# KatanaMajesty/Nebulae

Measured on AMD Instinct MI355X. Metric: denoised frames/s (1920x1080: GI 1 spp + SVGF temporal + a-trous), higher is better.
Workload: dtype f32

## Files before the change

### include/nebulae_hip.h

```cpp
#ifndef NEBULAE_HIP_H
#define NEBULAE_HIP_H

#include <stddef.h>
#include <stdint.h>

#ifdef __cplusplus
extern "C" {
#endif

typedef struct neb_ctx neb_ctx;
typedef void* neb_stream;

typedef enum neb_status {
    NEB_OK = 0,
    NEB_ERR_INVALID_ARG = -1,
    NEB_ERR_HIP = -2,
    NEB_ERR_NO_DEVICE = -3,
    NEB_ERR_STATE = -4,
    NEB_ERR_OUT_OF_RANGE = -5
} neb_status;

typedef enum neb_plane {
    NEB_PLANE_RADIANCE = 0,
    NEB_PLANE_NORMAL = 1,
    NEB_PLANE_DEPTH = 2,
    NEB_PLANE_MOMENTS = 3,
    NEB_PLANE_VARIANCE = 4,
    NEB_PLANE_SCRATCH = 5,
    NEB_PLANE_ALBEDO = 6,
    NEB_PLANE_ROUGH_METAL = 7,
    NEB_PLANE_WORLDPOS = 8,
    NEB_PLANE_LDR = 9,
    NEB_PLANE_GEOMETRY = 10,
    NEB_PLANE_HISTORY_LENGTH = 11,
    NEB_PLANE_COUNT = 12
} neb_plane;
#define NEB_PLANE_SUBMESH_ID 12

#define NEB_SLOT_CURRENT (-1)
#define NEB_SLOT_HISTORY (-2)

typedef struct neb_create_info {
    int32_t device;
    uint32_t width;
    uint32_t height;
    uint32_t row_begin;
    uint32_t row_end;
    uint32_t atrous_levels;
} neb_create_info;

typedef struct neb_svgf_params {
    float depthSigma;
    float alpha;
    float varianceEps;
    float phiColor;
    float phiNormal;
    float phiDepth;
} neb_svgf_params;

int neb_create(const neb_create_info* info, neb_ctx** out_ctx);
int neb_resize(neb_ctx* ctx, uint32_t width, uint32_t height);
int neb_destroy(neb_ctx* ctx);
const char* neb_last_error(const neb_ctx* ctx);
const char* neb_version(void);

int neb_marker_push(const char* name);
int neb_marker_pop(void);

int neb_begin_frame(neb_ctx* ctx, uint32_t frame_index);
int neb_end_frame(neb_ctx* ctx);
int neb_current_index(const neb_ctx* ctx);
int neb_history_index(const neb_ctx* ctx);

int neb_svgf_default_params(neb_svgf_params* out);
int neb_svgf_set_params(neb_ctx* ctx, const neb_svgf_params* p);
int neb_svgf_get_params(const neb_ctx* ctx, neb_svgf_params* out);
int neb_set_option(neb_ctx* ctx, const char* key, int value);

int neb_get_plane(neb_ctx* ctx, int plane, int slot, void** dptr, size_t* pitch_bytes, uint32_t* rows);
int neb_upload_rows(neb_ctx* ctx, int plane, int slot, uint32_t row0, uint32_t nrows, const void* host, neb_stream stream);
int neb_download_rows(neb_ctx* ctx, int plane, int slot, uint32_t row0, uint32_t nrows, void* host, neb_stream stream);
int neb_stream_synchronize(neb_ctx* ctx, neb_stream stream);

int neb_svgf_reset_history(neb_ctx* ctx, neb_stream stream);
int neb_svgf_temporal(neb_ctx* ctx, neb_stream stream);
int neb_svgf_atrous(neb_ctx* ctx, neb_stream stream);
int neb_svgf_denoise(neb_ctx* ctx, neb_stream stream);
int neb_svgf_level_times(neb_ctx* ctx, float* out_us, uint32_t capacity, uint32_t* n_out);
struct neb_camera;
int neb_svgf_set_camera(neb_ctx* ctx, int slot, const struct neb_camera* cam);
int neb_svgf_snapshot_transforms(neb_ctx* ctx, int slot, neb_stream stream);
int neb_svgf_debug_delta_table(neb_ctx* ctx, float* host, uint32_t capacity, uint32_t* n_out, neb_stream stream);
int neb_svgf_temporal_rows(neb_ctx* ctx, uint32_t row0, uint32_t row1, neb_stream stream);
int neb_svgf_atrous_level_rows(neb_ctx* ctx, uint32_t level, uint32_t row0, uint32_t row1, neb_stream stream);
int neb_svgf_atrous_level_planes(const neb_ctx* ctx, uint32_t level, int* src_plane, int* src_slot, int* dst_plane, int* dst_slot);

typedef struct neb_halo_plane {
    int32_t plane;
    int32_t slot;
} neb_halo_plane;
typedef struct neb_halo_swap {
    int32_t peer;
    uint32_t send_row0, send_row1;
    uint32_t recv_row0, recv_row1;
} neb_halo_swap;
int neb_strips_unique_id(void* id128);
int neb_strips_comm_create(int device, int n_ranks, int rank, const void* id128, void** out_comm);
int neb_strips_comm_destroy(void* comm);
int neb_strips_group_begin(void);
int neb_strips_group_end(void);
int neb_strips_exchange(neb_ctx* ctx, void* comm, const neb_halo_plane* planes, uint32_t n_planes, const neb_halo_swap* swaps, uint32_t n_swaps,
                        neb_stream stream);
const char* neb_strips_last_error(void);

enum { NEB_STRIPS_ONCE = 0, NEB_STRIPS_PER_LEVEL = 1, NEB_STRIPS_OVERLAP = 2 };
enum { NEB_STRIP_RESET_HISTORY = 1 };
typedef struct neb_strip_plan {
    uint32_t n_strips, strip;
    uint32_t scheme;
    uint32_t flags;
} neb_strip_plan;
typedef struct neb_strip_peers {
    neb_ctx* up;
    neb_ctx* down;
} neb_strip_peers;
struct neb_gi_constants;
int neb_strip_frame(neb_ctx* ctx, const struct neb_gi_constants* constants, void* comm, const neb_strip_plan* plan, neb_stream stream);
int neb_strip_frame_begin(neb_ctx* ctx, const struct neb_gi_constants* constants, const neb_strip_plan* plan, const neb_strip_peers* peers, neb_stream stream);
int neb_strip_frame_finish(neb_ctx* ctx, void* comm, const neb_strip_plan* plan, const neb_strip_peers* peers, neb_stream stream);
int neb_strip_rows(const neb_ctx* ctx, const neb_strip_plan* plan, uint32_t out[8]);


typedef struct neb_geometry_desc {
    float surfaceToWorld[16];
    int32_t materialIndex;
    uint32_t indexStride;
    uint32_t numIndices;
    uint32_t numVertices;
    const void* indices;
    const void* attributes[4];
    uint32_t attributeStrides[4];
    uint32_t _pad;
} neb_geometry_desc;

typedef struct neb_material_desc {
    int32_t textureIndices[3];
    float albedo[4];
    float roughnessMetalness[2];
    uint32_t _pad;
} neb_material_desc;

typedef struct neb_texture_desc {
    const void* rgba8;
    uint32_t width, height;
} neb_texture_desc;

typedef struct neb_gi_constants {
    uint32_t frameIndex;
    uint32_t samplesPerPixel;
    uint32_t maxPathVertices;
    float cameraWorldPos[3];
    float skyColor[3];
    float sunLightDirection[3];
    float sunLightRadiance[3];
    float sunTanHalfAngle;
    float throughputThreshold;
} neb_gi_constants;

typedef struct neb_gi_hit {
    float t;
    uint32_t geometry;
    uint32_t primitive;
    uint32_t flags;
} neb_gi_hit;

typedef struct neb_camera {
    float eye[3], target[3], up[3];
    float vfov_deg, znear, zfar;
} neb_camera;

int neb_gi_set_scene(neb_ctx* ctx, const neb_geometry_desc* geoms, uint32_t n_geoms, const neb_material_desc* mats,
                     uint32_t n_mats, const neb_texture_desc* texs, uint32_t n_texs);
int neb_gi_build_bvh(neb_ctx* ctx, neb_stream stream);
int neb_gi_update_transforms(neb_ctx* ctx, const uint32_t* geometry_indices, const float* surfaceToWorld ,
                             uint32_t n, neb_stream stream);
typedef struct neb_vertex_update {
    uint32_t geometry;
    uint32_t firstVertex, numVertices;
    const void* positions;
    uint32_t positionStride;
    const void* normals;
    uint32_t normalStride;
    const void* tangents;
    uint32_t tangentStride;
} neb_vertex_update;
int neb_gi_update_vertices(neb_ctx* ctx, const neb_vertex_update* updates, uint32_t n, neb_stream stream);
int neb_gi_scene_info(const neb_ctx* ctx, uint32_t* n_triangles, uint32_t* n_nodes);
int neb_gi_scene_bytes(const neb_ctx* ctx, uint64_t out[3]);
int neb_gi_bvh_depth(const neb_ctx* ctx, uint32_t* depth);
int neb_gi_build_passes(const neb_ctx* ctx, uint32_t* passes);
int neb_gi_build_ms(const neb_ctx* ctx, float* ms);
int neb_gi_trace(neb_ctx* ctx, const neb_gi_constants* constants, neb_stream stream);
int neb_gi_trace_rows(neb_ctx* ctx, const neb_gi_constants* constants, uint32_t row0, uint32_t row1, neb_stream stream);
int neb_gi_trace_begin(neb_ctx* ctx, const neb_gi_constants* constants, uint32_t row0, uint32_t row1, neb_stream stream);
int neb_gi_trace_finish(neb_ctx* ctx, neb_stream stream, void* after_shade_event);
int neb_gi_resolve(neb_ctx* ctx, neb_stream stream);
int neb_gi_ray_count(neb_ctx* ctx, uint64_t* rays, int reset, neb_stream stream);
int neb_gi_traversal_stats(neb_ctx* ctx, uint64_t out[5]);
int neb_gi_sun_table_stats(neb_ctx* ctx, uint64_t out[4], neb_stream stream);
int neb_gi_sun_table_build_ms(neb_ctx* ctx, float* ms);
int neb_gi_shadow_tail_mode(neb_ctx* ctx, int* mode, float us[2]);
int neb_gi_wave_stats(neb_ctx* ctx, uint64_t out[6]);
int neb_gi_node_index_stats(neb_ctx* ctx, uint64_t out[5]);
int neb_gi_debug_set_tile_order(neb_ctx* ctx, const uint32_t* order, uint32_t n);
int neb_gi_debug_sun_walk_stats(neb_ctx* ctx, uint64_t out[12]);
int neb_gi_download_hits(neb_ctx* ctx, neb_gi_hit* host, neb_stream stream);
int neb_debug_sort_pairs(neb_ctx* ctx, const uint32_t* keys, const uint32_t* values, uint32_t n, int bits, uint32_t* sorted_values);
int neb_pbr_direct(neb_ctx* ctx, const neb_gi_constants* constants, neb_stream stream);
int neb_tonemap(neb_ctx* ctx, neb_stream stream);
int neb_gbuffer_raycast(neb_ctx* ctx, const neb_camera* camera, neb_stream stream);

#ifdef __cplusplus
}
#endif
#endif
```

### nebulae_amd/_lib.py

```python
import ctypes as C
import os

from . import build as _build

NEB_OK = 0
PLANE_RADIANCE, PLANE_NORMAL, PLANE_DEPTH, PLANE_MOMENTS, PLANE_VARIANCE, PLANE_SCRATCH = 0, 1, 2, 3, 4, 5
PLANE_ALBEDO, PLANE_ROUGH_METAL, PLANE_WORLDPOS, PLANE_LDR, PLANE_GEOMETRY = 6, 7, 8, 9, 10
PLANE_HISTORY_LENGTH = 11
PLANE_SUBMESH_ID = 12
SLOT_CURRENT, SLOT_HISTORY = -1, -2


class NebError(RuntimeError):
    pass


class CreateInfo(C.Structure):
    _fields_ = [("device", C.c_int32), ("width", C.c_uint32), ("height", C.c_uint32), ("row_begin", C.c_uint32),
                ("row_end", C.c_uint32), ("atrous_levels", C.c_uint32)]


class HaloPlane(C.Structure):
    _fields_ = [("plane", C.c_int32), ("slot", C.c_int32)]


class HaloSwap(C.Structure):
    _fields_ = [("peer", C.c_int32), ("send_row0", C.c_uint32), ("send_row1", C.c_uint32), ("recv_row0", C.c_uint32), ("recv_row1", C.c_uint32)]


class SvgfParams(C.Structure):
    _fields_ = [(n, C.c_float) for n in ("depthSigma", "alpha", "varianceEps", "phiColor", "phiNormal", "phiDepth")]


_SIGS = {
    "neb_create": (C.c_int, [C.POINTER(CreateInfo), C.POINTER(C.c_void_p)]),
    "neb_resize": (C.c_int, [C.c_void_p, C.c_uint32, C.c_uint32]),
    "neb_destroy": (C.c_int, [C.c_void_p]),
    "neb_last_error": (C.c_char_p, [C.c_void_p]),
    "neb_version": (C.c_char_p, []),
    "neb_marker_push": (C.c_int, [C.c_char_p]),
    "neb_marker_pop": (C.c_int, []),
    "neb_begin_frame": (C.c_int, [C.c_void_p, C.c_uint32]),
    "neb_end_frame": (C.c_int, [C.c_void_p]),
    "neb_current_index": (C.c_int, [C.c_void_p]),
    "neb_history_index": (C.c_int, [C.c_void_p]),
    "neb_svgf_default_params": (C.c_int, [C.POINTER(SvgfParams)]),
    "neb_svgf_set_params": (C.c_int, [C.c_void_p, C.POINTER(SvgfParams)]),
    "neb_svgf_get_params": (C.c_int, [C.c_void_p, C.POINTER(SvgfParams)]),
    "neb_set_option": (C.c_int, [C.c_void_p, C.c_char_p, C.c_int]),
    "neb_get_plane": (C.c_int, [C.c_void_p, C.c_int, C.c_int, C.POINTER(C.c_void_p), C.POINTER(C.c_size_t),
                                C.POINTER(C.c_uint32)]),
    "neb_upload_rows": (C.c_int, [C.c_void_p, C.c_int, C.c_int, C.c_uint32, C.c_uint32, C.c_void_p, C.c_void_p]),
    "neb_download_rows": (C.c_int, [C.c_void_p, C.c_int, C.c_int, C.c_uint32, C.c_uint32, C.c_void_p, C.c_void_p]),
    "neb_stream_synchronize": (C.c_int, [C.c_void_p, C.c_void_p]),
    "neb_svgf_reset_history": (C.c_int, [C.c_void_p, C.c_void_p]),
    "neb_svgf_snapshot_transforms": (C.c_int, [C.c_void_p, C.c_int, C.c_void_p]),
    "neb_svgf_debug_delta_table": (C.c_int, [C.c_void_p, C.POINTER(C.c_float), C.c_uint32, C.POINTER(C.c_uint32), C.c_void_p]),
    "neb_svgf_level_times": (C.c_int, [C.c_void_p, C.POINTER(C.c_float), C.c_uint32, C.POINTER(C.c_uint32)]),
    "neb_svgf_temporal": (C.c_int, [C.c_void_p, C.c_void_p]),
    "neb_svgf_atrous": (C.c_int, [C.c_void_p, C.c_void_p]),
    "neb_svgf_denoise": (C.c_int, [C.c_void_p, C.c_void_p]),
    "neb_svgf_temporal_rows": (C.c_int, [C.c_void_p, C.c_uint32, C.c_uint32, C.c_void_p]),
    "neb_svgf_atrous_level_rows": (C.c_int, [C.c_void_p, C.c_uint32, C.c_uint32, C.c_uint32, C.c_void_p]),
    "neb_svgf_atrous_level_planes": (C.c_int, [C.c_void_p, C.c_uint32] + [C.POINTER(C.c_int)] * 4),
    "neb_strips_unique_id": (C.c_int, [C.c_void_p]),
    "neb_strips_comm_create": (C.c_int, [C.c_int, C.c_int, C.c_int, C.c_void_p, C.POINTER(C.c_void_p)]),
    "neb_strips_comm_destroy": (C.c_int, [C.c_void_p]),
    "neb_strips_group_begin": (C.c_int, []),
    "neb_strips_group_end": (C.c_int, []),
    "neb_strips_exchange": (C.c_int, [C.c_void_p, C.c_void_p, C.POINTER(HaloPlane), C.c_uint32, C.POINTER(HaloSwap), C.c_uint32, C.c_void_p]),
    "neb_strips_last_error": (C.c_char_p, []),
}



class StripPlan(C.Structure):
    _fields_ = [("n_strips", C.c_uint32), ("strip", C.c_uint32), ("scheme", C.c_uint32), ("flags", C.c_uint32)]


class StripPeers(C.Structure):
    _fields_ = [("up", C.c_void_p), ("down", C.c_void_p)]


class VertexUpdate(C.Structure):
    _fields_ = [("geometry", C.c_uint32), ("firstVertex", C.c_uint32), ("numVertices", C.c_uint32),
                ("positions", C.c_void_p), ("positionStride", C.c_uint32), ("normals", C.c_void_p), ("normalStride", C.c_uint32),
                ("tangents", C.c_void_p), ("tangentStride", C.c_uint32)]


STRIP_SCHEMES = {"once": 0, "per_level": 1, "overlap": 2}
STRIP_RESET_HISTORY = 1


def _gi_sigs():
    from . import scene as S
    return {
        "neb_gi_set_scene": (C.c_int, [C.c_void_p, C.POINTER(S.GeometryDesc), C.c_uint32, C.POINTER(S.MaterialDesc), C.c_uint32,
                                       C.POINTER(S.TextureDesc), C.c_uint32]),
        "neb_gi_build_bvh": (C.c_int, [C.c_void_p, C.c_void_p]),
        "neb_gi_update_transforms": (C.c_int, [C.c_void_p, C.POINTER(C.c_uint32), C.POINTER(C.c_float), C.c_uint32, C.c_void_p]),
        "neb_gi_update_vertices": (C.c_int, [C.c_void_p, C.POINTER(VertexUpdate), C.c_uint32, C.c_void_p]),
        "neb_gi_scene_info": (C.c_int, [C.c_void_p, C.POINTER(C.c_uint32), C.POINTER(C.c_uint32)]),
        "neb_gi_bvh_depth": (C.c_int, [C.c_void_p, C.POINTER(C.c_uint32)]),
        "neb_gi_build_passes": (C.c_int, [C.c_void_p, C.POINTER(C.c_uint32)]),
        "neb_gi_build_ms": (C.c_int, [C.c_void_p, C.POINTER(C.c_float)]),
        "neb_gi_scene_bytes": (C.c_int, [C.c_void_p, C.POINTER(C.c_uint64)]),
        "neb_gi_trace": (C.c_int, [C.c_void_p, C.POINTER(S.GIConstants), C.c_void_p]),
        "neb_gi_trace_rows": (C.c_int, [C.c_void_p, C.POINTER(S.GIConstants), C.c_uint32, C.c_uint32, C.c_void_p]),
        "neb_gi_resolve": (C.c_int, [C.c_void_p, C.c_void_p]),
        "neb_gi_trace_begin": (C.c_int, [C.c_void_p, C.POINTER(S.GIConstants), C.c_uint32, C.c_uint32, C.c_void_p]),
        "neb_gi_trace_finish": (C.c_int, [C.c_void_p, C.c_void_p, C.c_void_p]),
        "neb_gi_ray_count": (C.c_int, [C.c_void_p, C.POINTER(C.c_uint64), C.c_int, C.c_void_p]),
        "neb_gi_traversal_stats": (C.c_int, [C.c_void_p, C.POINTER(C.c_uint64)]),
        "neb_gi_wave_stats": (C.c_int, [C.c_void_p, C.POINTER(C.c_uint64)]),
        "neb_gi_node_index_stats": (C.c_int, [C.c_void_p, C.POINTER(C.c_uint64)]),
        "neb_gi_debug_set_tile_order": (C.c_int, [C.c_void_p, C.c_void_p, C.c_uint32]),
        "neb_gi_debug_sun_walk_stats": (C.c_int, [C.c_void_p, C.POINTER(C.c_uint64)]),
        "neb_gi_sun_table_build_ms": (C.c_int, [C.c_void_p, C.POINTER(C.c_float)]),
        "neb_gi_shadow_tail_mode": (C.c_int, [C.c_void_p, C.POINTER(C.c_int), C.POINTER(C.c_float)]),
        "neb_gi_sun_table_stats": (C.c_int, [C.c_void_p, C.POINTER(C.c_uint64), C.c_void_p]),
        "neb_gi_download_hits": (C.c_int, [C.c_void_p, C.c_void_p, C.c_void_p]),
        "neb_debug_sort_pairs": (C.c_int, [C.c_void_p, C.c_void_p, C.c_void_p, C.c_uint32, C.c_int, C.c_void_p]),
        "neb_pbr_direct": (C.c_int, [C.c_void_p, C.POINTER(S.GIConstants), C.c_void_p]),
        "neb_tonemap": (C.c_int, [C.c_void_p, C.c_void_p]),
        "neb_gbuffer_raycast": (C.c_int, [C.c_void_p, C.POINTER(S.CameraDesc), C.c_void_p]),
        "neb_svgf_set_camera": (C.c_int, [C.c_void_p, C.c_int, C.POINTER(S.CameraDesc)]),
        "neb_strip_frame": (C.c_int, [C.c_void_p, C.POINTER(S.GIConstants), C.c_void_p, C.POINTER(StripPlan), C.c_void_p]),
        "neb_strip_frame_begin": (C.c_int, [C.c_void_p, C.POINTER(S.GIConstants), C.POINTER(StripPlan), C.POINTER(StripPeers), C.c_void_p]),
        "neb_strip_frame_finish": (C.c_int, [C.c_void_p, C.c_void_p, C.POINTER(StripPlan), C.POINTER(StripPeers), C.c_void_p]),
        "neb_strip_rows": (C.c_int, [C.c_void_p, C.POINTER(StripPlan), C.POINTER(C.c_uint32)]),
    }


_LIB = None


def exported_symbols():
    return sorted(set(_SIGS) | set(_gi_sigs()))


def load(build_if_missing=True):
    global _LIB
    if _LIB is not None:
        return _LIB
    path = os.environ.get("NEB_LIB_PATH")
    if not path:
        path = _build.LIB_PATH
        if build_if_missing and _build.needs_build():
            _build.build()
    if not os.path.exists(path):
        raise NebError(f"{path} is missing and could not be built; nebulae_amd has no CPU fallback")
    lib = C.CDLL(path)
    for name, (res, args) in {**_SIGS, **_gi_sigs()}.items():
        fn = getattr(lib, name)
        fn.restype = res
        fn.argtypes = args
    _LIB = lib
    return lib


def check(lib, ctx, rc, what):
    if rc != NEB_OK:
        msg = lib.neb_last_error(ctx)
        raise NebError(f"{what} failed ({rc}): {msg.decode() if msg else '?'}")
```

### nebulae_amd/csrc/gi.hip

```cpp
#include "gi_device.h"
#include "svgf_reproject.h"

namespace neb {

#ifndef NEB_SORT_BITS
#define NEB_SORT_BITS 16
#endif
constexpr int kSortBits = NEB_SORT_BITS;
static_assert(kSortBits >= 1 && kSortBits <= 16, "raysort.hip sorts at most two 8-bit digits");

__device__ __forceinline__ uint32_t bounce_sort_key(float3 o, float3 d, const float* smin, const float* sinv)
{
    const uint32_t oct = (d.x < 0.f ? 1u : 0u) | (d.y < 0.f ? 2u : 0u) | (d.z < 0.f ? 4u : 0u);
    const uint32_t key = (oct << (kSortBits - 3)) | (morton30(o, smin, sinv) >> (30 - (kSortBits - 3)));
    return min(key, (1u << kSortBits) - 2u);
}

struct GiRecords {
    float4* ray_o;
    float4* ray_d;
    float4* hit;
    float4* path;
    float4* state;
    float4* srec;
};
constexpr int kSrO = 0, kSrD = 1, kSrContrib = 2, kSrSum = 3;

struct GiArgs {
    SceneView S;
    neb_gi_constants c;
    GiRecords R;
    const uint32_t* albedo;
    const uint32_t* rough_metal;
    const uint2* world_pos;
    const uint2* normal;
    float4* radiance;
    neb_gi_hit* hits;
    unsigned long long* ray_counter;
    uint32_t* bounce_counts;
    uint32_t* shadow_counts;
    uint32_t* table_counts;
    uint32_t sun_table;
    uint32_t hint_pairs;
    uint32_t W, row_begin, row0, row1, tiles_x;
    uint32_t sample;
    uint32_t bounce;
    uint32_t stats;
    uint32_t defer_resolve;
    const uint32_t* tile_order;
    uint32_t* sort_keys;
    uint32_t* sort_vals;
    const uint32_t* sort_order;
    uint32_t* bsort_keys;
    uint32_t* bsort_vals;
    uint32_t raygen_only;
    float4* list;
    uint32_t* list_counts;
    uint32_t list_cap, list_set;
    float smin[3], sinv[3];
    uint32_t first_px, n_px;
    const ShadeHeader* heads;
    float sun_L[3], sun_B[3], sun_T[3];
};
template <uint32_t RUNS>
__device__ __forceinline__ uint32_t gi_block()
{
    if constexpr (RUNS == 0u)
        return blockIdx.x;
    const uint32_t seg_len = ((gridDim.x + RUNS - 1u) / RUNS + 7u) & ~7u;
    const uint32_t seg = blockIdx.x / seg_len, b = blockIdx.x - seg * seg_len;
    const uint32_t n = min(seg_len, gridDim.x - seg * seg_len);
    const uint32_t q = n >> 3, r = n & 7u, xcd = b & 7u, k = b >> 3;
    return seg * seg_len + (xcd < r ? xcd * (q + 1u) + k : r * (q + 1u) + (xcd - r) * q + k);
}
constexpr uint32_t kShadeRuns = 16u, kRaygenRuns = 16u;
constexpr uint32_t kListSegments = 128u;
#ifndef NEB_LIST_QUAD_BELOW
#define NEB_LIST_QUAD_BELOW 1500000u
#endif
#ifndef NEB_LIST_WAVES
#define NEB_LIST_WAVES 6
#endif

template <uint32_t RUNS = 0u>
__device__ __forceinline__ bool gi_pixel(const GiArgs& a, uint32_t& x, uint32_t& y, size_t& i)
{
    const uint32_t lane = threadIdx.x;
    const uint32_t blk = gi_block<RUNS>();
    const uint32_t tile_x = blk % a.tiles_x, tile_y = blk / a.tiles_x;
    x = tile_x * 8 + (lane & 7);
    y = a.row0 + tile_y * 8 + (lane >> 3);
    i = (size_t)(y - a.row_begin) * a.W + x;
    return x < a.W && y < a.row1;
}

__device__ __forceinline__ void count_rays(uint32_t* block_counts, uint32_t mine, uint32_t slot)
{
    uint32_t total = mine;
#pragma unroll
    for (int off = 32; off > 0; off >>= 1)
        total += __shfl_down(total, off);
    if ((threadIdx.x & 63u) == 0 && total)
        block_counts[slot] += total;
}
__device__ __forceinline__ void count_rays(uint32_t* block_counts, uint32_t mine) { count_rays(block_counts, mine, blockIdx.x); }

#ifndef NEB_RG_STACK
#define NEB_RG_STACK 12
#endif
constexpr int kRgStack = NEB_RG_STACK;
static_assert(32 * (kRgStack * 256 + 1024) <= 160 * 1024 || NEB_TRACE_WAVES < 8, "LDS budget of the closest-hit pass: 32 waves per CU of stacks and child slots in 160 KB");
__global__ __launch_bounds__(64, NEB_TRACE_WAVES) void gi_raygen_trace_kernel(GiArgs a)
{
    __shared__ int stack_mem[kRgStack * 64];
    __shared__ __attribute__((aligned(16))) int child_slot_mem[256];
    uint32_t x, y;
    size_t i64;
    bool active;
    if (a.tile_order) {
        const uint32_t blk = a.tile_order[blockIdx.x], tile_x = blk % a.tiles_x, tile_y = blk / a.tiles_x;
        x = tile_x * 8 + (threadIdx.x & 7);
        y = a.row0 + tile_y * 8 + (threadIdx.x >> 3);
        i64 = (size_t)(y - a.row_begin) * a.W + x;
        active = x < a.W && y < a.row1;
    } else {
        active = gi_pixel<kRaygenRuns>(a, x, y, i64);
    }
    const uint32_t i = (uint32_t)i64, lane = threadIdx.x;
    uint32_t rays = 0;
    uint32_t wave_stamp[5] = {0u, 0u, 0u, 0u, 0u};
    if (active) {
        const float3 albedo = unpack_r11g11b10(a.albedo[i]);
        const uint2 wp = a.world_pos[i];
        const float3 worldPos = f3(half_bits_to_float(wp.x & 0xffffu), half_bits_to_float(wp.x >> 16), half_bits_to_float(wp.y & 0xffffu));
        const uint32_t nzw = a.normal[i].y;
        const float3 SN = oct_unpack(half_bits_to_float(nzw & 0xffffu), half_bits_to_float(nzw >> 16));
        const float metalness = half_bits_to_float(a.rough_metal[i] >> 16);
        uint32_t rng;
        float3 V;
        if (a.sample == 0) {
            rng = jenkins((x + y * a.W) ^ jenkins(a.c.frameIndex));
            V = f3(a.c.cameraWorldPos[0], a.c.cameraWorldPos[1], a.c.cameraWorldPos[2]) - worldPos;
        } else {
            const float4 st = a.R.state[i];
            V = f3(st.x, st.y, st.z);
            rng = __float_as_uint(st.w);
        }
        (void)rand01(rng);
        const float3 F0 = specular_f0(albedo, metalness);
        float3 throughput = f3(1, 1, 1) * (albedo * (1.0f - metalness));
        const float pd = 1.0f - specular_probability(saturate1(dot3(normalize3(V), SN)), F0, albedo);
        if (rand01(rng) < pd)
            throughput = f3(throughput.x / pd, throughput.y / pd, throughput.z / pd);
        const float u0 = rand01(rng), u1 = rand01(rng);
        const float3 dir = cosine_hemisphere_aligned(u0, u1, SN);
        const float3 org = worldPos + SN * 1e-2f;
        const bool bounce = a.c.maxPathVertices > 1;
        a.R.path[i] = make_float4(throughput.x, throughput.y, throughput.z, __uint_as_float(rng));
        a.R.ray_o[i] = make_float4(org.x, org.y, org.z, 0.01f);
        a.R.ray_d[i] = make_float4(dir.x, dir.y, dir.z, bounce ? 1.0f : 0.0f);
        if (a.sample + 1 < a.c.samplesPerPixel)
            a.R.state[i] = make_float4(V.x, V.y, V.z, __uint_as_float(rng));
        float4 h = make_float4(bounce ? -1.0f : -2.0f, 0.f, 0.f, 0.f);
        rays = bounce ? 1u : 0u;
        wave_stamp[0] = wave_stamp[1] = wave_stamp[2] = wave_stamp[3] = wave_stamp[4] = 0u;
        if (a.bsort_keys) {
            a.bsort_keys[i] = bounce ? bounce_sort_key(org, dir, a.smin, a.sinv) : (1u << kSortBits) - 1u;
            a.bsort_vals[i] = (uint32_t)i;
        }
        if (bounce && !a.raygen_only && a.S.n_tris) {
            Hit hit;
            const bool found = a.stats ? traverse_t<false, true, kRgStack, true>(a.S, org, dir, 0.01f, kTraceMax, stack_mem + lane, hit, stack_mem, child_slot_mem + 4u * lane)
                                       : traverse_t<false, false, kRgStack, true>(a.S, org, dir, 0.01f, kTraceMax, stack_mem + lane, hit, stack_mem, child_slot_mem + 4u * lane);
            if (found)
                h = make_float4(hit.t, hit.u, hit.v, __uint_as_float(hit.tri));
            if (a.stats) {
                wave_stamp[0] = hit.w_iters, wave_stamp[1] = hit.w_node_iters, wave_stamp[2] = hit.w_node_lanes, wave_stamp[3] = hit.w_leaf_iters,
                wave_stamp[4] = hit.w_leaf_lanes;
                atomicAdd(a.ray_counter + 1, (unsigned long long)hit.node_visits);
                atomicAdd(a.ray_counter + 2, (unsigned long long)hit.tri_tests);
#pragma unroll
                for (int k = 0; k < 4; ++k)
                    atomicAdd(a.ray_counter + 11 + k, (unsigned long long)hit.top_visits[k]);
                atomicAdd(a.ray_counter + 15, (unsigned long long)hit.deep_sp);
                a.R.srec[4 * i + kSrContrib].w = __uint_as_float(hit.node_visits + ((hit.tri_tests + 3u) >> 2));
            }
        }
        a.R.hit[i] = h;
    }
    count_rays(a.bounce_counts, rays);
    if (a.stats) {
#pragma unroll
        for (int k = 0; k < 5; ++k) {
            uint32_t v = wave_stamp[k];
#pragma unroll
            for (int off = 32; off > 0; off >>= 1)
                v = max(v, (uint32_t)__shfl_xor((int)v, off));
            if (lane == 0)
                atomicAdd(a.ray_counter + 6 + k, (unsigned long long)v);
        }
        if (lane == 0)
            atomicAdd(a.ray_counter + 5, 1ull);
    }
}

__global__ __launch_bounds__(64, NEB_TRACE_WAVES) void gi_bounce_trace_kernel(GiArgs a)
{
    __shared__ int stack_mem[kLdsStack * 64];
    uint32_t x, y;
    size_t i = 0;
    bool active;
    if (a.sort_order) {
        const uint32_t j = blockIdx.x * 64u + threadIdx.x;
        active = j < a.n_px;
        if (active)
            i = a.sort_order[j];
    } else {
        active = gi_pixel(a, x, y, i);
    }
    uint32_t rays = 0;
    if (active) {
        const float4 rd = a.R.ray_d[i];
        if (rd.w != 0.0f) {
            const float4 ro = a.R.ray_o[i];
            Hit hit;
            rays = 1;
            float4 h = make_float4(-1.0f, 0.f, 0.f, 0.f);
            if (traverse(a.S, f3(ro.x, ro.y, ro.z), f3(rd.x, rd.y, rd.z), ro.w, kTraceMax, false, stack_mem + threadIdx.x, hit))
                h = make_float4(hit.t, hit.u, hit.v, __uint_as_float(hit.tri));
            a.R.hit[i] = h;
        }
    }
    if (a.bounce > 1)
        count_rays(a.bounce_counts, rays);
}

struct ShadeOut {
    float4 rec_o = {0.f, 0.f, 0.f, 0.f}, shadow_d = {0.f, 0.f, 0.f, 0.f} , rec_c = {0.f, 0.f, 0.f, 0.f}, sum = {0.f, 0.f, 0.f, 0.f};
    uint32_t rays = 0;
    uint32_t table = 0;
};

template <bool FAST>
__device__ __forceinline__ void shade_pixel(const GiArgs& a, size_t i, const float4 h, const float4 pth, const float4 rd, const float4 ro, ShadeOut& o,
                                            const float4* staged, uint32_t staged_swz)
{
    const uint32_t trav_iters = a.stats ? __float_as_uint(a.R.srec[4 * i + kSrContrib].w) : 0u;
    float3 throughput = f3(pth.x, pth.y, pth.z);
    if (!(a.sample == 0 && a.bounce == 1))
        o.sum = a.R.srec[4 * i + kSrSum];
    float4 next_d = make_float4(0.f, 0.f, 0.f, 0.f);
    neb_gi_hit dbg = {-1.0f, ~0u, ~0u, 0u};
    const bool alive = rd.w != 0.0f;
    if (alive && h.x == -1.0f) {
        o.sum.x += a.c.skyColor[0] * throughput.x;
        o.sum.y += a.c.skyColor[1] * throughput.y;
        o.sum.z += a.c.skyColor[2] * throughput.z;
    } else if (alive && h.x >= 0.0f) {
        const uint32_t tri = __float_as_uint(h.w);
        Surface surf;
        const TriShade ts = load_tri_shade_at(staged, staged_swz);
        const ShadeHead head = load_shade_header(a.heads, ts.geom);
        const bool hint_fetch = a.sun_table && a.hint_pairs && !((ts.lit >> ts.hint_side) & 1u) && ts.hint[0] != kNoHint;
        float4 ha0 = make_float4(0.f, 0.f, 0.f, 0.f), hb0 = ha0, hc0 = ha0, ha1 = ha0, hb1 = ha0, hc1 = ha0;
        if (hint_fetch) {
            const uint32_t h0 = ts.hint[0], h1 = ts.hint[1] != kNoHint ? ts.hint[1] : h0;
            ha0 = a.S.tris[3 * h0], hb0 = a.S.tris[3 * h0 + 1], hc0 = a.S.tris[3 * h0 + 2];
            ha1 = a.S.tris[3 * h1], hb1 = a.S.tris[3 * h1 + 1], hc1 = a.S.tris[3 * h1 + 2];
        }
        const bool shaded = reconstruct_surface<FAST>(a.S, head, ts, h.y, h.z, surf);
        dbg.t = h.x;
        dbg.geometry = ts.geom;
        if (a.hits)
            dbg.primitive = __float_as_uint(a.S.shade[8 * (size_t)tri + 7].x);
        if (shaded) {
            const float3 org = f3(ro.x, ro.y, ro.z), dir = f3(rd.x, rd.y, rd.z);
            const float3 hitP = org + dir * h.x;
            const float3 V = normalize3<FAST>(-dir);
            uint32_t rng = __float_as_uint(pth.w);
            const float a0 = rand01(rng), a1 = rand01(rng);
            const float angle = a0 * 2.0f * 3.1415926535f, dist = fsqrt<false>(a1);
            const float3 sun_rad = f3(a.c.sunLightRadiance[0], a.c.sunLightRadiance[1], a.c.sunLightRadiance[2]);
            const float3 L = f3(a.sun_L[0], a.sun_L[1], a.sun_L[2]), Bv = f3(a.sun_B[0], a.sun_B[1], a.sun_B[2]), T = f3(a.sun_T[0], a.sun_T[1], a.sun_T[2]);
            float sn_a, cs_a;
            det_sincosf(angle, sn_a, cs_a);
            const float3 inc = normalize3<false>(L + (Bv * sn_a + T * cs_a) * a.c.sunTanHalfAngle * dist);
            const bool transition = dot3(surf.GN, inc) <= 0.0f;
            const float3 so = hitP + (transition ? -surf.GN : surf.GN) * 1e-2f;
            const float3 O = evaluate_direct_brdf<FAST>(surf, V, L) * sun_rad * throughput;
            o.rays = 1;
            const uint32_t side = transition ? 1u : 0u;
            bool hinted_hit = false;
            if (a.sun_table && !((ts.lit >> side) & 1u) && ts.hint_side == side && ts.hint[0] != kNoHint) {
                float tt, uu, vv;
#pragma unroll
                for (int pair = 0; pair < kHints && !hinted_hit; pair += 2) {
                    const uint32_t h0 = ts.hint[pair];
                    if (h0 == kNoHint || (uint32_t)pair >= 2u * a.hint_pairs)
                        break;
                    if (pair == 0) {
                        hinted_hit = intersect_tri_regs(ha0, hb0, hc0, so, inc, 0.001f, kTraceMax, tt, uu, vv) ||
                                     intersect_tri_regs(ha1, hb1, hc1, so, inc, 0.001f, kTraceMax, tt, uu, vv);
                        continue;
                    }
                    const uint32_t h1 = ts.hint[pair + 1] != kNoHint ? ts.hint[pair + 1] : h0;
                    const float4 a0 = a.S.tris[3 * h0], b0 = a.S.tris[3 * h0 + 1], c0 = a.S.tris[3 * h0 + 2];
                    const float4 a1 = a.S.tris[3 * h1], b1 = a.S.tris[3 * h1 + 1], c1 = a.S.tris[3 * h1 + 2];
                    hinted_hit = intersect_tri_regs(a0, b0, c0, so, inc, 0.001f, kTraceMax, tt, uu, vv) ||
                                 intersect_tri_regs(a1, b1, c1, so, inc, 0.001f, kTraceMax, tt, uu, vv);
                }
            }
            if (hinted_hit) {
                o.table = 1;
            } else if (a.sun_table && ((ts.lit >> side) & 1u)) {
                o.sum.x += O.x;
                o.sum.y += O.y;
                o.sum.z += O.z;
                o.table = 1;
                dbg.flags |= 1u;
            } else {
                o.rec_o = make_float4(so.x, so.y, so.z, 0.001f);
                o.shadow_d = make_float4(inc.x, inc.y, inc.z, 1.0f);
                o.rec_c = make_float4(O.x, O.y, O.z, 0.f);
            }
            if (a.bounce + 1 < a.c.maxPathVertices) {
                uint32_t rng_copy = rng;
                const float3 SNn = normalize3<FAST>(surf.SN);
                const float e0 = rand01(rng_copy), e1 = rand01(rng_copy);
                const float3 Ld = cosine_hemisphere_aligned<FAST>(e0, e1, SNn);
                const float pdiff = 1.0f - specular_probability<FAST>(saturate1(dot3(V, SNn)), specular_f0(surf.albedo, surf.metalness), surf.albedo);
                const float3 no = hitP + surf.GN * 1e-2f;
                throughput = throughput * (surf.albedo * (1.0f - surf.metalness));
                if (rand01(rng) < pdiff)
                    throughput = f3(fdiv<FAST>(throughput.x, pdiff), fdiv<FAST>(throughput.y, pdiff), fdiv<FAST>(throughput.z, pdiff));
                a.R.ray_o[i] = make_float4(no.x, no.y, no.z, 0.001f);
                next_d = make_float4(Ld.x, Ld.y, Ld.z, 1.0f);
                a.R.path[i] = make_float4(throughput.x, throughput.y, throughput.z, __uint_as_float(rng));
            }
            if (a.sample + 1 < a.c.samplesPerPixel)
                a.R.state[i] = make_float4(V.x, V.y, V.z, __uint_as_float(rng));
        }
    }
    if (a.bounce + 1 < a.c.maxPathVertices)
        a.R.ray_d[i] = next_d;
    if (a.sort_keys) {
        uint32_t key = (1u << kSortBits) - 1u;
        if (o.shadow_d.w != 0.0f) {
            key = min(morton30(f3(o.rec_o.x, o.rec_o.y, o.rec_o.z), a.smin, a.sinv) >> (30 - kSortBits), (1u << kSortBits) - 2u);
        }
        a.sort_keys[i] = key;
        a.sort_vals[i] = (uint32_t)i;
    }
    if (a.bsort_keys) {
        uint32_t key = (1u << kSortBits) - 1u;
        if (next_d.w != 0.0f) {
            const float4 no4 = a.R.ray_o[i];
            key = bounce_sort_key(f3(no4.x, no4.y, no4.z), f3(next_d.x, next_d.y, next_d.z), a.smin, a.sinv);
        }
        a.bsort_keys[i] = key;
        a.bsort_vals[i] = (uint32_t)i;
    }
    if (a.hits && a.bounce == 1) {
        if (a.stats)
            dbg.flags |= min(trav_iters, 4095u) << 8;
        a.hits[i] = dbg;
    }
}

template <bool FAST>
__global__ __launch_bounds__(64, NEB_SHADE_WAVES) void gi_shade_kernel(GiArgs a)
{
    uint32_t x, y;
    size_t i;
    const bool active = gi_pixel<kShadeRuns>(a, x, y, i);
    ShadeOut o;
    float4 h = make_float4(-2.0f, 0.f, 0.f, 0.f);
    const bool final_vertex = a.sample + 1 == a.c.samplesPerPixel && a.bounce + 1 >= a.c.maxPathVertices && !a.defer_resolve;
    float4 pth = make_float4(0.f, 0.f, 0.f, 0.f), rd = pth, ro = pth, rad = pth;
    if (active) {
        h = a.R.hit[i];
        pth = a.R.path[i];
        rd = a.R.ray_d[i];
        ro = a.R.ray_o[i];
        if (a.list && final_vertex)
            rad = a.radiance[i];
    }
    __shared__ float4 smem[64 * 8];
    const uint32_t lane = threadIdx.x;
    const bool has_hit = active && h.x >= 0.0f;
    const uint32_t my_tri = has_hit ? __float_as_uint(h.w) : ~0u;
#pragma unroll
    for (uint32_t it = 0; it < 8; ++it) {
        const uint32_t src = it * 8u + (lane >> 3);
        const uint32_t t = (uint32_t)__shfl((int)my_tri, (int)src);
        if (t != ~0u) {
            const float4* g = a.S.shade + 8 * (size_t)t + ((lane & 7u) ^ (src & 7u));
            __builtin_amdgcn_global_load_lds((const __attribute__((address_space(1))) void*)g, (__attribute__((address_space(3))) void*)(smem + it * 64u), 16, 0, 0);
        }
    }
    __syncthreads();
    if (active)
        shade_pixel<FAST>(a, i, h, pth, rd, ro, o, smem + lane * 8u, lane & 7u);
    if (a.list) {
        const bool trace = active && o.shadow_d.w != 0.0f;
        if (active && !trace) {
            if (final_vertex) {
                if (o.sum.x != 0.0f || o.sum.y != 0.0f || o.sum.z != 0.0f) {
                    const float inv_spp = 1.0f / (float)a.c.samplesPerPixel;
                    float4 r = rad;
                    r.x += o.sum.x * inv_spp;
                    r.y += o.sum.y * inv_spp;
                    r.z += o.sum.z * inv_spp;
                    a.radiance[i] = r;
                }
            } else {
                a.R.srec[4 * i + kSrSum] = o.sum;
            }
        }
        const unsigned long long m = __ballot(trace);
        if (m) {
            const uint32_t seg = blockIdx.x % kListSegments;
            uint32_t base = 0;
            if (lane == 0)
                base = atomicAdd(a.list_counts + a.list_set * kListSegments + seg, (uint32_t)__popcll(m));
            base = (uint32_t)__shfl((int)base, 0);
            if (trace) {
                const uint32_t slot = base + (uint32_t)__popcll(m & ((1ull << lane) - 1ull));
                float4* rec = a.list + 4 * ((size_t)seg * a.list_cap + slot);
                rec[kSrO] = make_float4(o.rec_o.x, o.rec_o.y, o.rec_o.z, __uint_as_float((uint32_t)i));
                rec[kSrD] = o.shadow_d;
                rec[kSrContrib] = o.rec_c;
                rec[kSrSum] = o.sum;
            }
        }
        count_rays(a.shadow_counts, o.rays);
        count_rays(a.table_counts, o.table);
        return;
    }
    __syncthreads();
    float4* xpose = smem;
    xpose[lane * 4 + kSrO] = o.rec_o;
    xpose[lane * 4 + kSrD] = o.shadow_d;
    xpose[lane * 4 + kSrContrib] = o.rec_c;
    xpose[lane * 4 + kSrSum] = o.sum;
    __syncthreads();
    const uint32_t blk = gi_block<kShadeRuns>();
    const uint32_t tile_x = blk % a.tiles_x, tile_y = blk / a.tiles_x;
#pragma unroll
    for (uint32_t k = 0; k < 4; ++k) {
        const uint32_t row = 2 * k + (lane >> 5), col = (lane & 31u) >> 2, comp = lane & 3u;
        const uint32_t px = tile_x * 8 + col, py = a.row0 + tile_y * 8 + row;
        if (px < a.W && py < a.row1)
            a.R.srec[4 * ((size_t)(py - a.row_begin) * a.W + px) + comp] = xpose[(row * 8 + col) * 4 + comp];
    }
    count_rays(a.shadow_counts, o.rays);
    count_rays(a.table_counts, o.table);
}

__device__ __forceinline__ void shadow_wave(const GiArgs& a, size_t i, bool valid, int* stack_mem)
{
    float4* stage = reinterpret_cast<float4*>(stack_mem);
    const uint32_t lane = threadIdx.x;
    const uint32_t my_px = valid ? (uint32_t)i : ~0u;
#pragma unroll
    for (uint32_t it = 0; it < 4; ++it) {
        const uint32_t src = it * 16u + (lane >> 2);
        const uint32_t p = (uint32_t)__shfl((int)my_px, (int)src);
        if (p != ~0u) {
            const float4* g = a.R.srec + 4 * (size_t)p + ((lane & 3u) ^ (src & 3u));
            __builtin_amdgcn_global_load_lds((const __attribute__((address_space(1))) void*)g, (__attribute__((address_space(3))) void*)(stage + it * 64u), 16, 0, 0);
        }
    }
    __syncthreads();
    const uint32_t swz = lane & 3u;
    const float4 rd = stage[lane * 4u + (kSrD ^ swz)], ro = stage[lane * 4u + (kSrO ^ swz)], contrib = stage[lane * 4u + (kSrContrib ^ swz)];
    float4 sum = stage[lane * 4u + (kSrSum ^ swz)];
    __syncthreads();
    if (!valid)
        return;
    if (rd.w != 0.0f) {
        Hit sh;
        const bool occluded = traverse(a.S, f3(ro.x, ro.y, ro.z), f3(rd.x, rd.y, rd.z), ro.w, kTraceMax, true, stack_mem + threadIdx.x, sh, a.stats != 0);
        if (a.stats) {
            if (a.hits && a.bounce == 1)
                a.hits[i].flags |= min(sh.node_visits, 4095u) << 20;
            atomicAdd(a.ray_counter + 3, (unsigned long long)sh.node_visits);
            atomicAdd(a.ray_counter + 4, (unsigned long long)sh.tri_tests);
        }
        if (!occluded) {
            sum.x += contrib.x;
            sum.y += contrib.y;
            sum.z += contrib.z;
            if (a.hits && a.bounce == 1)
                a.hits[i].flags |= 1u;
        }
    }
    const bool last_vertex = a.bounce + 1 >= a.c.maxPathVertices;
    if (a.sample + 1 == a.c.samplesPerPixel && last_vertex && !a.defer_resolve) {
        if (sum.x != 0.0f || sum.y != 0.0f || sum.z != 0.0f) {
            const float inv_spp = 1.0f / (float)a.c.samplesPerPixel;
            float4 r = a.radiance[i];
            r.x += sum.x * inv_spp;
            r.y += sum.y * inv_spp;
            r.z += sum.z * inv_spp;
            a.radiance[i] = r;
        }
    } else {
        a.R.srec[4 * i + kSrSum] = sum;
    }
}

__global__ __launch_bounds__(64, NEB_TRACE_WAVES) void gi_shadow_trace_kernel(GiArgs a)
{
    __shared__ int stack_mem[kLdsStack * 64];
    static_assert(kLdsStack * 64 * sizeof(int) >= 64 * 4 * sizeof(float4), "the shadow records are staged in the stack's LDS");
    uint32_t x, y;
    size_t i = 0;
    bool valid;
    if (a.sort_order) {
        const uint32_t j = blockIdx.x * 64u + threadIdx.x;
        valid = j < a.n_px;
        if (valid)
            i = a.sort_order[j];
    } else {
        valid = gi_pixel(a, x, y, i);
    }
    shadow_wave(a, i, valid, stack_mem);
}

constexpr uint32_t kListChunks = 64u;
template <bool QUAD>
__global__ __launch_bounds__(64, NEB_LIST_WAVES) void gi_shadow_list_kernel(GiArgs a)
{
    __shared__ int stack_mem[kLdsStack * 64];
    const uint32_t lane = threadIdx.x;
    const uint32_t seg = blockIdx.x % kListSegments, chunks = gridDim.x / kListSegments;
    const uint32_t count = a.list_counts[a.list_set * kListSegments + seg];
    if (blockIdx.x == 0)
        for (uint32_t k = lane; k < kListSegments; k += 64u)
            a.list_counts[(a.list_set ^ 1u) * kListSegments + k] = 0u;
    static_assert(kLdsStack * 64 >= 16 * 64, "a quad's LDS column holds the whole 64-entry stack");
    constexpr uint32_t kRaysPerWave = QUAD ? 16u : 64u;
    const uint32_t slot = QUAD ? lane >> 2 : lane;
    for (uint32_t first = (blockIdx.x / kListSegments) * kRaysPerWave; first < count; first += chunks * kRaysPerWave) {
        if (first + slot >= count)
            continue;
        const float4* rec = a.list + 4 * ((size_t)seg * a.list_cap + first + slot);
        const float4 ro = rec[kSrO], rd = rec[kSrD], contrib = rec[kSrContrib];
        float4 sum = rec[kSrSum];
        const size_t i = __float_as_uint(ro.w);
        Hit sh;
        bool occluded;
        if constexpr (QUAD) {
            occluded = a.stats ? traverse_any_quad<true>(a.S, f3(ro.x, ro.y, ro.z), f3(rd.x, rd.y, rd.z), 0.001f, kTraceMax, stack_mem + slot, sh.node_visits, sh.tri_tests)
                               : traverse_any_quad<false>(a.S, f3(ro.x, ro.y, ro.z), f3(rd.x, rd.y, rd.z), 0.001f, kTraceMax, stack_mem + slot, sh.node_visits, sh.tri_tests);
            if ((lane & 3u) != 0u)
                continue;
        } else {
            occluded = traverse(a.S, f3(ro.x, ro.y, ro.z), f3(rd.x, rd.y, rd.z), 0.001f, kTraceMax, true, stack_mem + lane, sh, a.stats != 0);
        }
        if (a.stats) {
            if (a.hits && a.bounce == 1)
                a.hits[i].flags |= min(sh.node_visits, 4095u) << 20;
            atomicAdd(a.ray_counter + 3, (unsigned long long)sh.node_visits);
            atomicAdd(a.ray_counter + 4, (unsigned long long)sh.tri_tests);
        }
        if (!occluded) {
            sum.x += contrib.x;
            sum.y += contrib.y;
            sum.z += contrib.z;
            if (a.hits && a.bounce == 1)
                a.hits[i].flags |= 1u;
        }
        const bool last_vertex = a.bounce + 1 >= a.c.maxPathVertices;
        if (a.sample + 1 == a.c.samplesPerPixel && last_vertex && !a.defer_resolve) {
            if (sum.x != 0.0f || sum.y != 0.0f || sum.z != 0.0f) {
                const float inv_spp = 1.0f / (float)a.c.samplesPerPixel;
                float4 r = a.radiance[i];
                r.x += sum.x * inv_spp;
                r.y += sum.y * inv_spp;
                r.z += sum.z * inv_spp;
                a.radiance[i] = r;
            }
        } else {
            a.R.srec[4 * i + kSrSum] = sum;
        }
    }
}

struct GbufArgs {
    SceneView S;
    float eye[3], xaxis[3], yaxis[3], zaxis[3];
    float tan_half, aspect, m22, m32;
    uint32_t* albedo;
    uint32_t* rough_metal;
    uint2* world_pos;
    uint2* normal;
    uint32_t* depth;
    uint32_t W, H, row_begin, row0, row1, tiles_x;
    uint32_t* submesh_id;
};

__global__ __launch_bounds__(64) void gbuffer_kernel(GbufArgs a)
{
    __shared__ int stack_mem[kLdsStack * 64];
    const uint32_t lane = threadIdx.x;
    int* stack = stack_mem + lane;
    const uint32_t tile_x = blockIdx.x % a.tiles_x, tile_y = blockIdx.x / a.tiles_x;
    const uint32_t x = tile_x * 8 + (lane & 7), y = a.row0 + tile_y * 8 + (lane >> 3);
    if (x >= a.W || y >= a.row1)
        return;
    const size_t i = (size_t)(y - a.row_begin) * a.W + x;
    const float3 eye = f3(a.eye[0], a.eye[1], a.eye[2]), xa = f3(a.xaxis[0], a.xaxis[1], a.xaxis[2]),
                 ya = f3(a.yaxis[0], a.yaxis[1], a.yaxis[2]), za = f3(a.zaxis[0], a.zaxis[1], a.zaxis[2]);
    const float ndc_x = ((float)x + 0.5f) / (float)a.W * 2.0f - 1.0f;
    const float ndc_y = 1.0f - ((float)y + 0.5f) / (float)a.H * 2.0f;
    const float3 dir = normalize3(xa * (ndc_x * a.aspect * a.tan_half) + ya * (ndc_y * a.tan_half) - za);
    Hit h;
    bool hit = traverse(a.S, eye, dir, 0.0f, 1e30f, false, stack, h);
    float depth = 1.0f;
    float3 hitP = f3(0, 0, 0);
    if (hit) {
        hitP = eye + dir * h.t;
        const float zv = dot3(hitP - eye, za);
        depth = (a.m22 * zv + a.m32) / (-zv);
        if (!(depth >= 0.0f && depth <= 1.0f))
            hit = false;
    }
    float3 alb = f3(0, 0, 0);
    float rm0 = 0.f, rm1 = 0.f;
    float2 egn = make_float2(0.f, 0.f), esn = make_float2(0.f, 0.f);
    uint32_t ds = 0x00ffffffu;
    uint32_t geom = 0xFFFFFFFFu;
    if (hit) {
        const float4 ids = a.S.tris[3 * h.tri + 2];
        geom = __float_as_uint(ids.y);
        const DevGeom g = a.S.geoms[geom];
        const float b1 = h.u, b2 = h.v, b0 = 1.0f - (b1 + b2);
        rm0 = 1.0f;
        float3 GN = f3(0, 0, 1), SN = f3(0, 0, 1);
        if (g.valid) {
            const TriShade ts = load_tri_shade(a.S, h.tri);
            const float3 n0 = ts.n0, n1 = ts.n1, n2 = ts.n2;
            const float3 w0 = normalize3(xform_dir(g.m, n0)), w1 = normalize3(xform_dir(g.m, n1)), w2 = normalize3(xform_dir(g.m, n2));
            GN = normalize3(w0 * b0 + w1 * b1 + w2 * b2);
            SN = GN;
            const float u = ts.uv0.x * b0 + ts.uv1.x * b1 + ts.uv2.x * b2;
            const float v = ts.uv0.y * b0 + ts.uv1.y * b1 + ts.uv2.y * b2;
            if (g.material >= 0) {
                const DevMat m = a.S.mats[g.material];
                MapSamples maps;
                sample_material_maps(a.S, m, u, v, maps);
                if (m.tex[0] >= 0) {
                    const float4 t = maps.albedo;
                    alb = f3(t.x, t.y, t.z);
                }
                if (m.tex[1] >= 0) {
                    const float3 tg0 = f3(ts.t0.x, ts.t0.y, ts.t0.z), tg1 = f3(ts.t1.x, ts.t1.y, ts.t1.z), tg2 = f3(ts.t2.x, ts.t2.y, ts.t2.z);
                    const float3 bt0 = normalize3(cross3(normalize3(n0), tg0) * ts.t0.w);
                    const float3 bt1 = normalize3(cross3(normalize3(n1), tg1) * ts.t1.w);
                    const float3 bt2 = normalize3(cross3(normalize3(n2), tg2) * ts.t2.w);
                    const float3 T = normalize3(tg0 * b0 + tg1 * b1 + tg2 * b2);
                    const float3 B = normalize3(bt0 * b0 + bt1 * b1 + bt2 * b2);
                    const float4 t = maps.normal;
                    const float3 N = f3(t.x * 2.0f - 1.0f, t.y * 2.0f - 1.0f, t.z * 2.0f - 1.0f);
                    SN = normalize3(T * N.x + B * N.y + GN * N.z);
                }
                if (m.tex[2] >= 0) {
                    const float4 t = maps.rm;
                    rm0 = t.y;
                    rm1 = t.z;
                }
            }
        }
        egn = oct_pack(GN);
        esn = oct_pack(SN);
        ds = (uint32_t)rint((double)depth * 16777215.0) | 0xff000000u;
    }
    a.albedo[i] = small_float_encode(alb.x, 6) | (small_float_encode(alb.y, 6) << 11) | (small_float_encode(alb.z, 5) << 22);
    a.rough_metal[i] = float_to_half_bits(rm0) | (float_to_half_bits(rm1) << 16);
    a.world_pos[i] = make_uint2(float_to_half_bits(hitP.x) | (float_to_half_bits(hitP.y) << 16), float_to_half_bits(hitP.z));
    a.normal[i] = make_uint2(float_to_half_bits(egn.x) | (float_to_half_bits(egn.y) << 16),
                             float_to_half_bits(esn.x) | (float_to_half_bits(esn.y) << 16));
    a.depth[i] = ds;
    if (a.submesh_id)
        a.submesh_id[i] = geom;
}

__global__ __launch_bounds__(256) void gi_resolve_kernel(float4* __restrict__ radiance, const float4* __restrict__ srec, size_t first, size_t n,
                                                         float inv_spp)
{
    const size_t k = (size_t)blockIdx.x * 256 + threadIdx.x;
    if (k >= n)
        return;
    const float4 s = srec[4 * (first + k) + kSrSum];
    float4 r = radiance[first + k];
    r.x += s.x * inv_spp;
    r.y += s.y * inv_spp;
    r.z += s.z * inv_spp;
    radiance[first + k] = r;
}

__global__ __launch_bounds__(64) void pbr_direct_kernel(GiArgs a)
{
    __shared__ int stack_mem[kLdsStack * 64];
    uint32_t x, y;
    size_t i;
    const bool active = gi_pixel(a, x, y, i);
    uint32_t rays = 0;
    if (active) {
        const float3 albedo = unpack_r11g11b10(a.albedo[i]);
        const uint2 wp = a.world_pos[i];
        const float3 worldPos = f3(half_bits_to_float(wp.x & 0xffffu), half_bits_to_float(wp.x >> 16), half_bits_to_float(wp.y & 0xffffu));
        const uint32_t nzw = a.normal[i].y;
        const float3 SN = oct_unpack(half_bits_to_float(nzw & 0xffffu), half_bits_to_float(nzw >> 16));
        const uint32_t rm = a.rough_metal[i];
        const float rough = half_bits_to_float(rm & 0xffffu), metal = half_bits_to_float(rm >> 16);
        const float3 eye = f3(a.c.cameraWorldPos[0], a.c.cameraWorldPos[1], a.c.cameraWorldPos[2]);
        const float3 sun_dir = f3(a.c.sunLightDirection[0], a.c.sunLightDirection[1], a.c.sunLightDirection[2]);
        const float3 sun_rad = f3(a.c.sunLightRadiance[0], a.c.sunLightRadiance[1], a.c.sunLightRadiance[2]);
        const float3 V = normalize3(eye - worldPos);
        const float VdotN = fminf(fmaxf(dot3(V, SN), 0.00001f), 1.0f);
        const float3 L = normalize3(-sun_dir);
        const float3 Hv = normalize3(L + V);
        const float LdotN = fminf(fmaxf(dot3(L, SN), 0.00001f), 1.0f);
        const float VdotH = fminf(fmaxf(dot3(V, Hv), 0.00001f), 1.0f);
        const float NdotH = fminf(fmaxf(dot3(SN, Hv), 0.00001f), 1.0f);
        const float3 F0 = specular_f0(albedo, metal);
        const float3 F = fresnel_schlick(F0, VdotH);
        const float3 Kd = f3(1.0f - F.x, 1.0f - F.y, 1.0f - F.z);
        const float denom = 1.0f / (4.0f * VdotN * LdotN);
        const float alpha = rough * rough, a2 = alpha * alpha;
        const float dd = (NdotH * NdotH) * (a2 - 1.0f) + 1.0f;
        const float ndf = a2 / (kPi * dd * dd);
        const float k = alpha * 0.5f;
        const float gsf = (VdotN * (1.0f / (VdotN * (1.0f - k) + k))) * (LdotN * (1.0f / (LdotN * (1.0f - k) + k)));
        const float cs = ndf * gsf;
        const float3 O = Kd * (albedo * kPiInv) + f3(cs * F.x * denom, cs * F.y * denom, cs * F.z * denom);
        uint32_t rng = jenkins((x + y * (x / 8u)) ^ jenkins(a.c.frameIndex));
        const float a0 = rand01(rng), a1 = rand01(rng);
        const float angle = a0 * 2.0f * 3.1415926535f, dist = sqrtf(a1);
        const float3 Bv = normalize3(perpendicular(L));
        const float3 T = cross3(Bv, L);
        float sn_a, cs_a;
        det_sincosf(angle, sn_a, cs_a);
        const float3 inc = normalize3(L + (Bv * sn_a + T * cs_a) * a.c.sunTanHalfAngle * dist);
        Hit h;
        rays = 1;
        const bool occluded = traverse(a.S, worldPos + SN * 1e-2f, inc, 0.0f, 3.402823466e+38f, true, stack_mem + threadIdx.x, h);
        const float vis = occluded ? 0.0f : 1.0f;
        a.radiance[i] = make_float4(O.x * LdotN * sun_rad.x * vis, O.y * LdotN * sun_rad.y * vis, O.z * LdotN * sun_rad.z * vis, 1.0f);
    }
    count_rays(a.shadow_counts, rays);
}

__global__ __launch_bounds__(256) void tonemap_kernel(const float4* __restrict__ radiance, uint32_t* __restrict__ ldr, size_t n)
{
    const size_t i = (size_t)blockIdx.x * 256 + threadIdx.x;
    if (i >= n)
        return;
    const float4 c = radiance[i];
    float v[3] = {0.59719f * c.x + 0.35458f * c.y + 0.04823f * c.z, 0.07600f * c.x + 0.90834f * c.y + 0.01566f * c.z,
                  0.02840f * c.x + 0.13383f * c.y + 0.83777f * c.z};
#pragma unroll
    for (int r = 0; r < 3; ++r) {
        const float aa = v[r] * (v[r] + 0.0245786f) - 0.000090537f;
        const float bb = v[r] * (0.983729f * v[r] + 0.4329510f) + 0.238081f;
        v[r] = aa / bb;
    }
    const float o0 = saturate1(1.60475f * v[0] + -0.53108f * v[1] + -0.07367f * v[2]);
    const float o1 = saturate1(-0.10208f * v[0] + 1.10813f * v[1] + -0.00605f * v[2]);
    const float o2 = saturate1(-0.00327f * v[0] + -0.07276f * v[1] + 1.07602f * v[2]);
    const float luma = saturate1(o0 * 0.2126f + o1 * 0.7152f + o2 * 0.0722f);
    ldr[i] = (uint32_t)(o0 * 255.0f + 0.5f) | ((uint32_t)(o1 * 255.0f + 0.5f) << 8) | ((uint32_t)(o2 * 255.0f + 0.5f) << 16) |
             ((uint32_t)(luma * 255.0f + 0.5f) << 24);
}

}

using namespace neb;

extern "C" {

static int gi_dispatch(neb_ctx* ctx, const neb_gi_constants* c, uint32_t row0, uint32_t row1, neb_stream stream, int phase, hipEvent_t after_shade)
{
    if (!ctx || !c)
        return ctx ? gi_fail(ctx, NEB_ERR_INVALID_ARG, "neb_gi_trace: null constants") : NEB_ERR_INVALID_ARG;
    if (int rc = neb::svgf_flush_pending(ctx))
        return rc;
    GiState* g = ctx->gi;
    if (!g || !g->built)
        return gi_fail(ctx, NEB_ERR_STATE, "neb_gi_trace: scene/BVH not ready (neb_gi_set_scene + neb_gi_build_bvh)");
    if (row0 < ctx->row_begin || row1 > ctx->row_end || row0 > row1)
        return gi_fail(ctx, NEB_ERR_OUT_OF_RANGE, "neb_gi_trace: rows not resident");
    if (c->samplesPerPixel == 0 || c->maxPathVertices > 8)
        return gi_fail(ctx, NEB_ERR_INVALID_ARG, "neb_gi_trace: samplesPerPixel must be >= 1 and maxPathVertices <= 8 (MaxPathtracingRecursionDepth)");
    if (row0 == row1) {
        if (phase == 1 && g->begun - g->finished < 2u) {
            GiState::DispatchSet& e = g->sets[g->begun & 1u];
            e.split_c = *c;
            e.split_row0 = e.split_row1 = row0;
            g->begun++;
        } else if (phase == 2) {
            g->finished++;
        }
        return NEB_OK;
    }
    GI_GUARD(ctx);
    ScopedRange range("GI: Query Pass");
    const size_t npx = (size_t)ctx->W * (ctx->row_end - ctx->row_begin);
    if (g->defer_resolve == 2 && g->traces - g->resolves >= 2u)
        return gi_fail(ctx, NEB_ERR_STATE, "neb_gi_trace: both record sets hold a dispatch that neb_gi_resolve has not retired yet");
    if (phase == 0 && g->begun != g->finished)
        return gi_fail(ctx, NEB_ERR_STATE, "neb_gi_trace: a dispatch begun with neb_gi_trace_begin still waits for its neb_gi_trace_finish");
    if (phase != 0) {
        if (g->defer_resolve == 2)
            return gi_fail(ctx, NEB_ERR_STATE, "neb_gi_trace_begin / _finish: not together with gi_defer_resolve = 2 (the two-call form alternates the record sets itself; 1 is fine)");
        if (c->samplesPerPixel != 1 || c->maxPathVertices > 2 || g->sort_bounce)
            return gi_fail(ctx, NEB_ERR_STATE, "neb_gi_trace_begin / _finish: one sample and one bounce per pixel only, bounce-ray sorting off (use neb_gi_trace)");
        if (phase == 1 && g->begun - g->finished >= 2u)
            return gi_fail(ctx, NEB_ERR_STATE, "neb_gi_trace_begin: both record sets hold a dispatch that neb_gi_trace_finish has not completed yet");
    }
    GiState::DispatchSet& ds = g->sets[phase == 1 ? (g->begun & 1u) : phase == 2 ? (g->finished & 1u) : g->defer_resolve == 2 ? (g->traces & 1u) : 0u];
    if (g->debug_hits && !g->d_hits) {
        void* p = nullptr;
        GI_HIP(ctx, hipMalloc(&p, npx * sizeof(neb_gi_hit)));
        GI_HIP(ctx, hipMemset(p, 0, npx * sizeof(neb_gi_hit)));
        g->allocs.push_back(p);
        g->d_hits = (neb_gi_hit*)p;
    }
    if (!ds.d_records) {
        void* p = nullptr;
        GI_HIP(ctx, hipMalloc(&p, npx * sizeof(float4) * 9));
        g->allocs.push_back(p);
        ds.d_records = (float4*)p;
    }
    GiArgs a;
    a.S = g->view;
    a.c = *c;
    a.R.ray_o = ds.d_records;
    a.R.ray_d = ds.d_records + npx;
    a.R.hit = ds.d_records + 2 * npx;
    a.R.path = ds.d_records + 3 * npx;
    a.R.state = ds.d_records + 4 * npx;
    a.R.srec = ds.d_records + 5 * npx;
    a.albedo = (const uint32_t*)ctx->planes[NEB_PLANE_ALBEDO][0];
    a.rough_metal = (const uint32_t*)ctx->planes[NEB_PLANE_ROUGH_METAL][0];
    a.world_pos = (const uint2*)ctx->planes[NEB_PLANE_WORLDPOS][0];
    a.normal = (const uint2*)ctx->planes[NEB_PLANE_NORMAL][ctx->cur];
    a.radiance = (float4*)ctx->planes[NEB_PLANE_RADIANCE][ctx->cur];
    a.hits = g->debug_hits ? g->d_hits : nullptr;
    a.ray_counter = g->d_ray_counter;
    a.W = ctx->W;
    a.row_begin = ctx->row_begin;
    a.row0 = row0;
    a.row1 = row1;
    a.tiles_x = (ctx->W + 7) / 8;
    a.stats = g->debug_hits ? 1u : 0u;
    a.sort_keys = a.sort_vals = nullptr;
    a.sort_order = nullptr;
    a.tile_order = (g->d_tile_order && g->tile_order_n == a.tiles_x * ((row1 - row0 + 7) / 8)) ? g->d_tile_order : nullptr;
    a.first_px = (uint32_t)((size_t)(row0 - ctx->row_begin) * ctx->W);
    a.n_px = (uint32_t)((size_t)(row1 - row0) * ctx->W);
    for (int q = 0; q < 3; ++q) {
        a.smin[q] = g->scene_min[q];
        a.sinv[q] = 1.0f / fmaxf(g->scene_max[q] - g->scene_min[q], 1e-20f);
    }
    a.bsort_keys = a.bsort_vals = nullptr;
    a.raygen_only = 0;
    GI_HIP(ctx, gi_scene_reader(g, (hipStream_t)stream));
    if (phase != 1) {
        GI_HIP(ctx, gi_sun_table_update(g, *c, (hipStream_t)stream));
        GI_HIP(ctx, gi_sun_table_order(g, (hipStream_t)stream));
        g->last_dispatch_stream = (hipStream_t)stream;
        g->last_dispatch_stream_set = true;
    }
    a.heads = g->shade_heads;
    sun_frame(c->sunLightDirection, a.sun_L, a.sun_B, a.sun_T);
    a.sun_table = g->sun_table_state == 1 ? 1u : 0u;
    a.hint_pairs = (uint32_t)g->sun_hints / 2u;
    int tail_slot = -1;
    bool tail_warm = false;
    if (a.sun_table && g->compact_shadow && g->tail_tune && phase != 1) {
        if (g->tail_phase == 3 && hipEventQuery(g->tail_ev[1]) == hipSuccess && hipEventQuery(g->tail_ev[3]) == hipSuccess) {
            float ms_lists = 0.f, ms_sorted = 0.f;
            if (hipEventElapsedTime(&ms_lists, g->tail_ev[0], g->tail_ev[1]) == hipSuccess && hipEventElapsedTime(&ms_sorted, g->tail_ev[2], g->tail_ev[3]) == hipSuccess) {
                g->tail_us[0] = ms_lists * 1e3f, g->tail_us[1] = ms_sorted * 1e3f;
                g->tail_sorted = ms_sorted < 0.95f * ms_lists;
            }
            g->tail_phase = 0;
        } else if (g->tail_phase == 1 && !ds.d_list) {
        } else if (g->tail_phase == 2 && !ds.d_sort && (g->sort_shadow_auto ? a.n_px >= 1500000u : g->sort_shadow)) {
            tail_warm = true;
        } else if (g->tail_phase == 1 || g->tail_phase == 2) {
            tail_slot = g->tail_phase == 1 ? 0 : 2;
            for (int k = 0; k < 2; ++k)
                if (!g->tail_ev[tail_slot + k])
                    GI_HIP(ctx, hipEventCreate(&g->tail_ev[tail_slot + k]));
            g->tail_phase++;
        }
        (void)hipGetLastError();
    }
    const bool compact = a.sun_table && g->compact_shadow && !tail_warm && (tail_slot >= 0 ? tail_slot == 0 : !g->tail_sorted);
    const bool sort_shadow = !compact && (g->sort_shadow_auto ? a.n_px >= 1500000u : g->sort_shadow);
    if (sort_shadow || g->sort_bounce) {
        if (!ds.d_sort) {
            void* p = nullptr;
            GI_HIP(ctx, hipMalloc(&p, 8 * npx * sizeof(uint32_t)));
            g->allocs.push_back(p);
            ds.d_sort = (uint32_t*)p;
            const size_t bytes = ray_sort_scratch_bytes(npx);
            GI_HIP(ctx, hipMalloc(&p, bytes));
            g->allocs.push_back(p);
            ds.d_sort_temp = p;
            g->sort_temp_bytes = bytes;
        }
        if (sort_shadow) {
            a.sort_keys = ds.d_sort;
            a.sort_vals = ds.d_sort + npx;
        }
        if (g->sort_bounce) {
            a.bsort_keys = ds.d_sort + 4 * npx;
            a.bsort_vals = ds.d_sort + 5 * npx;
            a.raygen_only = 1;
        }
    }
    a.defer_resolve = g->defer_resolve ? 1u : 0u;
    ds.pending_spp = c->samplesPerPixel;
    ds.pending_row0 = row0;
    ds.pending_row1 = row1;
    if (g->defer_resolve == 2)
        g->traces++;
    if (g->defer_resolve == 1 && phase != 1) {
        ds.awaiting_resolve = true;
        ds.resolve_seq = ++g->resolve_seq;
    }
    const uint32_t tiles_y = (row1 - row0 + 7) / 8;
    const dim3 grid(a.tiles_x * tiles_y), block(64);
    const size_t n_blocks = (size_t)a.tiles_x * ((ctx->row_end - ctx->row_begin + 7) / 8 + 1);
    if (!ds.d_block_counts) {
        void* p = nullptr;
        GI_HIP(ctx, hipMalloc(&p, 3 * n_blocks * sizeof(uint32_t)));
        GI_HIP(ctx, hipMemset(p, 0, 3 * n_blocks * sizeof(uint32_t)));
        g->allocs.push_back(p);
        ds.d_block_counts = (uint32_t*)p;
        g->n_block_counts = n_blocks;
    }
    a.bounce_counts = ds.d_block_counts;
    a.shadow_counts = ds.d_block_counts + g->n_block_counts;
    a.table_counts = ds.d_block_counts + 2 * g->n_block_counts;
    a.list = nullptr;
    a.list_counts = nullptr;
    a.list_cap = a.list_set = 0;
    uint32_t list_waves = 0;
    if (compact) {
        const uint32_t wg_per_list = (uint32_t)((g->n_block_counts + kListSegments - 1) / kListSegments);
        if (!ds.d_list) {
            void* p = nullptr;
            GI_HIP(ctx, hipMalloc(&p, (size_t)kListSegments * wg_per_list * 64u * 64u + 4096u));
            GI_HIP(ctx, hipMemset(p, 0, 4096u));
            g->allocs.push_back(p);
            ds.d_list = (uint32_t*)p;
        }
        a.list_counts = ds.d_list;
        a.list = (float4*)((char*)ds.d_list + 4096);
        a.list_cap = wg_per_list * 64u;
        list_waves = kListSegments * (wg_per_list < kListChunks ? wg_per_list : kListChunks);
    }
    const uint32_t n_vertices = c->maxPathVertices > 1 ? c->maxPathVertices - 1 : 1;
    for (uint32_t s = 0; s < c->samplesPerPixel; ++s) {
        a.sample = s;
        for (uint32_t b = 1; b <= n_vertices; ++b) {
            a.bounce = b;
            if (b == 1 && phase != 2) {
                hipLaunchKernelGGL(gi_raygen_trace_kernel, grid, block, 0, (hipStream_t)stream, a);
            }
            if (phase == 1)
                continue;
            if (g->sort_bounce) {
                uint32_t* bs = ds.d_sort + 4 * npx;
                GI_HIP(ctx, ray_sort_pairs(bs + a.first_px, bs + npx + a.first_px, bs + 2 * npx + a.first_px, bs + 3 * npx + a.first_px,
                                           bs + npx + a.first_px, a.n_px, kSortBits, ds.d_sort_temp, (hipStream_t)stream));
                GiArgs b1 = a;
                b1.sort_order = bs + npx + a.first_px;
                hipLaunchKernelGGL(gi_bounce_trace_kernel, dim3((a.n_px + 63) / 64), block, 0, (hipStream_t)stream, b1);
            } else if (b > 1) {
                hipLaunchKernelGGL(gi_bounce_trace_kernel, grid, block, 0, (hipStream_t)stream, a);
            }
            a.list_set = ds.list_epoch & 1u;
            if (tail_slot >= 0 && s == 0 && b == 1)
                GI_HIP(ctx, hipEventRecord(g->tail_ev[tail_slot], (hipStream_t)stream));
            if (!g->exact_shade)
                hipLaunchKernelGGL(gi_shade_kernel<true>, grid, block, 0, (hipStream_t)stream, a);
            else
                hipLaunchKernelGGL(gi_shade_kernel<false>, grid, block, 0, (hipStream_t)stream, a);
            if (after_shade)
                GI_HIP(ctx, hipEventRecord(after_shade, (hipStream_t)stream));
            if (a.list) {
                if (a.n_px < NEB_LIST_QUAD_BELOW)
                    hipLaunchKernelGGL(gi_shadow_list_kernel<true>, dim3(list_waves), block, 0, (hipStream_t)stream, a);
                else
                    hipLaunchKernelGGL(gi_shadow_list_kernel<false>, dim3(list_waves), block, 0, (hipStream_t)stream, a);
                ds.list_epoch++;
            } else if (sort_shadow) {
                GI_HIP(ctx, ray_sort_pairs(ds.d_sort + a.first_px, ds.d_sort + npx + a.first_px, ds.d_sort + 2 * npx + a.first_px,
                                           ds.d_sort + 3 * npx + a.first_px, ds.d_sort + npx + a.first_px, a.n_px, kSortBits, ds.d_sort_temp,
                                           (hipStream_t)stream));
                GiArgs b2 = a;
                b2.sort_order = ds.d_sort + npx + a.first_px;
                hipLaunchKernelGGL(gi_shadow_trace_kernel, dim3((a.n_px + 63) / 64), block, 0, (hipStream_t)stream, b2);
            } else {
                hipLaunchKernelGGL(gi_shadow_trace_kernel, grid, block, 0, (hipStream_t)stream, a);
            }
        }
    }
    if (tail_slot >= 0)
        GI_HIP(ctx, hipEventRecord(g->tail_ev[tail_slot + 1], (hipStream_t)stream));
    GI_HIP(ctx, hipGetLastError());
    if (phase == 1) {
        ds.split_c = *c;
        ds.split_row0 = row0;
        ds.split_row1 = row1;
        g->begun++;
    } else if (phase == 2) {
        g->finished++;
    }
    return NEB_OK;
}

int neb_gi_trace_rows(neb_ctx* ctx, const neb_gi_constants* c, uint32_t row0, uint32_t row1, neb_stream stream)
{
    return gi_dispatch(ctx, c, row0, row1, stream, 0, nullptr);
}

int neb_gi_trace_begin(neb_ctx* ctx, const neb_gi_constants* c, uint32_t row0, uint32_t row1, neb_stream stream)
{
    return gi_dispatch(ctx, c, row0, row1, stream, 1, nullptr);
}

int neb_gi_trace_finish(neb_ctx* ctx, neb_stream stream, void* after_shade_event)
{
    if (!ctx || !ctx->gi)
        return ctx ? gi_fail(ctx, NEB_ERR_STATE, "neb_gi_trace_finish: no scene") : NEB_ERR_INVALID_ARG;
    GiState* g = ctx->gi;
    if (g->begun == g->finished)
        return gi_fail(ctx, NEB_ERR_STATE, "neb_gi_trace_finish: nothing begun (neb_gi_trace_begin first)");
    const GiState::DispatchSet& ds = g->sets[g->finished & 1u];
    const neb_gi_constants c = ds.split_c;
    return gi_dispatch(ctx, &c, ds.split_row0, ds.split_row1, stream, 2, (hipEvent_t)after_shade_event);
}

int neb_gi_resolve(neb_ctx* ctx, neb_stream stream)
{
    if (!ctx)
        return NEB_ERR_INVALID_ARG;
    if (int rc = neb::svgf_flush_pending(ctx))
        return rc;
    GiState* g = ctx->gi;
    if (!g || !g->defer_resolve || (g->defer_resolve == 2 && g->resolves == g->traces))
        return gi_fail(ctx, NEB_ERR_STATE, "neb_gi_resolve: nothing pending (set option gi_defer_resolve=1 and call neb_gi_trace first)");
    uint32_t which = g->defer_resolve == 2 ? (g->resolves & 1u) : 0u;
    if (g->defer_resolve == 1) {
        const bool a0 = g->sets[0].awaiting_resolve, a1 = g->sets[1].awaiting_resolve;
        if (!a0 && !a1)
            return gi_fail(ctx, NEB_ERR_STATE, "neb_gi_resolve: nothing pending (set option gi_defer_resolve=1 and call neb_gi_trace first)");
        which = (a0 && a1) ? (g->sets[1].resolve_seq < g->sets[0].resolve_seq ? 1u : 0u) : (a1 ? 1u : 0u);
        g->sets[which].awaiting_resolve = false;
    }
    GiState::DispatchSet& ds = g->sets[which];
    if (!ds.d_records)
        return gi_fail(ctx, NEB_ERR_STATE, "neb_gi_resolve: nothing pending (set option gi_defer_resolve=1 and call neb_gi_trace first)");
    if (g->defer_resolve == 2)
        g->resolves++;
    if (ds.pending_row1 <= ds.pending_row0)
        return NEB_OK;
    GI_GUARD(ctx);
    ScopedRange range("GI: Resolve query data");
    const size_t npx = (size_t)ctx->W * (ctx->row_end - ctx->row_begin);
    const size_t first = (size_t)(ds.pending_row0 - ctx->row_begin) * ctx->W, n = (size_t)(ds.pending_row1 - ds.pending_row0) * ctx->W;
    hipLaunchKernelGGL(gi_resolve_kernel, dim3((unsigned)((n + 255) / 256)), dim3(256), 0, (hipStream_t)stream,
                       (float4*)ctx->planes[NEB_PLANE_RADIANCE][ctx->cur], ds.d_records + 5 * npx, first, n, 1.0f / (float)ds.pending_spp);
    GI_HIP(ctx, hipGetLastError());
    return NEB_OK;
}

int neb_pbr_direct(neb_ctx* ctx, const neb_gi_constants* c, neb_stream stream)
{
    if (!ctx || !c)
        return ctx ? gi_fail(ctx, NEB_ERR_INVALID_ARG, "neb_pbr_direct: null constants") : NEB_ERR_INVALID_ARG;
    if (int rc = neb::svgf_flush_pending(ctx))
        return rc;
    GiState* g = ctx->gi;
    if (!g || !g->built)
        return gi_fail(ctx, NEB_ERR_STATE, "neb_pbr_direct: scene/BVH not ready (neb_gi_set_scene + neb_gi_build_bvh)");
    GI_GUARD(ctx);
    ScopedRange range("PBR Direct Lighting + Shadows");
    GI_HIP(ctx, gi_scene_reader(g, (hipStream_t)stream));
    GiArgs a{};
    a.S = g->view;
    a.c = *c;
    a.albedo = (const uint32_t*)ctx->planes[NEB_PLANE_ALBEDO][0];
    a.rough_metal = (const uint32_t*)ctx->planes[NEB_PLANE_ROUGH_METAL][0];
    a.world_pos = (const uint2*)ctx->planes[NEB_PLANE_WORLDPOS][0];
    a.normal = (const uint2*)ctx->planes[NEB_PLANE_NORMAL][ctx->cur];
    a.radiance = (float4*)ctx->planes[NEB_PLANE_RADIANCE][ctx->cur];
    a.W = ctx->W;
    a.row_begin = ctx->row_begin;
    a.row0 = ctx->row_begin;
    a.row1 = ctx->row_end;
    a.tiles_x = (ctx->W + 7) / 8;
    const uint32_t tiles_y = (a.row1 - a.row0 + 7) / 8;
    const size_t n_blocks = (size_t)a.tiles_x * ((ctx->row_end - ctx->row_begin + 7) / 8 + 1);
    if (!g->d_direct_counts) {
        void* p = nullptr;
        GI_HIP(ctx, hipMalloc(&p, 3 * n_blocks * sizeof(uint32_t)));
        GI_HIP(ctx, hipMemset(p, 0, 3 * n_blocks * sizeof(uint32_t)));
        g->allocs.push_back(p);
        g->d_direct_counts = (uint32_t*)p;
        g->n_block_counts = n_blocks;
    }
    a.bounce_counts = g->d_direct_counts;
    a.shadow_counts = g->d_direct_counts + g->n_block_counts;
    a.table_counts = g->d_direct_counts + 2 * g->n_block_counts;
    hipLaunchKernelGGL(pbr_direct_kernel, dim3(a.tiles_x * tiles_y), dim3(64), 0, (hipStream_t)stream, a);
    GI_HIP(ctx, hipGetLastError());
    return NEB_OK;
}

int neb_tonemap(neb_ctx* ctx, neb_stream stream)
{
    if (!ctx)
        return NEB_ERR_INVALID_ARG;
    if (int rc = neb::svgf_flush_pending(ctx))
        return rc;
    GI_GUARD(ctx);
    const size_t n = (size_t)ctx->W * (ctx->row_end - ctx->row_begin);
    hipLaunchKernelGGL(tonemap_kernel, dim3((unsigned)((n + 255) / 256)), dim3(256), 0, (hipStream_t)stream,
                       (const float4*)ctx->planes[NEB_PLANE_RADIANCE][ctx->cur], (uint32_t*)ctx->planes[NEB_PLANE_LDR][0], n);
    hipError_t e = hipGetLastError();
    if (e != hipSuccess)
        return gi_fail(ctx, NEB_ERR_HIP, "neb_tonemap", e);
    return NEB_OK;
}

int neb_gi_trace(neb_ctx* ctx, const neb_gi_constants* c, neb_stream stream)
{
    if (!ctx)
        return NEB_ERR_INVALID_ARG;
    return neb_gi_trace_rows(ctx, c, ctx->row_begin, ctx->row_end, stream);
}

int neb_gi_ray_count(neb_ctx* ctx, uint64_t* rays, int reset, neb_stream stream)
{
    if (!ctx || !ctx->gi)
        return ctx ? gi_fail(ctx, NEB_ERR_STATE, "neb_gi_ray_count: no scene") : NEB_ERR_INVALID_ARG;
    GiState* g = ctx->gi;
    GI_GUARD(ctx);
    unsigned long long v[16] = {};
    uint32_t* arrays[3] = {g->sets[0].d_block_counts, g->sets[1].d_block_counts, g->d_direct_counts};
    const size_t n3 = 3 * g->n_block_counts;
    std::vector<uint32_t> counts(3 * n3);
    GI_HIP(ctx, hipMemcpyAsync(v, g->d_ray_counter, sizeof(v), hipMemcpyDeviceToHost, (hipStream_t)stream));
    for (int q = 0; q < 3; ++q)
        if (arrays[q])
            GI_HIP(ctx, hipMemcpyAsync(counts.data() + q * n3, arrays[q], n3 * sizeof(uint32_t), hipMemcpyDeviceToHost, (hipStream_t)stream));
    GI_HIP(ctx, hipStreamSynchronize((hipStream_t)stream));
    if (reset) {
        GI_HIP(ctx, hipMemsetAsync(g->d_ray_counter, 0, sizeof(v), (hipStream_t)stream));
        for (int q = 0; q < 3; ++q)
            if (arrays[q])
                GI_HIP(ctx, hipMemsetAsync(arrays[q], 0, n3 * sizeof(uint32_t), (hipStream_t)stream));
    }
    unsigned long long total = 0, table = 0;
    for (int q = 0; q < 3; ++q) {
        for (size_t k = 0; k < 2 * g->n_block_counts; ++k)
            total += counts[q * n3 + k];
        for (size_t k = 2 * g->n_block_counts; k < n3; ++k)
            table += counts[q * n3 + k];
    }
    g->table_rays = table;
    v[0] = total;
    if (rays)
        *rays = total;
    memcpy(g->last_stats, v, sizeof(v));
    return NEB_OK;
}

int neb_gi_traversal_stats(neb_ctx* ctx, uint64_t out[5])
{
    if (!ctx || !ctx->gi || !out)
        return NEB_ERR_INVALID_ARG;
    for (int k = 0; k < 5; ++k)
        out[k] = ctx->gi->last_stats[k];
    return NEB_OK;
}

int neb_gi_wave_stats(neb_ctx* ctx, uint64_t out[6])
{
    if (!ctx || !ctx->gi || !out)
        return NEB_ERR_INVALID_ARG;
    for (int k = 0; k < 6; ++k)
        out[k] = ctx->gi->last_stats[5 + k];
    return NEB_OK;
}

int neb_gi_debug_set_tile_order(neb_ctx* ctx, const uint32_t* order, uint32_t n)
{
    if (!ctx || !ctx->gi)
        return NEB_ERR_INVALID_ARG;
    GiState* g = ctx->gi;
    GI_GUARD(ctx);
    GI_HIP(ctx, hipDeviceSynchronize());
    if (!order || n == 0) {
        g->tile_order_n = 0;
        return NEB_OK;
    }
    if (g->tile_order_cap < n) {
        void* p = nullptr;
        GI_HIP(ctx, hipMalloc(&p, (size_t)n * sizeof(uint32_t)));
        g->allocs.push_back(p);
        g->d_tile_order = (uint32_t*)p;
        g->tile_order_cap = n;
    }
    GI_HIP(ctx, hipMemcpy(g->d_tile_order, order, (size_t)n * sizeof(uint32_t), hipMemcpyHostToDevice));
    g->tile_order_n = n;
    return NEB_OK;
}

int neb_gi_debug_sun_walk_stats(neb_ctx* ctx, uint64_t out[12])
{
    if (!ctx || !ctx->gi || !out || !ctx->gi->d_sun_counts)
        return NEB_ERR_INVALID_ARG;
    GI_GUARD(ctx);
    GI_HIP(ctx, hipDeviceSynchronize());
    GI_HIP(ctx, hipMemcpy(out, ctx->gi->d_sun_counts + 8, 12 * sizeof(uint64_t), hipMemcpyDeviceToHost));
    return NEB_OK;
}

int neb_gi_node_index_stats(neb_ctx* ctx, uint64_t out[5])
{
    if (!ctx || !ctx->gi || !out)
        return NEB_ERR_INVALID_ARG;
    for (int k = 0; k < 5; ++k)
        out[k] = ctx->gi->last_stats[11 + k];
    return NEB_OK;
}

int neb_gi_sun_table_stats(neb_ctx* ctx, uint64_t out[4], neb_stream stream)
{
    if (!ctx || !ctx->gi || !out)
        return NEB_ERR_INVALID_ARG;
    GiState* g = ctx->gi;
    GI_GUARD(ctx);
    unsigned long long sides[2] = {0, 0};
    if (g->d_sun_counts && g->sun_table_state == 1) {
        GI_HIP(ctx, hipMemcpyAsync(sides, g->d_sun_counts, sizeof(sides), hipMemcpyDeviceToHost, (hipStream_t)stream));
        GI_HIP(ctx, hipStreamSynchronize((hipStream_t)stream));
    }
    out[0] = sides[0];
    out[1] = sides[1];
    out[2] = g->table_rays;
    out[3] = g->sun_table_builds;
    return NEB_OK;
}

int neb_gi_sun_table_build_ms(neb_ctx* ctx, float* ms)
{
    if (!ctx || !ctx->gi || !ms)
        return NEB_ERR_INVALID_ARG;
    GiState* g = ctx->gi;
    if (!g->sun_table_builds || !g->sun_build_ev[1])
        return gi_fail(ctx, NEB_ERR_STATE, "neb_gi_sun_table_build_ms: no table has been built");
    GI_GUARD(ctx);
    GI_HIP(ctx, hipEventSynchronize(g->sun_build_ev[1]));
    GI_HIP(ctx, hipEventElapsedTime(ms, g->sun_build_ev[0], g->sun_build_ev[1]));
    return NEB_OK;
}

int neb_gi_shadow_tail_mode(neb_ctx* ctx, int* mode, float us[2])
{
    if (!ctx || !ctx->gi || !mode)
        return NEB_ERR_INVALID_ARG;
    const GiState* g = ctx->gi;
    *mode = g->tail_phase != 0 ? -1 : (g->tail_sorted ? 1 : 0);
    if (us)
        us[0] = g->tail_us[0], us[1] = g->tail_us[1];
    return NEB_OK;
}

int neb_gi_download_hits(neb_ctx* ctx, neb_gi_hit* host, neb_stream stream)
{
    if (!ctx || !host)
        return NEB_ERR_INVALID_ARG;
    if (!ctx->gi || !ctx->gi->d_hits)
        return gi_fail(ctx, NEB_ERR_STATE, "neb_gi_download_hits: set option gi_debug_hits=1 and trace first");
    GI_GUARD(ctx);
    const size_t npx = (size_t)ctx->W * (ctx->row_end - ctx->row_begin);
    GI_HIP(ctx, hipMemcpyAsync(host, ctx->gi->d_hits, npx * sizeof(neb_gi_hit), hipMemcpyDeviceToHost, (hipStream_t)stream));
    GI_HIP(ctx, hipStreamSynchronize((hipStream_t)stream));
    return NEB_OK;
}

int neb_gbuffer_raycast(neb_ctx* ctx, const neb_camera* cam, neb_stream stream)
{
    if (!ctx || !cam)
        return NEB_ERR_INVALID_ARG;
    if (int rc = neb::svgf_flush_pending(ctx))
        return rc;
    GiState* g = ctx->gi;
    if (!g || !g->built)
        return gi_fail(ctx, NEB_ERR_STATE, "neb_gbuffer_raycast: scene/BVH not ready");
    GI_GUARD(ctx);
    ScopedRange range("Deferred G-Buffers (geometry)");
    GI_HIP(ctx, gi_scene_reader(g, (hipStream_t)stream));
    GbufArgs a;
    a.S = g->view;
    const CameraBasis b = camera_basis(*cam, ctx->W, ctx->H);
    memcpy(a.eye, b.eye, 12);
    memcpy(a.xaxis, b.xaxis, 12);
    memcpy(a.yaxis, b.yaxis, 12);
    memcpy(a.zaxis, b.zaxis, 12);
    a.tan_half = b.tan_half;
    a.aspect = b.aspect;
    a.m22 = b.m22;
    a.m32 = b.m32;
    a.albedo = (uint32_t*)ctx->planes[NEB_PLANE_ALBEDO][0];
    a.rough_metal = (uint32_t*)ctx->planes[NEB_PLANE_ROUGH_METAL][0];
    a.world_pos = (uint2*)ctx->planes[NEB_PLANE_WORLDPOS][0];
    a.normal = (uint2*)ctx->planes[NEB_PLANE_NORMAL][ctx->cur];
    a.depth = (uint32_t*)ctx->planes[NEB_PLANE_DEPTH][ctx->cur];
    a.W = ctx->W;
    a.H = ctx->H;
    a.row_begin = ctx->row_begin;
    a.row0 = ctx->row_begin;
    a.row1 = ctx->row_end;
    a.tiles_x = (ctx->W + 7) / 8;
    const uint32_t tiles_y = (a.row1 - a.row0 + 7) / 8;
    ctx->geom_lo = ctx->geom_hi = 0;
    ctx->cams[ctx->cur] = *cam;
    ctx->has_cam[ctx->cur] = true;
    a.submesh_id = ctx->motion ? (uint32_t*)ctx->planes[NEB_PLANE_SUBMESH_ID][ctx->cur] : nullptr;
    hipLaunchKernelGGL(gbuffer_kernel, dim3(a.tiles_x * tiles_y), dim3(64), 0, (hipStream_t)stream, a);
    GI_HIP(ctx, hipGetLastError());
    if (ctx->motion)
        return neb::gi_snapshot_transforms(ctx, ctx->cur, (hipStream_t)stream);
    return NEB_OK;
}

}

namespace neb {
void gi_motion_tables_free(neb_ctx* ctx)
{
    for (void* p : {(void*)ctx->xf_snap[0], (void*)ctx->xf_snap[1], (void*)ctx->motion_delta})
        if (p)
            (void)hipFree(p);
    ctx->xf_snap[0] = ctx->xf_snap[1] = nullptr;
    ctx->motion_delta = nullptr;
    ctx->motion_geoms = 0;
    ctx->has_snap[0] = ctx->has_snap[1] = false;
}

int gi_motion_tables_alloc(neb_ctx* ctx)
{
    gi_motion_tables_free(ctx);
    const GiState* g = ctx->gi;
    if (!g || !g->n_geoms || !g->d_xf)
        return NEB_OK;
    GI_GUARD(ctx);
    hipError_t e = hipSuccess;
    for (int s = 0; s < 2 && e == hipSuccess; ++s)
        e = hipMalloc(&ctx->xf_snap[s], (size_t)g->n_geoms * 64);
    if (e == hipSuccess)
        e = hipMalloc(&ctx->motion_delta, (size_t)g->n_geoms * kReprojDeltaFloat4 * sizeof(float4));
    if (e != hipSuccess) {
        gi_motion_tables_free(ctx);
        return gi_fail(ctx, NEB_ERR_HIP, "svgf_motion: transform tables", e);
    }
    ctx->motion_geoms = g->n_geoms;
    return NEB_OK;
}

int gi_snapshot_transforms(neb_ctx* ctx, int s, hipStream_t stream)
{
    GiState* g = ctx->gi;
    if (!g || !ctx->xf_snap[s] || ctx->motion_geoms != g->n_geoms) {
        ctx->has_snap[s] = false;
        return NEB_OK;
    }
    GI_GUARD(ctx);
    GI_HIP(ctx, gi_scene_reader(g, stream));
    GI_HIP(ctx, hipMemcpyAsync(ctx->xf_snap[s], g->d_xf, (size_t)g->n_geoms * 64, hipMemcpyDeviceToDevice, stream));
    ctx->has_snap[s] = true;
    ctx->snap_epoch[s] = g->epoch;
    return NEB_OK;
}

int gi_set_sort_rays(neb_ctx* ctx, int mask)
{
    if (!ctx->gi || mask < 0 || mask > 3)
        return NEB_ERR_STATE;
    ctx->gi->sort_shadow = (mask & 1) != 0;
    ctx->gi->sort_shadow_auto = false;
    ctx->gi->sort_bounce = (mask & 2) != 0;
    return NEB_OK;
}
int gi_set_max_bvh_depth(neb_ctx* ctx, int depth)
{
    if (!ctx->gi || depth < 1 || depth > (kLdsStack + kSpillStack) / 3)
        return NEB_ERR_STATE;
    ctx->gi->max_bvh_depth = (uint32_t)depth;
    return NEB_OK;
}
int gi_set_exact_shade(neb_ctx* ctx, int on)
{
    if (!ctx->gi)
        return NEB_ERR_STATE;
    ctx->gi->exact_shade = on != 0;
    return NEB_OK;
}
int gi_set_defer_resolve(neb_ctx* ctx, int on)
{
    if (!ctx->gi)
        return NEB_ERR_STATE;
    if (on < 0 || on > 2)
        return NEB_ERR_STATE;
    GiState* g = ctx->gi;
    if (g->defer_resolve == 2 && g->traces != g->resolves)
        return NEB_ERR_STATE;
    g->defer_resolve = on;
    g->traces = g->resolves = 0;
    return NEB_OK;
}
int gi_set_sun_table(neb_ctx* ctx, int on)
{
    if (!ctx->gi || on < 0 || on > 3)
        return NEB_ERR_STATE;
    GiState* g = ctx->gi;
    g->sun_table = on != 0;
    g->compact_shadow = on != 2;
    g->tail_tune = on == 1;
    g->tail_sorted = false;
    g->tail_phase = (g->tail_tune && g->sun_table_state == 1) ? 1 : 0;
    return NEB_OK;
}
int gi_set_sun_hold(neb_ctx* ctx, int n)
{
    if (!ctx->gi || n < 0 || n == 1 || n > 100000)
        return NEB_ERR_STATE;
    ctx->gi->sun_hold_option = n;
    ctx->gi->sun_hold = n > 0 ? (uint32_t)n : 2u;
    return NEB_OK;
}
int gi_set_sun_hints(neb_ctx* ctx, int n)
{
    if (!ctx->gi || (n != 0 && n != 2 && n != 4))
        return NEB_ERR_STATE;
    ctx->gi->sun_hints = n;
    return NEB_OK;
}
int gi_set_deform_stage(neb_ctx* ctx, int mode)
{
    if (!ctx->gi || (mode != 0 && mode != 1))
        return NEB_ERR_STATE;
    ctx->gi->deform_stage = mode;
    return NEB_OK;
}
int gi_set_debug_hits(neb_ctx* ctx, int on)
{
    if (!ctx->gi)
        return NEB_ERR_STATE;
    ctx->gi->debug_hits = on != 0;
    return NEB_OK;
}
}
```

### nebulae_amd/csrc/gi_build.hip

```cpp
#include <cstring>
#include <rocprim/device/device_radix_sort.hpp>
#include <rocprim/device/device_scan.hpp>

#include <algorithm>
#include <chrono>
#include <cstdlib>

#include "gi_device.h"

namespace neb {

void gi_on_resize(GiState* g)
{
    if (!g)
        return;
    std::vector<void*> stale = {g->d_hits, g->d_direct_counts};
    for (GiState::DispatchSet& ds : g->sets) {
        for (void* p : {(void*)ds.d_records, (void*)ds.d_block_counts, (void*)ds.d_sort, ds.d_sort_temp, (void*)ds.d_list})
            stale.push_back(p);
        ds = GiState::DispatchSet{};
    }
    g->traces = g->resolves = 0;
    g->begun = g->finished = 0;
    for (void* p : stale) {
// ... 990 lines not shown
        if (!(mn <= mx))
            mn = mx = 0.0f;
        {
            const float pad = fmaxf(fmaxf(fabsf(mn), fabsf(mx)), mx - mn) * 0x1p-20f;
            mn -= pad;
            mx += pad;
        }
        float sc = fmaxf((mx - mn) / 255.0f * (1.0f + 0x1p-21f), 1e-30f);
        for (int guard = 0; guard < 8 && fmaf(255.0f, sc, mn) < mx; ++guard)
            sc *= 1.0f + 0x1p-20f;
        org[ax] = mn;
        scl[ax] = sc;
        qlo[ax] = qhi[ax] = 0u;
        for (int q = 0; q < 4; ++q) {
            uint32_t l = 255u, h = 0u;
            if (lo[ax][q] <= hi[ax][q]) {
                l = (uint32_t)fminf(floorf((lo[ax][q] - mn) / sc), 255.0f);
                while (l > 0u && fmaf((float)l, sc, mn) >= lo[ax][q])
                    --l;
                h = (uint32_t)fminf(ceilf((hi[ax][q] - mn) / sc), 255.0f);
                while (h < 255u && fmaf((float)h, sc, mn) <= hi[ax][q])
                    ++h;
            }
            qlo[ax] |= l << (8 * q);
            qhi[ax] |= h << (8 * q);
        }
    }
    Bvh4NodeQ o;
    o.ox = org[0], o.oy = org[1], o.oz = org[2];
    o.sx = scl[0], o.sy = scl[1], o.sz = scl[2];
    o.qlox = qlo[0], o.qloy = qlo[1], o.qloz = qlo[2];
    o.qhix = qhi[0], o.qhiy = qhi[1], o.qhiz = qhi[2];
    o.child = nd.child;
    out[i] = o;
}

hipError_t gi_quantise_nodes(const Bvh4Node* nodes, uint32_t n, Bvh4NodeQ* out, hipStream_t stream)
{
    if (!n)
        return hipSuccess;
    hipLaunchKernelGGL(quantise_nodes_kernel, dim3((n + 127) / 128), dim3(128), 0, stream, nodes, n, out);
    return hipGetLastError();
}

void gi_rebake_host(GiState* g)
{
    for (uint32_t gi = 0; gi < (uint32_t)g->h_geoms.size(); ++gi) {
        GiState::HostGeom& hg = g->h_geoms[gi];
        if (!hg.dirty)
            continue;
        hg.dirty = false;
        for (uint32_t p = 0; p < hg.n_tris; ++p) {
            float w[3][3];
            for (int k = 0; k < 3; ++k)
                (void)gi_bake_point(hg.m, &g->h_pos[3 * (size_t)(hg.vertexBase + g->h_indices[hg.firstIndex + 3 * p + k])], w[k]);
            float* t = &g->h_tris[12 * (size_t)(hg.firstTri + p)];
            for (int q = 0; q < 3; ++q) {
                t[q] = w[0][q];
                t[3 + q] = w[1][q] - w[0][q];
                t[6 + q] = w[2][q] - w[0][q];
            }
        }
    }
}

}

using namespace neb;

extern "C" {

int neb_gi_set_scene(neb_ctx* ctx, const neb_geometry_desc* geoms, uint32_t n_geoms, const neb_material_desc* mats,
                     uint32_t n_mats, const neb_texture_desc* texs, uint32_t n_texs)
{
    if (!ctx)
        return NEB_ERR_INVALID_ARG;
    if ((n_geoms && !geoms) || (n_mats && !mats) || (n_texs && !texs))
        return gi_fail(ctx, NEB_ERR_INVALID_ARG, "neb_gi_set_scene: null table");
    GI_GUARD(ctx);
    GI_HIP(ctx, hipDeviceSynchronize());
    gi_motion_tables_free(ctx);
    gi_destroy(ctx->gi);
    ctx->gi = nullptr;
    GiState* g = new GiState();
    g->h_geoms.resize(n_geoms);
    g->h_seen.assign(n_geoms, 0u);
    g->n_geoms = n_geoms;
    std::vector<DevGeom> dgeoms(n_geoms);
    std::vector<DevMat> dmats(n_mats);
    std::vector<DevTex> dtexs(n_texs);
    std::vector<uint32_t>& indices = g->h_indices;
    std::vector<float> normals, uvs, tangents;
    uint32_t vertex_base = 0;
    float smin[3] = {3.4e38f, 3.4e38f, 3.4e38f}, smax[3] = {-3.4e38f, -3.4e38f, -3.4e38f};
    for (uint32_t gi = 0; gi < n_geoms; ++gi) {
        const neb_geometry_desc& s = geoms[gi];
        if (s.indices && s.indexStride != 2 && s.indexStride != 4) {
            delete g;
            return gi_fail(ctx, NEB_ERR_INVALID_ARG, "neb_gi_set_scene: indexStride must be 2 or 4");
        }
        DevGeom& d = dgeoms[gi];
        const float* m = s.surfaceToWorld;
        const float m3[9] = {m[0], m[1], m[2], m[4], m[5], m[6], m[8], m[9], m[10]};
        memcpy(d.m, m3, sizeof(m3));
        d.material = (s.materialIndex >= 0 && (uint32_t)s.materialIndex < n_mats) ? s.materialIndex : -1;
        d.firstIndex = (uint32_t)indices.size();
        d.vertexBase = vertex_base;
        d.valid = (s.indices && s.attributes[0] && s.attributes[1] && s.attributes[2] && s.attributes[3]) ? 1u : 0u;
        d.pad[0] = d.pad[1] = d.pad[2] = 0;
        GiState::HostGeom& hg = g->h_geoms[gi];
        memcpy(hg.m, m, sizeof(hg.m));
        hg.firstIndex = d.firstIndex;
        hg.vertexBase = vertex_base;
        hg.n_verts = s.numVertices;
        hg.valid = d.valid != 0;
        hg.firstTri = (uint32_t)(g->h_tris.size() / 12);
        hg.firstRef = (uint32_t)g->h_ref_verts.size();
        auto rd_index = [&](uint32_t i) -> uint32_t {
            const uint8_t* p = (const uint8_t*)s.indices + (size_t)i * s.indexStride;
            if (s.indexStride == 2) {
                uint16_t v;
                memcpy(&v, p, 2);
                return v;
            }
            uint32_t v;
            memcpy(&v, p, 4);
            return v;
        };
        auto rd_attr = [&](int a, uint32_t vtx, float* out, int n) {
            if (s.attributes[a])
                memcpy(out, (const uint8_t*)s.attributes[a] + (size_t)vtx * s.attributeStrides[a], sizeof(float) * n);
            else
                for (int k = 0; k < n; ++k)
                    out[k] = 0.f;
        };
        const uint32_t ntri = s.indices ? s.numIndices / 3 : 0;
        for (uint32_t i = 0; i < ntri * 3; ++i) {
            const uint32_t v = rd_index(i);
            if (v >= s.numVertices) {
                delete g;
                return gi_fail(ctx, NEB_ERR_OUT_OF_RANGE, "neb_gi_set_scene: index beyond numVertices");
            }
            indices.push_back(v);
        }
        for (uint32_t v = 0; v < s.numVertices; ++v) {
            float t[4];
            rd_attr(0, v, t, 3);
            g->h_pos.insert(g->h_pos.end(), t, t + 3);
            rd_attr(1, v, t, 3);
            normals.insert(normals.end(), t, t + 3);
            rd_attr(2, v, t, 2);
            uvs.insert(uvs.end(), t, t + 2);
            rd_attr(3, v, t, 4);
            tangents.insert(tangents.end(), t, t + 4);
        }
        vertex_base += s.numVertices;
        if (s.attributes[0]) {
            hg.n_tris = ntri;
            {
                std::vector<char> named(s.numVertices, 0);
                for (uint32_t i = 0; i < ntri * 3; ++i)
                    named[g->h_indices[hg.firstIndex + i]] = 1;
                for (int q = 0; q < 3; ++q)
                    hg.obj_lo[q] = 3.4e38f, hg.obj_hi[q] = -3.4e38f;
                for (uint32_t v = 0; v < s.numVertices; ++v)
                    if (named[v]) {
                        g->h_ref_verts.push_back(v);
                        for (int q = 0; q < 3; ++q) {
                            const float c = g->h_pos[3 * (size_t)(hg.vertexBase + v) + q];
                            hg.obj_lo[q] = fminf(hg.obj_lo[q], c);
                            hg.obj_hi[q] = fmaxf(hg.obj_hi[q], c);
                        }
                    }
                hg.n_refs = (uint32_t)g->h_ref_verts.size() - hg.firstRef;
                for (int q = 0; q < 3; ++q)
                    hg.world_lo[q] = 3.4e38f, hg.world_hi[q] = -3.4e38f;
            }
            for (uint32_t p = 0; p < ntri; ++p) {
                float w[3][3];
                for (int k = 0; k < 3; ++k) {
                    float a[3];
                    rd_attr(0, rd_index(3 * p + k), a, 3);
                    if (!gi_bake_point(m, a, w[k])) {
                        delete g;
                        return gi_fail(ctx, NEB_ERR_OUT_OF_RANGE, "neb_gi_set_scene: a vertex position (after the instance transform) is not a finite number");
                    }
                    for (int q = 0; q < 3; ++q) {
                        smin[q] = fminf(smin[q], w[k][q]);
                        smax[q] = fmaxf(smax[q], w[k][q]);
                        hg.world_lo[q] = fminf(hg.world_lo[q], w[k][q]);
                        hg.world_hi[q] = fmaxf(hg.world_hi[q], w[k][q]);
                    }
                }
                float t12[12] = {w[0][0], w[0][1], w[0][2], w[1][0] - w[0][0], w[1][1] - w[0][1], w[1][2] - w[0][2],
                                 w[2][0] - w[0][0], w[2][1] - w[0][1], w[2][2] - w[0][2], 0.f, 0.f, 0.f};
                memcpy(&t12[9], &gi, 4);
                memcpy(&t12[10], &p, 4);
                g->h_tris.insert(g->h_tris.end(), t12, t12 + 12);
            }
        }
    }
    for (uint32_t i = 0; i < n_mats; ++i) {
        DevMat& d = dmats[i];
        for (int k = 0; k < 3; ++k)
            d.tex[k] = (mats[i].textureIndices[k] >= 0 && (uint32_t)mats[i].textureIndices[k] < n_texs) ? mats[i].textureIndices[k] : -1;
        d.albedo[0] = mats[i].albedo[0];
        d.albedo[1] = mats[i].albedo[1];
        d.albedo[2] = mats[i].albedo[2];
        d.rough = mats[i].roughnessMetalness[0];
        d.metal = mats[i].roughnessMetalness[1];
    }
    std::vector<size_t> raw_off(n_texs);
    size_t raw_total = 0;
    for (uint32_t i = 0; i < n_texs; ++i) {
        if (!texs[i].rgba8 || !texs[i].width || !texs[i].height) {
            delete g;
            return gi_fail(ctx, NEB_ERR_INVALID_ARG, "neb_gi_set_scene: empty texture");
        }
        dtexs[i].offset = 0xffffffffu;
        dtexs[i].w = texs[i].width;
        dtexs[i].h = texs[i].height;
        dtexs[i].pad = 0;
        raw_off[i] = raw_total;
        raw_total += (size_t)texs[i].width * texs[i].height;
    }
    constexpr size_t kBundleBudget = (size_t)4 << 30;
    size_t bundle_entries = 0, table_entries = 0;
    std::vector<char> standalone(n_texs, 0);
    for (uint32_t i = 0; i < n_mats; ++i) {
        DevMat& d = dmats[i];
        d.bundle = d.bundle_w = d.bundle_h = d.pad = 0;
        bool bundled = false;
        if (d.tex[0] >= 0 && d.tex[1] >= 0 && d.tex[2] >= 0) {
            const DevTex &ta = dtexs[d.tex[0]], &tn = dtexs[d.tex[1]], &tr = dtexs[d.tex[2]];
            const size_t n_pos = (size_t)ta.w * ta.h;
            if (ta.w == tn.w && ta.w == tr.w && ta.h == tn.h && ta.h == tr.h && (bundle_entries + n_pos) * 32 <= kBundleBudget &&
                bundle_entries + n_pos <= 0xffffffffull) {
                d.bundle = (uint32_t)bundle_entries;
                d.bundle_w = ta.w;
                d.bundle_h = ta.h;
                bundle_entries += n_pos;
                bundled = true;
            }
        }
        if (!bundled)
            for (int k = 0; k < 3; ++k)
                if (d.tex[k] >= 0)
                    standalone[d.tex[k]] = 1;
    }
    for (uint32_t i = 0; i < n_texs; ++i)
        if (standalone[i]) {
            if (table_entries + (size_t)dtexs[i].w * dtexs[i].h > 0xfffffffeull) {
                delete g;
                return gi_fail(ctx, NEB_ERR_OUT_OF_RANGE, "neb_gi_set_scene: more than 2^32 texels in standalone texture tables");
            }
            dtexs[i].offset = (uint32_t)table_entries;
            table_entries += (size_t)dtexs[i].w * dtexs[i].h;
        }
    g->texture_table_bytes = table_entries * 16 + bundle_entries * 32;
    {
        uint32_t* d_raw = nullptr;
        uint4* d_tables = nullptr;
        uint4* d_bundles = nullptr;
        hipError_t te = hipSuccess;
        auto talloc = [&](void** p, size_t bytes, bool keep) {
            if (te != hipSuccess)
                return;
            te = hipMalloc(p, bytes ? bytes : 16);
            if (te == hipSuccess && keep)
                g->allocs.push_back(*p);
        };
        talloc((void**)&d_raw, raw_total * 4, false);
        talloc((void**)&d_tables, table_entries * 16, true);
        talloc((void**)&d_bundles, bundle_entries * 32, true);
        for (uint32_t i = 0; i < n_texs && te == hipSuccess; ++i)
            te = hipMemcpy(d_raw + raw_off[i], texs[i].rgba8, (size_t)texs[i].width * texs[i].height * 4, hipMemcpyHostToDevice);
        for (uint32_t i = 0; i < n_texs && te == hipSuccess; ++i)
            if (standalone[i]) {
                const size_t n_pos = (size_t)dtexs[i].w * dtexs[i].h;
                hipLaunchKernelGGL(texture_footprints_kernel, dim3((unsigned)((n_pos + 255) / 256)), dim3(256), 0, nullptr, d_raw + raw_off[i],
                                   dtexs[i].w, dtexs[i].h, d_tables + dtexs[i].offset, 1u);
                te = hipGetLastError();
            }
        for (uint32_t i = 0; i < n_mats && te == hipSuccess; ++i) {
            const DevMat& d = dmats[i];
            if (!d.bundle_w)
                continue;
            const size_t n_pos = (size_t)d.bundle_w * d.bundle_h;
            hipLaunchKernelGGL(material_bundle_kernel, dim3((unsigned)((n_pos + 255) / 256)), dim3(256), 0, nullptr, d_raw + raw_off[d.tex[0]],
                               d_raw + raw_off[d.tex[1]], d_raw + raw_off[d.tex[2]], d.bundle_w, d.bundle_h, d_bundles + 2 * (size_t)d.bundle);
            te = hipGetLastError();
        }
        if (te == hipSuccess)
            te = hipDeviceSynchronize();
        if (d_raw)
            (void)hipFree(d_raw);
        if (te != hipSuccess) {
            gi_destroy(g);
            return gi_fail(ctx, NEB_ERR_HIP, "neb_gi_set_scene: texture tables", te);
        }
        g->view.texels = reinterpret_cast<const uint32_t*>(d_tables);
        g->view.bundles = d_bundles;
    }
    std::vector<ShadeHeader> heads(n_geoms);
    for (uint32_t gi = 0; gi < n_geoms; ++gi) {
        ShadeHeader& hd = heads[gi];
        const DevGeom& d = dgeoms[gi];
        memset(&hd, 0, sizeof(hd));
        memcpy(hd.m, d.m, sizeof(hd.m));
        hd.valid = d.valid;
        hd.material = d.material;
        hd.tex[0] = hd.tex[1] = hd.tex[2] = -1;
        if (d.material >= 0) {
            const DevMat& mt = dmats[d.material];
            hd.bundle = mt.bundle, hd.bundle_w = mt.bundle_w, hd.bundle_h = mt.bundle_h;
            memcpy(hd.tex, mt.tex, sizeof(hd.tex));
            memcpy(hd.albedo, mt.albedo, sizeof(hd.albedo));
            hd.rough = mt.rough, hd.metal = mt.metal;
        }
    }
    g->n_tris = (uint32_t)(g->h_tris.size() / 12);
    memcpy(g->scene_min, smin, sizeof(smin));
    memcpy(g->scene_max, smax, sizeof(smax));
    hipError_t e = hipSuccess;
    if ((e = upload(g, dgeoms, &g->view.geoms)) != hipSuccess || (e = upload(g, dmats, &g->view.mats)) != hipSuccess ||
        (e = upload(g, dtexs, &g->view.texs)) != hipSuccess || (e = upload(g, indices, &g->view.indices)) != hipSuccess ||
        (e = upload(g, normals, &g->view.normals)) != hipSuccess || (e = upload(g, uvs, &g->view.uvs)) != hipSuccess ||
        (e = upload(g, tangents, &g->view.tangents)) != hipSuccess || (e = upload(g, heads, &g->shade_heads)) != hipSuccess ||
        (e = upload(g, g->h_pos, const_cast<const float**>(&g->d_pos))) != hipSuccess) {
        gi_destroy(g);
        return gi_fail(ctx, NEB_ERR_HIP, "neb_gi_set_scene: upload", e);
    }
    if (n_geoms) {
        std::vector<float> xf((size_t)n_geoms * 16);
        for (uint32_t gi = 0; gi < n_geoms; ++gi)
            memcpy(&xf[16 * (size_t)gi], g->h_geoms[gi].m, 64);
        const float* d_xf = nullptr;
        void* stamps = nullptr;
        void* stage = nullptr;
        if ((e = upload(g, xf, &d_xf)) != hipSuccess || (e = hipMalloc(&stamps, (size_t)n_geoms * 4)) != hipSuccess) {
            gi_destroy(g);
            return gi_fail(ctx, NEB_ERR_HIP, "neb_gi_set_scene: transform tables", e);
        }
        g->allocs.push_back(stamps);
        g->d_xf = const_cast<float*>(d_xf);
        g->d_geom_epoch = (uint32_t*)stamps;
        if ((e = hipMemset(stamps, 0, (size_t)n_geoms * 4)) != hipSuccess ||
            (e = hipHostMalloc(&stage, (size_t)GiState::kStageSlots * n_geoms * sizeof(GiState::StageEntry), hipHostMallocDefault)) != hipSuccess) {
            gi_destroy(g);
            return gi_fail(ctx, NEB_ERR_HIP, "neb_gi_set_scene: transform tables", e);
        }
        g->h_stage = (GiState::StageEntry*)stage;
    }
    void* ctr = nullptr;
    if ((e = hipMalloc(&ctr, 16 * sizeof(unsigned long long))) != hipSuccess || (e = hipMemset(ctr, 0, 16 * sizeof(unsigned long long))) != hipSuccess) {
        gi_destroy(g);
        return gi_fail(ctx, NEB_ERR_HIP, "neb_gi_set_scene: counter", e);
    }
    g->allocs.push_back(ctr);
    g->d_ray_counter = (unsigned long long*)ctr;
    g->view.n_tris = g->n_tris;
    ctx->gi = g;
    return ctx->motion ? gi_motion_tables_alloc(ctx) : NEB_OK;
}

#ifndef NEB_SPLIT_AREA_FACTOR
#define NEB_SPLIT_AREA_FACTOR 16.0
#endif
constexpr double kSplitAreaFactor = NEB_SPLIT_AREA_FACTOR, kSplitBudget = 0.25;

struct HostRef {
    uint32_t tri;
    float lo[3], hi[3];
    bool clipped;
};

static double half_area(const float lo[3], const float hi[3])
{
    const double dx = (double)hi[0] - lo[0], dy = (double)hi[1] - lo[1], dz = (double)hi[2] - lo[2];
    return dx * dy + dy * dz + dz * dx;
}

static bool clipped_bounds(const float* t, const float lo[3], const float hi[3], float out_lo[3], float out_hi[3])
{
    double poly[16][3], tmp[16][3];
    int n = 3;
    for (int c = 0; c < 3; ++c) {
        poly[0][c] = t[c];
        poly[1][c] = (double)t[c] + t[3 + c];
        poly[2][c] = (double)t[c] + t[6 + c];
    }
    for (int axis = 0; axis < 3 && n > 0; ++axis)
        for (int side = 0; side < 2 && n > 0; ++side) {
            const double plane = side == 0 ? (double)lo[axis] : (double)hi[axis], sgn = side == 0 ? 1.0 : -1.0;
            int m = 0;
            for (int i = 0; i < n; ++i) {
                const int j = (i + 1) % n;
                const double di = sgn * (poly[i][axis] - plane), dj = sgn * (poly[j][axis] - plane);
                if (di >= 0.0) {
                    for (int c = 0; c < 3; ++c)
                        tmp[m][c] = poly[i][c];
                    ++m;
                }
                if ((di >= 0.0) != (dj >= 0.0)) {
                    const double u = di / (di - dj);
                    for (int c = 0; c < 3; ++c)
                        tmp[m][c] = poly[i][c] + u * (poly[j][c] - poly[i][c]);
                    tmp[m][axis] = plane;
                    ++m;
                }
            }
            n = m;
            for (int i = 0; i < n; ++i)
                for (int c = 0; c < 3; ++c)
                    poly[i][c] = tmp[i][c];
        }
    if (n == 0)
        return false;
    for (int c = 0; c < 3; ++c) {
        double mn = poly[0][c], mx = poly[0][c];
        for (int i = 1; i < n; ++i) {
            mn = std::min(mn, poly[i][c]);
            mx = std::max(mx, poly[i][c]);
        }
        float fl = (float)mn, fh = (float)mx;
        if ((double)fl > mn)
            fl = std::nextafter(fl, -INFINITY);
        if ((double)fh < mx)
            fh = std::nextafter(fh, INFINITY);
        out_lo[c] = std::max(fl, lo[c]);
        out_hi[c] = std::min(fh, hi[c]);
        if (out_lo[c] > out_hi[c])
            out_lo[c] = out_hi[c] = 0.5f * (out_lo[c] + out_hi[c]);
    }
    return true;
}

static void split_references(const std::vector<float>& tris12, std::vector<HostRef>& refs)
{
    const uint32_t n = (uint32_t)(tris12.size() / 12);
    refs.resize(n);
    double sum_area = 0.0;
    for (uint32_t i = 0; i < n; ++i) {
        const float* t = &tris12[12 * (size_t)i];
        HostRef& r = refs[i];
        r.tri = i;
        r.clipped = false;
        for (int c = 0; c < 3; ++c) {
            const float v0 = t[c], v1 = t[c] + t[3 + c], v2 = t[c] + t[6 + c];
            r.lo[c] = std::min(v0, std::min(v1, v2));
            r.hi[c] = std::max(v0, std::max(v1, v2));
        }
        sum_area += half_area(r.lo, r.hi);
    }
    if (kSplitAreaFactor <= 0.0 || n < 8)
        return;
    const double limit = kSplitAreaFactor * sum_area / n;
    size_t budget = (size_t)(kSplitBudget * n);
    std::vector<std::pair<double, uint32_t>> heap;
    for (uint32_t i = 0; i < n; ++i) {
        const double a = half_area(refs[i].lo, refs[i].hi);
        if (a > limit)
            heap.emplace_back(a, i);
    }
    if (heap.empty())
        return;
    std::make_heap(heap.begin(), heap.end());
    std::vector<std::vector<HostRef>> pieces(n);
    std::vector<std::pair<uint32_t, uint32_t>> where;
    auto payload_ref = [&](uint32_t k) -> HostRef& { return k < n ? refs[k] : pieces[where[k - n].first][where[k - n].second]; };
    while (!heap.empty() && budget > 0) {
        std::pop_heap(heap.begin(), heap.end());
        const uint32_t k = heap.back().second;
        heap.pop_back();
        HostRef cur = payload_ref(k);
        int axis = 0;
        for (int c = 1; c < 3; ++c)
            if (cur.hi[c] - cur.lo[c] > cur.hi[axis] - cur.lo[axis])
                axis = c;
        const float mid = 0.5f * (cur.lo[axis] + cur.hi[axis]);
        if (!(mid > cur.lo[axis] && mid < cur.hi[axis]))
            continue;
        HostRef a = cur, b = cur;
        float alo[3], ahi[3], blo[3], bhi[3];
        for (int c = 0; c < 3; ++c)
            alo[c] = blo[c] = cur.lo[c], ahi[c] = bhi[c] = cur.hi[c];
        ahi[axis] = mid;
        blo[axis] = mid;
        const float* t = &tris12[12 * (size_t)cur.tri];
        const bool ha = clipped_bounds(t, alo, ahi, a.lo, a.hi), hb = clipped_bounds(t, blo, bhi, b.lo, b.hi);
        if (!ha || !hb)
            continue;
        a.clipped = b.clipped = true;
        std::vector<HostRef>& pc = pieces[cur.tri];
        uint32_t ia, ib;
        if (k < n) {
            pc.push_back(a);
            pc.push_back(b);
            ia = 0, ib = 1;
        } else {
            ia = where[k - n].second;
            pc[ia] = a;
            pc.push_back(b);
            ib = (uint32_t)pc.size() - 1u;
        }
        --budget;
        for (uint32_t which = 0; which < 2; ++which) {
            const HostRef& r = which == 0 ? a : b;
            const double area = half_area(r.lo, r.hi);
            if (area > limit) {
                uint32_t id;
                if (which == 0 && k >= n) {
                    id = k;
                } else {
                    where.emplace_back(cur.tri, which == 0 ? ia : ib);
                    id = n + (uint32_t)where.size() - 1u;
                }
                heap.emplace_back(area, id);
                std::push_heap(heap.begin(), heap.end());
            }
        }
    }
    std::vector<HostRef> out;
    out.reserve(n + (size_t)(kSplitBudget * n) + 8);
    for (uint32_t i = 0; i < n; ++i) {
        if (pieces[i].empty())
            out.push_back(refs[i]);
        else
            for (const HostRef& r : pieces[i])
                out.push_back(r);
    }
    refs.swap(out);
}

int neb_gi_build_bvh(neb_ctx* ctx, neb_stream stream_)
{
    if (!ctx)
        return NEB_ERR_INVALID_ARG;
    GiState* g = ctx->gi;
    if (!g)
        return gi_fail(ctx, NEB_ERR_STATE, "neb_gi_build_bvh: no scene (call neb_gi_set_scene first)");
    hipStream_t stream = (hipStream_t)stream_;
    GI_GUARD(ctx);
    const auto t_build0 = std::chrono::steady_clock::now();
    gi_rebake_host(g);
    if (g->n_tris == 0) {
        g->built = true;
        g->n_nodes = 0;
        g->bvh_depth = 0;
        g->view.root = -1;
        return NEB_OK;
    }
    std::vector<HostRef> refs;
    split_references(g->h_tris, refs);
    const uint32_t n = (uint32_t)refs.size();
    const bool have_pieces = n != g->n_tris;
    std::vector<float> h_refs;
    std::vector<float> h_boxes;
    if (have_pieces) {
        h_refs.resize((size_t)n * 12);
        h_boxes.resize((size_t)n * 8);
        for (uint32_t i = 0; i < n; ++i) {
            memcpy(&h_refs[12 * (size_t)i], &g->h_tris[12 * (size_t)refs[i].tri], 48);
            float* b = &h_boxes[8 * (size_t)i];
            b[0] = refs[i].lo[0], b[1] = refs[i].lo[1], b[2] = refs[i].lo[2], b[3] = refs[i].clipped ? 1.0f : 0.0f;
            b[4] = refs[i].hi[0], b[5] = refs[i].hi[1], b[6] = refs[i].hi[2], b[7] = 0.0f;
        }
    }
    std::vector<void*> temps, fresh;
    bool oom = false;
    auto dalloc = [&](size_t bytes, bool keep) -> void* {
        void* p = nullptr;
        if (oom || hipMalloc(&p, bytes ? bytes : 16) != hipSuccess) {
            oom = true;
            return nullptr;
        }
        (keep ? fresh : temps).push_back(p);
        return p;
    };
    auto release = [&](std::vector<void*>& v) {
        for (void* p : v)
            (void)hipFree(p);
        v.clear();
    };
    const size_t n2 = 2 * (size_t)n;
    float* d_tris12 = (float*)dalloc((size_t)n * 48, false);
    float4* d_sorted = (float4*)dalloc((size_t)n * 48, false);
    float4* d_boxes = have_pieces ? (float4*)dalloc((size_t)n * 32, false) : nullptr;
    float4* d_boxes_sorted = have_pieces ? (float4*)dalloc((size_t)n * 32, false) : nullptr;
    float4* d_final = (float4*)dalloc((size_t)n * 48, true);
    uint64_t* d_keys = (uint64_t*)dalloc((size_t)n * 8, false);
    uint64_t* d_keys2 = (uint64_t*)dalloc((size_t)n * 8, false);
    BinaryNodes N;
    N.lo = (float4*)dalloc(n2 * 16, false);
    N.hi = (float4*)dalloc(n2 * 16, false);
    N.size = (uint32_t*)dalloc(n2 * 4, false);
    uint32_t* d_idx[2] = {(uint32_t*)dalloc((size_t)n * 4, false), (uint32_t*)dalloc((size_t)n * 4, false)};
    SahSegment* d_segs[2] = {(SahSegment*)dalloc((size_t)n * sizeof(SahSegment), false), (SahSegment*)dalloc((size_t)n * sizeof(SahSegment), false)};
    SahSplit* d_splits = (SahSplit*)dalloc((size_t)n * sizeof(SahSplit), false);
    const uint32_t max_slices = n / kSahSlice + kSahBigMaxSegs + 1u;
    SahBig big;
    big.slice_begin = (uint32_t*)dalloc((kSahBigMaxSegs + 1u) * 4, false);
    big.cb = (uint32_t*)dalloc(kSahBigMaxSegs * 6 * 4, false);
    big.bins = (uint32_t*)dalloc((size_t)kSahBigMaxSegs * 4 * kSahBins * 7 * 4, false);
    big.slice_left = (uint32_t*)dalloc((size_t)max_slices * 4, false);
    SahBigPick* d_picks = (SahBigPick*)dalloc(kSahBigMaxSegs * sizeof(SahBigPick), false);
    unsigned long long* d_flags = (unsigned long long*)dalloc((size_t)n * 8, false);
    unsigned long long* d_scan = (unsigned long long*)dalloc((size_t)n * 8, false);
    uint32_t* d_state = (uint32_t*)dalloc(8 * 4, false);
    Bvh4Node* d_wide_tmp = (Bvh4Node*)dalloc((size_t)n * sizeof(Bvh4Node), false);
    uint32_t* d_qnode = (uint32_t*)dalloc((size_t)n * 4, false);
    uint32_t* d_qoff = (uint32_t*)dalloc((size_t)n * 4, false);
    int4* d_opened = (int4*)dalloc((size_t)n * 16, false);
    uint32_t* d_icount = (uint32_t*)dalloc((size_t)n * 4, false);
    uint32_t* d_iscan = (uint32_t*)dalloc((size_t)n * 4, false);
    float4* d_shade = (float4*)dalloc((size_t)n * 128, true);
    float4* d_plan = (float4*)dalloc(n2 * 16, false);
    size_t cub_bytes = 0, cub_b2 = 0, cub_b3 = 0;
    (void)rocprim::radix_sort_keys(nullptr, cub_bytes, d_keys, d_keys2, (size_t)n, 0u, 64u, stream);
    (void)rocprim::exclusive_scan(nullptr, cub_b2, d_flags, d_scan, 0ull, (size_t)n, rocprim::plus<unsigned long long>(), stream);
    (void)rocprim::exclusive_scan(nullptr, cub_b3, d_icount, d_iscan, 0u, (size_t)n, rocprim::plus<uint32_t>(), stream);
    cub_bytes = std::max(cub_bytes, std::max(cub_b2, cub_b3));
    void* d_cub = dalloc(cub_bytes, false);
    if (oom) {
        release(temps);
        release(fresh);
        return gi_fail(ctx, NEB_ERR_HIP, "neb_gi_build_bvh: out of device memory");
    }
    auto bail = [&](int code, const char* what, hipError_t e = hipSuccess) {
        (void)hipStreamSynchronize(stream);
        release(temps);
        release(fresh);
        return gi_fail(ctx, code, what, e);
    };
#define BUILD_HIP(call)                                   \
    do {                                                  \
        hipError_t e_ = (call);                           \
        if (e_ != hipSuccess)                             \
            return bail(NEB_ERR_HIP, #call, e_);          \
    } while (0)
    BUILD_HIP(hipMemcpyAsync(d_tris12, have_pieces ? h_refs.data() : g->h_tris.data(), (size_t)n * 48, hipMemcpyHostToDevice, stream));
    if (have_pieces)
        BUILD_HIP(hipMemcpyAsync(d_boxes, h_boxes.data(), (size_t)n * 32, hipMemcpyHostToDevice, stream));
    const float3 smin = make_float3(g->scene_min[0], g->scene_min[1], g->scene_min[2]);
    const float3 sinv = make_float3(1.0f / fmaxf(g->scene_max[0] - g->scene_min[0], 1e-20f), 1.0f / fmaxf(g->scene_max[1] - g->scene_min[1], 1e-20f),
                                    1.0f / fmaxf(g->scene_max[2] - g->scene_min[2], 1e-20f));
    const uint32_t nb = (n + 255) / 256;
    uint32_t index_bits = 1;
    while (index_bits < 32 && (1ull << index_bits) < (unsigned long long)n)
        ++index_bits;
    const uint32_t axis_bits = (64 - index_bits) / 3 < 21 ? (64 - index_bits) / 3 : 21;
    hipLaunchKernelGGL(lbvh_morton_kernel, dim3(nb), dim3(256), 0, stream, d_tris12, (const float4*)d_boxes, n, smin, sinv, axis_bits, index_bits, d_keys);
    BUILD_HIP(hipGetLastError());
    BUILD_HIP(rocprim::radix_sort_keys(d_cub, cub_bytes, d_keys, d_keys2, (size_t)n, 0u, 64u, stream));
    hipLaunchKernelGGL(lbvh_gather_kernel, dim3(nb), dim3(256), 0, stream, d_tris12, (const float4*)d_boxes, d_keys2, n, (1ull << index_bits) - 1ull, d_sorted,
                       d_boxes_sorted);
    BUILD_HIP(hipGetLastError());
    hipLaunchKernelGGL(sah_init_kernel, dim3(nb), dim3(256), 0, stream, (const float4*)d_sorted, (const float4*)d_boxes_sorted, n, N, d_idx[0]);
// ... 227 lines not shown
```

### nebulae_amd/csrc/gi_device.h

```cpp
#pragma once
#pragma clang fp contract(off)

#include "gi_internal.h"

namespace neb {

__device__ __forceinline__ float3 f3(float x, float y, float z) { return make_float3(x, y, z); }
__device__ __forceinline__ float3 operator+(float3 a, float3 b) { return f3(a.x + b.x, a.y + b.y, a.z + b.z); }
__device__ __forceinline__ float3 operator-(float3 a, float3 b) { return f3(a.x - b.x, a.y - b.y, a.z - b.z); }
__device__ __forceinline__ float3 operator*(float3 a, float s) { return f3(a.x * s, a.y * s, a.z * s); }
__device__ __forceinline__ float3 operator*(float3 a, float3 b) { return f3(a.x * b.x, a.y * b.y, a.z * b.z); }
__device__ __forceinline__ float3 operator-(float3 a) { return f3(-a.x, -a.y, -a.z); }
__device__ __forceinline__ float dot3(float3 a, float3 b) { return a.x * b.x + a.y * b.y + a.z * b.z; }
__device__ __forceinline__ float3 cross3(float3 a, float3 b)
{
    return f3(a.y * b.z - a.z * b.y, a.z * b.x - a.x * b.z, a.x * b.y - a.y * b.x);
}
template <bool FAST> __device__ __forceinline__ float fdiv(float a, float b) { return FAST ? a * __builtin_amdgcn_rcpf(b) : a / b; }
template <bool FAST> __device__ __forceinline__ float fsqrt(float x) { return FAST ? __builtin_amdgcn_sqrtf(x) : sqrtf(x); }
__device__ __forceinline__ void det_sincosf(float x, float& s, float& c)
{
    const float k = rintf(x * 0.636619772367581343f);
    float r = fmaf(-k, 1.57079637050628662109375f, x);
    r = fmaf(-k, -4.37113900018624283e-8f, r);
// ... 387 lines not shown
                        st.push(node);
                    node = ch.z;
                }
                if (k1 != kMiss) {
                    if (node != kTravDone)
                        st.push(node);
                    node = ch.y;
                }
                if (k0 != kMiss) {
                    if (node != kTravDone)
                        st.push(node);
                    node = ch.x;
                }
            }
            if (STATS)
                hit.deep_sp += st.depth() > 12;
            if (node == kTravDone && !st.empty())
                node = st.pop();
        }
        const bool holds_leaf = node < 0 && node != kTravDone;
        bool run_leaves = true;
        if (ANY_HIT && kLeafBatch > 1)
            run_leaves = __popcll(__ballot(holds_leaf)) >= kLeafBatch || __ballot(node >= 0) == 0ull;
        if (STATS) {
            const uint32_t nl = (uint32_t)__popcll(__ballot(holds_leaf && run_leaves));
            hit.w_leaf_iters += nl ? 1u : 0u;
            hit.w_leaf_lanes += nl;
        }
        if (holds_leaf && run_leaves) {
            const uint32_t code = (uint32_t)~node;
            const uint32_t first = code >> 2, count = (code & 3u) + 1u;
            if (STATS)
                hit.tri_tests += count;
            if constexpr (kMaxLeafTris <= 2) {
                const uint32_t second = first + count - 1u;
                float4 a0 = S.tris[3 * first];
                const float4 b0 = S.tris[3 * first + 1], c0 = S.tris[3 * first + 2];
                const float4 a1 = S.tris[3 * second], b1 = S.tris[3 * second + 1], c1 = S.tris[3 * second + 2];
                asm volatile("" : "+v"(a0.x), "+v"(a0.y), "+v"(a0.z));
                float t, u, v;
                if (intersect_tri_regs(a0, b0, c0, o, d, tmin, hit.t, t, u, v)) {
                    hit.t = t, hit.u = u, hit.v = v, hit.tri = first;
                    if constexpr (ANY_HIT)
                        found = true;
                }
                if (intersect_tri_regs(a1, b1, c1, o, d, tmin, hit.t, t, u, v)) {
                    hit.t = t, hit.u = u, hit.v = v, hit.tri = second;
                    if constexpr (ANY_HIT)
                        found = true;
                }
            } else {
                for (uint32_t k = 0; k < count; ++k) {
                    float t, u, v;
                    if (intersect_tri(S.tris, first + k, o, d, tmin, hit.t, t, u, v)) {
                        hit.t = t, hit.u = u, hit.v = v, hit.tri = first + k;
                        if constexpr (ANY_HIT)
                            found = true;
                    }
                }
            }
            if (ANY_HIT && found) {
                node = kTravDone;
                return;
            }
            node = st.empty() ? kTravDone : st.pop();
        }
    }
    if constexpr (!ANY_HIT)
        found = hit.tri != ~0u;
}

template <bool ANY_HIT, bool STATS, int N = kLdsStack, bool FAST = false>
__device__ bool traverse_t(const SceneView& S, float3 o, float3 d, float tmin, float tmax, int* lds_stack, Hit& hit, int* lds_array = nullptr,
                           int* child_slots = nullptr)
{
    hit.t = tmax;
    hit.tri = ~0u;
    hit.node_visits = hit.tri_tests = 0;
    hit.w_iters = hit.w_node_iters = hit.w_node_lanes = hit.w_leaf_iters = hit.w_leaf_lanes = 0;
    hit.top_visits[0] = hit.top_visits[1] = hit.top_visits[2] = hit.top_visits[3] = hit.deep_sp = 0;
    if (S.n_tris == 0)
        return false;
    bool found = false;
    int spill_mem[64 - N];
    const float dd = dot3(d, d), oo = dot3(o, o);
    const bool walkable = dd > 0.0f && dd < __builtin_inff() && oo < __builtin_inff();
    int node = walkable ? S.root : kTravDone;
    if constexpr (FAST) {
        TravStackA<N> st((LdsInt*)lds_stack, (LdsInt*)lds_array, spill_mem);
        traverse_core<ANY_HIT, STATS, !ANY_HIT>(S, o, d, tmin, st, node, hit, found, (LdsInt*)child_slots);
    } else {
        TravStackT<N> st{(LdsInt*)lds_stack, spill_mem, 0};
        traverse_core<ANY_HIT, STATS, false>(S, o, d, tmin, st, node, hit, found);
    }
    return found;
}

template <bool STATS>
__device__ __forceinline__ bool traverse_any_quad(const SceneView& S, float3 o, float3 d, float tmin, float tmax, int* stack, uint32_t& node_visits,
                                                  uint32_t& tri_tests)
{
    node_visits = tri_tests = 0;
    if (S.n_tris == 0)
        return false;
    const float dd = dot3(d, d), oo = dot3(o, o);
    if (!(dd > 0.0f && dd < __builtin_inff() && oo < __builtin_inff()))
        return false;
    const uint32_t lane = threadIdx.x & 63u, q = lane & 3u, qbase = lane & 60u;
    const float3 inv = f3(1.0f / d.x, 1.0f / d.y, 1.0f / d.z);
    const float3 oinv = f3(o.x * inv.x, o.y * inv.y, o.z * inv.z);
    const bool negx = d.x < 0.0f, negy = d.y < 0.0f, negz = d.z < 0.0f;
    constexpr uint32_t kMiss = 0xffffffffu;
    int node = S.root, sp = 0;
    bool found = false;
    auto push = [&](int v) {
        stack[16 * sp] = v;
        ++sp;
    };
    auto pop = [&]() -> int {
        --sp;
        return stack[16 * sp];
    };
    while (node != kTravDone) {
        if (node >= 0) {
            if (STATS)
                node_visits++;
            const char* nodes = reinterpret_cast<const char*>(S.qnodes);
            const uint32_t nb = (uint32_t)node << 6;
            const float4 p0 = *reinterpret_cast<const float4*>(nodes + nb);
            const float4 p1 = *reinterpret_cast<const float4*>(nodes + (nb + 16u));
            const uint4 p2 = *reinterpret_cast<const uint4*>(nodes + (nb + 32u));
            const int4 ch = *reinterpret_cast<const int4*>(nodes + (nb + 48u));
            const float sx = p0.w * inv.x, sy = p1.x * inv.y, sz = p1.y * inv.z;
            const float bx = fmaf(p0.x, inv.x, -oinv.x), by = fmaf(p0.y, inv.y, -oinv.y), bz = fmaf(p0.z, inv.z, -oinv.z);
            const uint32_t lox = __float_as_uint(p1.z), loy = __float_as_uint(p1.w);
            const uint32_t qnx = negx ? p2.y : lox, qfx = negx ? lox : p2.y;
            const uint32_t qny = negy ? p2.z : loy, qfy = negy ? loy : p2.z;
            const uint32_t qnz = negz ? p2.w : p2.x, qfz = negz ? p2.x : p2.w;
            auto un = [&](uint32_t w) { return (float)((w >> (8u * q)) & 0xffu); };
            const uint32_t key = slab_key_t(fmaf(un(qnx), sx, bx), fmaf(un(qny), sy, by), fmaf(un(qnz), sz, bz), fmaf(un(qfx), sx, bx),
                                            fmaf(un(qfy), sy, by), fmaf(un(qfz), sz, bz), tmin, tmax, q);
            const uint32_t m = (uint32_t)(__ballot(key != kMiss) >> qbase) & 0xfu;
            node = kTravDone;
            if (m & 8u)
                node = ch.w;
            if (m & 4u) {
                if (node != kTravDone)
                    push(node);
                node = ch.z;
            }
            if (m & 2u) {
                if (node != kTravDone)
                    push(node);
                node = ch.y;
            }
            if (m & 1u) {
                if (node != kTravDone)
                    push(node);
                node = ch.x;
            }
            if (node == kTravDone && sp)
                node = pop();
        }
        if (node < 0 && node != kTravDone) {
            const uint32_t code = (uint32_t)~node;
            const uint32_t first = code >> 2, count = (code & 3u) + 1u;
            if (STATS)
                tri_tests += count;
            const uint32_t ti = first + min(q, count - 1u);
            float t, u, v;
            const bool h = intersect_tri(S.tris, ti, o, d, tmin, tmax, t, u, v);
            if ((uint32_t)(__ballot(h) >> qbase) & 0xfu) {
                found = true;
                node = kTravDone;
            } else {
                node = sp ? pop() : kTravDone;
            }
        }
    }
    return found;
}

__device__ __forceinline__ bool traverse(const SceneView& S, float3 o, float3 d, float tmin, float tmax, bool any_hit, int* lds_stack,
                                         Hit& hit, bool stats = false)
{
    if (stats)
        return any_hit ? traverse_t<true, true>(S, o, d, tmin, tmax, lds_stack, hit) : traverse_t<false, true>(S, o, d, tmin, tmax, lds_stack, hit);
    return any_hit ? traverse_t<true, false>(S, o, d, tmin, tmax, lds_stack, hit) : traverse_t<false, false>(S, o, d, tmin, tmax, lds_stack, hit);
}

__device__ __forceinline__ void texel_position(uint32_t w, uint32_t h, float u, float v, int& x0, int& y0, float& fx, float& fy)
{
    const float x = u * (float)w - 0.5f, y = v * (float)h - 0.5f;
    const float fx0 = floorf(x), fy0 = floorf(y);
    fx = x - fx0;
    fy = y - fy0;
    const int W = (int)w, H = (int)h;
    x0 = (int)fx0 % W;
    y0 = (int)fy0 % H;
    if (x0 < 0)
        x0 += W;
    if (y0 < 0)
        y0 += H;
}
template <bool FAST = false> __device__ __forceinline__ float4 filter_footprint(uint4 fp, float fx, float fy)
{
    const uint32_t p00 = fp.x, p10 = fp.y, p01 = fp.z, p11 = fp.w;
    float r[4];
#pragma unroll
    for (int c = 0; c < 4; ++c) {
        auto un = [&](uint32_t p) { const float q = (float)((p >> (8 * c)) & 0xffu); return FAST ? q * (1.0f / 255.0f) : q / 255.0f; };
        const float a = un(p00), b = un(p10), cc = un(p01), dd = un(p11);
        const float top = a + fx * (b - a), bot = cc + fx * (dd - cc);
        r[c] = top + fy * (bot - top);
    }
    return make_float4(r[0], r[1], r[2], r[3]);
}
template <bool FAST = false> __device__ float4 sample_texture(const SceneView& S, int ti, float u, float v)
{
    const DevTex t = S.texs[ti];
    int x0, y0;
    float fx, fy;
    texel_position(t.w, t.h, u, v, x0, y0, fx, fy);
    const uint4 fp = reinterpret_cast<const uint4*>(S.texels)[(size_t)t.offset + (size_t)y0 * (int)t.w + x0];
    return filter_footprint<FAST>(fp, fx, fy);
}

struct MapSamples {
    float4 albedo = {0.f, 0.f, 0.f, 0.f}, normal = {0.f, 0.f, 0.f, 0.f}, rm = {0.f, 0.f, 0.f, 0.f};
};
template <bool FAST = false> __device__ __forceinline__ void sample_material_maps(const SceneView& S, const DevMat& m, float u, float v, MapSamples& out)
{
    if (m.bundle_w != 0) {
        int x0, y0;
        float fx, fy;
        texel_position(m.bundle_w, m.bundle_h, u, v, x0, y0, fx, fy);
        const uint4* e = S.bundles + 2 * ((size_t)m.bundle + (size_t)y0 * m.bundle_w + x0);
        const uint4 top = e[0], bot = e[1];
        float ch[8];
#pragma unroll
        for (int c = 0; c < 8; ++c) {
            auto un = [&](uint32_t lo, uint32_t hi) {
                const float q = (float)(((c < 4 ? lo : hi) >> (8 * (c & 3))) & 0xffu);
                return FAST ? q * (1.0f / 255.0f) : q / 255.0f;
            };
            const float a = un(top.x, top.y), b = un(top.z, top.w), cc = un(bot.x, bot.y), dd = un(bot.z, bot.w);
            const float tp = a + fx * (b - a), bt = cc + fx * (dd - cc);
            ch[c] = tp + fy * (bt - tp);
        }
        out.albedo = make_float4(ch[0], ch[1], ch[2], 0.0f);
        out.normal = make_float4(ch[3], ch[4], ch[5], 0.0f);
        out.rm = make_float4(0.0f, ch[6], ch[7], 0.0f);
        return;
    }
    if (m.tex[0] >= 0)
        out.albedo = sample_texture<FAST>(S, m.tex[0], u, v);
    if (m.tex[1] >= 0)
        out.normal = sample_texture<FAST>(S, m.tex[1], u, v);
    if (m.tex[2] >= 0)
        out.rm = sample_texture<FAST>(S, m.tex[2], u, v);
}

__device__ __forceinline__ float3 load3(const float* p, uint32_t i) { return f3(p[3 * i], p[3 * i + 1], p[3 * i + 2]); }
__device__ __forceinline__ float3 xform_dir(const float* m, float3 p)
{
    return f3(p.x * m[0] + p.y * m[3] + p.z * m[6], p.x * m[1] + p.y * m[4] + p.z * m[7], p.x * m[2] + p.y * m[5] + p.z * m[8]);
}

struct TriShade {
    float3 n0, n1, n2;
    float2 uv0, uv1, uv2;
    float4 t0, t1, t2;
    uint32_t geom;
    uint32_t lit;
    uint32_t hint[kHints], hint_side;
};
template <typename Ptr> __device__ __forceinline__ TriShade load_tri_shade_at(Ptr r, uint32_t swz)
{
    const float4 r0 = r[0 ^ swz], r1 = r[1 ^ swz], r2 = r[2 ^ swz], r6 = r[6 ^ swz];
    TriShade t;
    t.n0 = f3(r0.x, r0.y, r0.z);
    t.n1 = f3(r1.x, r1.y, r1.z);
    t.n2 = f3(r2.x, r2.y, r2.z);
    t.uv0 = make_float2(r0.w, r1.w);
    t.uv1 = make_float2(r2.w, r6.x);
    t.uv2 = make_float2(r6.y, r6.z);
    t.geom = __float_as_uint(r6.w) & kGeomMask;
    t.lit = __float_as_uint(r6.w) >> kLitShift;
    t.t0 = r[3 ^ swz];
    t.t1 = r[4 ^ swz];
    t.t2 = r[5 ^ swz];
    const float4 r7 = r[7 ^ swz];
    unpack_hints(r7, t.hint, t.hint_side);
    return t;
}
__device__ __forceinline__ TriShade load_tri_shade(const SceneView& S, uint32_t tri) { return load_tri_shade_at(S.shade + 8 * (size_t)tri, 0u); }

struct ShadeHead {
    float m[9];
    uint32_t valid;
    int32_t material;
    DevMat mat;
};
__device__ __forceinline__ ShadeHead load_shade_header(const ShadeHeader* heads, uint32_t geom)
{
    const float4* q = reinterpret_cast<const float4*>(heads + geom);
    const float4 q0 = q[0], q1 = q[1], q2 = q[2], q3 = q[3], q4 = q[4], q5 = q[5];
    ShadeHead h;
    h.m[0] = q0.x, h.m[1] = q0.y, h.m[2] = q0.z, h.m[3] = q0.w;
    h.m[4] = q1.x, h.m[5] = q1.y, h.m[6] = q1.z, h.m[7] = q1.w;
    h.m[8] = q2.x;
    h.valid = __float_as_uint(q2.y);
    h.material = (int32_t)__float_as_uint(q2.z);
    h.mat.bundle = __float_as_uint(q2.w);
    h.mat.bundle_w = __float_as_uint(q3.x);
    h.mat.bundle_h = __float_as_uint(q3.y);
    h.mat.tex[0] = (int32_t)__float_as_uint(q3.z);
    h.mat.tex[1] = (int32_t)__float_as_uint(q3.w);
    h.mat.tex[2] = (int32_t)__float_as_uint(q4.x);
    h.mat.albedo[0] = q4.y, h.mat.albedo[1] = q4.z, h.mat.albedo[2] = q4.w;
    h.mat.rough = q5.x, h.mat.metal = q5.y;
    h.mat.pad = 0;
    return h;
}

template <bool FAST = false> __device__ __forceinline__ bool reconstruct_surface(const SceneView& S, const ShadeHead& g, const TriShade& ts, float bu, float bv, Surface& out)
{
    const float b0 = 1.0f - (bu + bv), b1 = bu, b2 = bv;
    if (!g.valid)
        return false;
    const float3 n0 = ts.n0, n1 = ts.n1, n2 = ts.n2;
    const float3 gn = normalize3<FAST>(f3(n0.x * b0 + n1.x * b1 + n2.x * b2, n0.y * b0 + n1.y * b1 + n2.y * b2, n0.z * b0 + n1.z * b1 + n2.z * b2));
    out.GN = normalize3<FAST>(xform_dir(g.m, gn));
    const float u = ts.uv0.x * b0 + ts.uv1.x * b1 + ts.uv2.x * b2;
    const float v = ts.uv0.y * b0 + ts.uv1.y * b1 + ts.uv2.y * b2;
    if (g.material < 0)
        return false;
    const DevMat& m = g.mat;
    MapSamples maps;
    sample_material_maps<FAST>(S, m, u, v, maps);
    if (m.tex[0] < 0) {
        out.albedo = f3(m.albedo[0], m.albedo[1], m.albedo[2]);
    } else {
        const float4 t = maps.albedo;
        out.albedo = f3(t.x, t.y, t.z);
    }
    if (m.tex[1] < 0) {
        out.SN = out.GN;
    } else {
        float tg[4];
        tg[0] = ts.t0.x * b0 + ts.t1.x * b1 + ts.t2.x * b2;
        tg[1] = ts.t0.y * b0 + ts.t1.y * b1 + ts.t2.y * b2;
        tg[2] = ts.t0.z * b0 + ts.t1.z * b1 + ts.t2.z * b2;
        tg[3] = ts.t0.w * b0 + ts.t1.w * b1 + ts.t2.w * b2;
        const float l4 = fsqrt<FAST>(tg[0] * tg[0] + tg[1] * tg[1] + tg[2] * tg[2] + tg[3] * tg[3]);
#pragma unroll
        for (int k = 0; k < 4; ++k)
            tg[k] = fdiv<FAST>(tg[k], l4);
        const float3 T = f3(tg[0], tg[1], tg[2]);
        const float3 B = normalize3<FAST>(cross3(out.GN, T) * tg[3]);
        const float4 t = maps.normal;
        const float3 N = f3(t.x * 2.0f - 1.0f, t.y * 2.0f - 1.0f, t.z * 2.0f - 1.0f);
        out.SN = normalize3<FAST>(T * N.x + B * N.y + out.GN * N.z);
    }
    if (m.tex[2] < 0) {
        out.roughness = m.rough;
        out.metalness = m.metal;
    } else {
        const float4 t = maps.rm;
        out.roughness = t.y;
        out.metalness = t.z;
    }
    return true;
}

__device__ __forceinline__ uint32_t expand_bits10(uint32_t v)
{
    v = (v * 0x00010001u) & 0xFF0000FFu;
    v = (v * 0x00000101u) & 0x0F00F00Fu;
    v = (v * 0x00000011u) & 0xC30C30C3u;
    v = (v * 0x00000005u) & 0x49249249u;
    return v;
}

__device__ __forceinline__ uint32_t morton30(float3 p, const float* smin, const float* sinv)
{
    const uint32_t qx = (uint32_t)fminf(fmaxf((p.x - smin[0]) * sinv[0] * 1024.0f, 0.0f), 1023.0f);
    const uint32_t qy = (uint32_t)fminf(fmaxf((p.y - smin[1]) * sinv[1] * 1024.0f, 0.0f), 1023.0f);
    const uint32_t qz = (uint32_t)fminf(fmaxf((p.z - smin[2]) * sinv[2] * 1024.0f, 0.0f), 1023.0f);
    return (expand_bits10(qx) << 2) | (expand_bits10(qy) << 1) | expand_bits10(qz);
}

}
```

### nebulae_amd/csrc/gi_internal.h

```cpp
#pragma once
#include <cmath>
#include <cstdio>
#include <cstring>
#include <vector>

#include "neb_device.h"
#include "neb_internal.h"

namespace neb {


struct DevGeom {
    float m[9];
    int32_t material;
    uint32_t firstIndex;
    uint32_t vertexBase;
    uint32_t valid;
    uint32_t pad[3];
};
struct DevMat {
    int32_t tex[3];
    float albedo[3];
    float rough, metal;
    uint32_t bundle;
    uint32_t bundle_w, bundle_h;
    uint32_t pad;
};
struct alignas(128) ShadeHeader {
    float m[9];
    uint32_t valid;
    int32_t material;
    uint32_t bundle;
    uint32_t bundle_w, bundle_h;
    int32_t tex[3];
    float albedo[3];
    float rough, metal;
    uint32_t pad[10];
};
static_assert(sizeof(ShadeHeader) == 128 && offsetof(ShadeHeader, rough) == 80, "shade header layout (load_shade_header, gi_device.h)");
struct DevTex {
    uint32_t offset;
    uint32_t w, h, pad;
};
struct BvhNode {
    float c0min[3];
    int32_t c0;
    float c0max[3];
    int32_t c1;
    float c1min[3];
    uint32_t pad0;
    float c1max[3];
    uint32_t pad1;
};

struct Bvh4Node {
    float4 lox, loy, loz;
    int4 child;
    float4 hix, hiy, hiz;
    int4 pad;
};
static_assert(sizeof(Bvh4Node) == 128 && offsetof(Bvh4Node, hix) == offsetof(Bvh4Node, lox) + 64, "node layout");
struct Bvh4NodeQ {
    float ox, oy, oz, sx;
    float sy, sz;
    uint32_t qlox, qloy;
    uint32_t qloz, qhix, qhiy, qhiz;
    int4 child;
};
static_assert(sizeof(Bvh4NodeQ) == 64, "quantised node layout");
#ifndef NEB_TRACE_WAVES
#define NEB_TRACE_WAVES 8
#endif
#ifndef NEB_SHADE_WAVES
#define NEB_SHADE_WAVES 4
#endif
#ifndef NEB_LEAF_BATCH
#define NEB_LEAF_BATCH 12
#endif
constexpr int kLeafBatch = NEB_LEAF_BATCH;
#ifndef NEB_MAX_LEAF_TRIS
#define NEB_MAX_LEAF_TRIS 2
#endif
constexpr int kMaxLeafTris = NEB_MAX_LEAF_TRIS;
constexpr uint32_t kLitShift = 30u, kGeomMask = (1u << kLitShift) - 1u;
constexpr int kHints = 4;
constexpr uint32_t kNoHint = 0x7fffffu;
__host__ __device__ inline void pack_hints(const uint32_t hint[kHints], uint32_t side, float4& r7)
{
    uint32_t h[kHints];
    for (int k = 0; k < kHints; ++k)
        h[k] = hint[k] < kNoHint ? hint[k] : kNoHint;
    const unsigned long long lo = (unsigned long long)h[0] | ((unsigned long long)h[1] << 23) | ((unsigned long long)(h[2] & 0x3ffffu) << 46);
    union { uint32_t u; float f; } y, z, w;
    y.u = (uint32_t)lo;
    z.u = (uint32_t)(lo >> 32);
    w.u = (h[2] >> 18) | (h[3] << 5) | (side << 31);
    r7.y = y.f, r7.z = z.f, r7.w = w.f;
}
__host__ __device__ inline void unpack_hints(const float4& r7, uint32_t hint[kHints], uint32_t& side)
{
    union { float f; uint32_t u; } y, z, w;
    y.f = r7.y, z.f = r7.z, w.f = r7.w;
    const unsigned long long lo = (unsigned long long)y.u | ((unsigned long long)z.u << 32);
    hint[0] = (uint32_t)lo & kNoHint;
    hint[1] = (uint32_t)(lo >> 23) & kNoHint;
    hint[2] = ((uint32_t)(lo >> 46) | (w.u << 18)) & kNoHint;
    hint[3] = (w.u >> 5) & kNoHint;
    side = w.u >> 31;
}

struct SceneView {
    const float4* tris;
    const Bvh4Node* nodes;
    const Bvh4NodeQ* qnodes;
    const DevGeom* geoms;
    const DevMat* mats;
    const DevTex* texs;
    const uint32_t* indices;
    const float* normals;
    const float* uvs;
    const float* tangents;
    const uint32_t* texels;
    const uint4* bundles;
    const float4* shade;
    uint32_t n_tris;
    int32_t root;
    uint32_t n_qnodes;
};

struct GiState {
    SceneView view{};
    const ShadeHeader* shade_heads = nullptr;
    std::vector<void*> allocs;
    std::vector<float> h_tris;
    float scene_min[3] = {0, 0, 0}, scene_max[3] = {0, 0, 0};
    uint32_t n_tris = 0, n_nodes = 0, bvh_depth = 0, build_passes = 0;
    float build_ms = 0.f;
    size_t texture_table_bytes = 0;
    uint32_t max_bvh_depth = 21;
    bool built = false;
    unsigned long long* d_ray_counter = nullptr;
    neb_gi_hit* d_hits = nullptr;
    bool debug_hits = false;
    struct DispatchSet {
        float4* d_records = nullptr;
        uint32_t* d_sort = nullptr;
        void* d_sort_temp = nullptr;
        uint32_t* d_block_counts = nullptr;
        uint32_t* d_list = nullptr;
        uint32_t list_epoch = 0;
        uint32_t pending_spp = 1, pending_row0 = 0, pending_row1 = 0;
        bool awaiting_resolve = false;
        uint32_t resolve_seq = 0;
        neb_gi_constants split_c{};
        uint32_t split_row0 = 0, split_row1 = 0;
    } sets[2];
    uint32_t resolve_seq = 0;
    uint32_t* d_tile_order = nullptr;
    uint32_t tile_order_n = 0, tile_order_cap = 0;
    uint32_t traces = 0, resolves = 0;
    uint32_t begun = 0, finished = 0;
    uint32_t* d_direct_counts = nullptr;
    unsigned long long last_stats[16] = {};
    int defer_resolve = 0;
    bool exact_shade = false;
    bool sort_shadow = true;
    bool sort_shadow_auto = true;
    bool sort_bounce = false;
    size_t sort_temp_bytes = 0;
    size_t n_block_counts = 0;
    bool sun_table = true;
    int sun_table_state = 0;
    float sun_table_pending[4] = {0, 0, 0, 0};
    uint32_t sun_hold = 2, sun_seen = 0, sun_table_age = 0;
    int sun_hold_option = 0;
    float sun_table_key[4] = {0, 0, 0, 0};
    unsigned long long* d_sun_counts = nullptr;
    uint32_t* d_sun_hint_list = nullptr;
    uint32_t sun_hint_list_cap = 0;
    uint32_t sun_table_builds = 0;
    hipEvent_t sun_table_event = nullptr;
    hipEvent_t sun_build_ev[2] = {nullptr, nullptr};
    hipStream_t sun_table_stream = nullptr;
    bool sun_table_event_pending = false;
    hipStream_t last_dispatch_stream = nullptr;
    bool last_dispatch_stream_set = false;
    unsigned long long table_rays = 0;
    int sun_hints = 4;
    bool compact_shadow = true;
    bool tail_tune = true;
    int tail_phase = 0;
    bool tail_sorted = false;
    hipEvent_t tail_ev[4] = {nullptr, nullptr, nullptr, nullptr};
    float tail_us[2] = {0.f, 0.f};
    bool sun_table_stale = false;
    struct HostGeom {
        uint32_t firstIndex = 0, vertexBase = 0, n_tris = 0;
        uint32_t firstTri = 0;
        uint32_t firstRef = 0, n_refs = 0;
        uint32_t n_verts = 0;
        bool valid = false;
        float obj_lo[3] = {0, 0, 0}, obj_hi[3] = {0, 0, 0};
        float world_lo[3] = {0, 0, 0}, world_hi[3] = {0, 0, 0};
        float m[16] = {};
        bool dirty = false;
    };
    std::vector<HostGeom> h_geoms;
    std::vector<uint32_t> h_indices, h_ref_verts;
    std::vector<float> h_pos;
    std::vector<uint32_t> h_seen;
    uint32_t seen_stamp = 0;
    float* d_pos = nullptr;
    float* d_xf = nullptr;
    uint32_t* d_geom_epoch = nullptr;
    uint32_t* d_node_epoch = nullptr;
    uint32_t epoch = 0;
    std::vector<uint32_t> level_first;
    static constexpr int kStageSlots = 4;
    struct StageEntry { uint32_t geom, pad[3]; float m[16]; };
    StageEntry* h_stage = nullptr;
    hipEvent_t stage_ev[kStageSlots] = {nullptr, nullptr, nullptr, nullptr};
    bool stage_used[kStageSlots] = {false, false, false, false};
    struct DeformRange { uint32_t first_lane, count, dst, geom, pos_off, nrm_off, tan_off, pad; };
    static constexpr uint32_t kNoStream = 0xffffffffu;
    void* h_vstage = nullptr;
    size_t vstage_cap = 0;
    void* d_vstage = nullptr;
    size_t d_vstage_cap = 0;
    int deform_stage = 0;
    static constexpr int kReaderStreams = 4;
    hipStream_t reader_streams[kReaderStreams] = {nullptr, nullptr, nullptr, nullptr};
    hipEvent_t reader_ev[kReaderStreams] = {nullptr, nullptr, nullptr, nullptr};
    int n_reader_streams = 0;
    bool reader_overflow = false;
    uint32_t n_geoms = 0;
};
hipError_t gi_sun_table_update(GiState* g, const neb_gi_constants& c, hipStream_t stream);
hipError_t gi_sun_table_order(GiState* g, hipStream_t stream);
hipError_t mark_rewrite(GiState* g, hipStream_t stream);
hipError_t gi_quantise_nodes(const Bvh4Node* nodes, uint32_t n, Bvh4NodeQ* out, hipStream_t stream);
void gi_rebake_host(GiState* g);

inline hipError_t gi_scene_reader(GiState* g, hipStream_t stream)
{
    bool known = false;
    for (int k = 0; k < g->n_reader_streams; ++k)
        known = known || g->reader_streams[k] == stream;
    if (!known) {
        if (g->n_reader_streams < GiState::kReaderStreams)
            g->reader_streams[g->n_reader_streams++] = stream;
        else
            g->reader_overflow = true;
    }
    return gi_sun_table_order(g, stream);
}

inline bool gi_bake_point(const float* m, const float a[3], float w[3])
{
#pragma clang fp contract(off)
    w[0] = a[0] * m[0] + a[1] * m[4] + a[2] * m[8] + m[12];
    w[1] = a[0] * m[1] + a[1] * m[5] + a[2] * m[9] + m[13];
    w[2] = a[0] * m[2] + a[1] * m[6] + a[2] * m[10] + m[14];
    return fabsf(w[0]) <= 3.0e38f && fabsf(w[1]) <= 3.0e38f && fabsf(w[2]) <= 3.0e38f;
}

void gi_on_resize(GiState* g);
void gi_destroy(GiState* g);

}

static inline int gi_fail(neb_ctx* ctx, int code, const char* what, hipError_t e = hipSuccess)
{
    char buf[512];
    if (e != hipSuccess)
        snprintf(buf, sizeof(buf), "%s: %s (%s)", what, hipGetErrorName(e), hipGetErrorString(e));
    else
        snprintf(buf, sizeof(buf), "%s", what);
    ctx->last_error = buf;
    return code;
}

#define GI_HIP(ctx, call)                                   \
    do {                                                    \
        hipError_t e_ = (call);                             \
        if (e_ != hipSuccess)                               \
            return gi_fail((ctx), NEB_ERR_HIP, #call, e_);  \
    } while (0)

#define GI_GUARD(ctx)                                                        \
    neb::DeviceGuard gi_guard_((ctx)->device);                               \
    if (gi_guard_.err != hipSuccess)                                         \
    return gi_fail((ctx), NEB_ERR_HIP, "hipSetDevice", gi_guard_.err)

template <typename T>
static inline hipError_t upload(neb::GiState* g, const std::vector<T>& h, const T** out)
{
    *out = nullptr;
    if (h.empty())
        return hipSuccess;
    void* d = nullptr;
    hipError_t e = hipMalloc(&d, h.size() * sizeof(T));
    if (e != hipSuccess)
        return e;
    g->allocs.push_back(d);
    *out = (const T*)d;
    return hipMemcpy(d, h.data(), h.size() * sizeof(T), hipMemcpyHostToDevice);
}
```

### nebulae_amd/csrc/gi_sun_table.hip

```cpp
#include <cstdlib>
#include <type_traits>

#include "gi_device.h"
#include "lit_predicate.h"

namespace neb {

struct SunTableArgs {
    SceneView S;
    lit::Frame F;
    double scene_hmax;
    double box_pad;
    float4* shade;
    unsigned long long* counts;
    uint32_t* hint_list;
    unsigned long long* walk_stats;
};

__device__ inline void node_child_box(const Bvh4Node& nd, int q, double lo[3], double hi[3])
{
    const float l0[4] = {nd.lox.x, nd.lox.y, nd.lox.z, nd.lox.w}, l1[4] = {nd.loy.x, nd.loy.y, nd.loy.z, nd.loy.w},
                l2[4] = {nd.loz.x, nd.loz.y, nd.loz.z, nd.loz.w};
    const float h0[4] = {nd.hix.x, nd.hix.y, nd.hix.z, nd.hix.w}, h1[4] = {nd.hiy.x, nd.hiy.y, nd.hiy.z, nd.hiy.w},
                h2[4] = {nd.hiz.x, nd.hiz.y, nd.hiz.z, nd.hiz.w};
// ... 234 lines not shown
                    continue;
                if (ch[q] < 0) {
                    queue_leaf(ch[q]);
                } else if (node == kTravDone) {
                    node = ch[q];
                } else if (sp < 64) {
                    stack[sp++] = ch[q];
                } else {
                    alive = false;
                }
            }
            if (node == kTravDone && sp > 0)
                node = stack[--sp];
        }
        const bool wave_walks = __ballot(walking) != 0ull;
        if (__ballot(qn > (uint32_t)kSunQueue - 16u) != 0ull || !wave_walks) {
            test_queued();
            if (!wave_walks)
                break;
        }
    }
    return alive;
}

template <int PASS>
__global__ __launch_bounds__(64, PASS == 1 ? NEB_SUN_WAVES : 2) void sun_table_kernel(SunTableArgs a)
{
    static_assert(PASS == 1 || PASS == 2, "pass 1 = lit bits, pass 2 = hints");
    uint32_t ti = blockIdx.x * blockDim.x + threadIdx.x;
    bool mine = ti < a.S.n_tris;
    int primary = 0;
    if constexpr (PASS == 2) {
        mine = ti < (uint32_t)a.counts[3];
        if (mine) {
            const uint32_t entry = a.hint_list[ti];
            ti = entry & 0x7fffffffu;
            primary = (int)(entry >> 31);
        }
    }
    uint32_t flags = 0;
    bool hinted = false, listed = false;
    __shared__ SunWaveLds<PASS == 2> lds;
    uint32_t visits = 0, tested = 0;
    const unsigned long long clock0 = a.walk_stats ? wall_clock64() : 0ull;
    double v[3][3], gn[3][3];
    float4 r6 = {0.f, 0.f, 0.f, 0.f};
    uint32_t geom = 0;
    bool ok = false;
    if (mine) {
        const float4 t0 = a.S.tris[3 * ti], t1 = a.S.tris[3 * ti + 1], t2 = a.S.tris[3 * ti + 2];
        v[0][0] = t0.x, v[0][1] = t0.y, v[0][2] = t0.z;
        v[1][0] = (double)t0.x + t0.w, v[1][1] = (double)t0.y + t1.x, v[1][2] = (double)t0.z + t1.y;
        v[2][0] = (double)t0.x + t1.z, v[2][1] = (double)t0.y + t1.w, v[2][2] = (double)t0.z + t2.x;
        const float4* rec = a.S.shade + 8 * (size_t)ti;
        const float4 r0 = rec[0], r1 = rec[1], r2 = rec[2];
        r6 = rec[6];
        geom = __float_as_uint(r6.w) & kGeomMask;
        const DevGeom g = a.S.geoms[geom];
        ok = g.valid;
        if (ok) {
            const float n[3][3] = {{r0.x, r0.y, r0.z}, {r1.x, r1.y, r1.z}, {r2.x, r2.y, r2.z}};
#pragma unroll
            for (int i = 0; i < 3; ++i) {
                const double x = (double)n[i][0] * g.m[0] + (double)n[i][1] * g.m[3] + (double)n[i][2] * g.m[6];
                const double y = (double)n[i][0] * g.m[1] + (double)n[i][1] * g.m[4] + (double)n[i][2] * g.m[7];
                const double z = (double)n[i][0] * g.m[2] + (double)n[i][1] * g.m[5] + (double)n[i][2] * g.m[8];
                const double l = sqrt(x * x + y * y + z * z);
                ok = ok && l > 0.0 && l < 1e30;
                gn[i][0] = x / l, gn[i][1] = y / l, gn[i][2] = z / l;
            }
        }
    }
    if (!ok) {
#pragma unroll
        for (int i = 0; i < 3; ++i)
            v[i][0] = v[i][1] = v[i][2] = 0.0, gn[i][0] = gn[i][1] = 0.0, gn[i][2] = 1.0;
    }
    SunCands cands;
    cands.clear();
    uint32_t hint[kHints];
#pragma unroll
    for (int h = 0; h < kHints; ++h)
        hint[h] = kNoHint;
    if constexpr (PASS == 1) {
        bool valid0 = false, valid1 = false, alive0 = false, alive1 = false;
        double clo0 = 0.0, clo1 = 0.0;
#pragma unroll 1
        for (int sd = 0; sd < 2; ++sd) {
            lit::Receiver R;
            lit::make_receiver(a.F, v, gn, sd ? -1 : +1, R);
            const bool valid = ok && R.valid;
            bool alive = valid && !lit::may_occlude(a.F, R, R.t);
            alive = sun_walk_column<false>(a, R, alive, ti, cands, lds, visits, tested);
            if (sd == 0)
                valid0 = valid, alive0 = alive, clo0 = R.c_lo;
            else
                valid1 = valid, alive1 = alive, clo1 = R.c_lo;
        }
        primary = (valid0 && valid1) ? (clo1 > clo0 ? 1 : 0) : (valid1 ? 1 : 0);
        flags = (alive0 ? 1u : 0u) | (alive1 ? 2u : 0u);
        if (mine) {
            float4 w6 = r6;
            w6.w = __uint_as_float(geom | (flags << kLitShift));
            a.shade[8 * (size_t)ti + 6] = w6;
        }
        listed = mine && (primary ? (valid1 && !alive1) : (valid0 && !alive0));
    } else {
        lit::Receiver R;
        lit::make_receiver(a.F, v, gn, primary ? -1 : +1, R);
        const bool valid = ok && R.valid;
        sun_walk_column<true>(a, R, valid, ti, cands, lds, visits, tested);
        if (valid)
            cands.choose(hint);
    }
    if (mine) {
        float4 w7 = a.S.shade[8 * (size_t)ti + 7];
        pack_hints(hint, (uint32_t)primary, w7);
        a.shade[8 * (size_t)ti + 7] = w7;
        hinted = hint[0] != kNoHint;
    }
    const unsigned long long m0 = __ballot(PASS == 1 && (flags & 1u) != 0u), m1 = __ballot(PASS == 1 && (flags & 2u) != 0u), m2 = __ballot(hinted);
    if (a.walk_stats) {
        unsigned long long vs = visits, mx = visits, ts = tested;
#pragma unroll
        for (int off = 32; off > 0; off >>= 1) {
            vs += __shfl_down(vs, off);
            mx = max(mx, (unsigned long long)__shfl_down(mx, off));
            ts += __shfl_down(ts, off);
        }
        if ((threadIdx.x & 63u) == 0) {
            const unsigned long long dt = wall_clock64() - clock0;
            unsigned long long* w = a.walk_stats + 6 * (PASS - 1);
            atomicAdd(w + 0, vs);
            atomicMax(w + 1, mx);
            atomicAdd(w + 2, ts);
            atomicAdd(w + 3, dt);
            atomicMax(w + 4, dt);
            atomicAdd(w + 5, 1ull);
        }
    }
    const unsigned long long m3 = __ballot(listed);
    unsigned long long base = 0;
    if ((threadIdx.x & 63u) == 0) {
        if (m0)
            atomicAdd(a.counts + 0, (unsigned long long)__popcll(m0));
        if (m1)
            atomicAdd(a.counts + 1, (unsigned long long)__popcll(m1));
        if (m2)
            atomicAdd(a.counts + 2, (unsigned long long)__popcll(m2));
        if (m3)
            base = atomicAdd(a.counts + 3, (unsigned long long)__popcll(m3));
    }
    if (PASS == 1 && m3) {
        base = (unsigned long long)__shfl((int)(uint32_t)base, 0);
        if (listed)
            a.hint_list[(uint32_t)base + (uint32_t)__popcll(m3 & ((1ull << (threadIdx.x & 63u)) - 1ull))] = ti | ((uint32_t)primary << 31);
    }
}

__global__ void sun_table_clear_kernel(float4* shade, uint32_t n)
{
    const uint32_t ti = blockIdx.x * blockDim.x + threadIdx.x;
    if (ti < n) {
        float4* p = shade + 8 * (size_t)ti + 6;
        p->w = __uint_as_float(__float_as_uint(p->w) & kGeomMask);
        const uint32_t none[kHints] = {kNoHint, kNoHint, kNoHint, kNoHint};
        pack_hints(none, 0u, p[1]);
    }
}

hipError_t mark_rewrite(GiState* g, hipStream_t stream)
{
    if (!g->sun_table_event)
        if (hipError_t e = hipEventCreateWithFlags(&g->sun_table_event, hipEventDisableTiming); e != hipSuccess)
            return e;
    g->sun_table_stream = stream;
    g->sun_table_event_pending = true;
    return hipEventRecord(g->sun_table_event, stream);
}

hipError_t gi_sun_table_order(GiState* g, hipStream_t stream)
{
    if (!g->sun_table_event_pending || stream == g->sun_table_stream)
        return hipSuccess;
    const hipError_t q = hipEventQuery(g->sun_table_event);
    if (q == hipSuccess) {
        g->sun_table_event_pending = false;
        return hipSuccess;
    }
    (void)hipGetLastError();
    return hipStreamWaitEvent(stream, g->sun_table_event, 0);
}

hipError_t gi_sun_table_update(GiState* g, const neb_gi_constants& c, hipStream_t stream)
{
    if (!g->built || g->view.n_tris == 0 || !g->view.shade)
        return hipSuccess;
    const float key[4] = {c.sunLightDirection[0], c.sunLightDirection[1], c.sunLightDirection[2], c.sunTanHalfAngle};
    const bool want = g->sun_table;
    auto quiesce = [&]() { return (g->defer_resolve == 2 || (g->last_dispatch_stream_set && g->last_dispatch_stream != stream)) ? hipDeviceSynchronize() : hipSuccess; };
    if (!want) {
        if (g->sun_table_state != 0) {
            if (hipError_t e = quiesce(); e != hipSuccess)
                return e;
            hipLaunchKernelGGL(sun_table_clear_kernel, dim3((g->view.n_tris + 255) / 256), dim3(256), 0, stream, const_cast<float4*>(g->view.shade), g->view.n_tris);
            if (hipError_t em = mark_rewrite(g, stream); em != hipSuccess)
                return em;
            g->sun_table_state = 0;
            g->sun_table_stale = false;
        }
        return hipGetLastError();
    }
    if (g->sun_table_state != 0 && !g->sun_table_stale && !memcmp(key, g->sun_table_key, sizeof(key))) {
        g->sun_table_state = 1;
        g->sun_table_age++;
        return hipSuccess;
    }
    constexpr uint32_t kSunTableLife = 32u, kSunHoldAfterShortLife = 32u;
    if (g->sun_table_state != 0) {
        if (memcmp(key, g->sun_table_pending, sizeof(key)) || g->sun_table_state == 1) {
            memcpy(g->sun_table_pending, key, sizeof(key));
            g->sun_seen = 0;
            if (g->sun_table_state == 1)
                g->sun_hold = g->sun_hold_option > 0 ? (uint32_t)g->sun_hold_option : (g->sun_table_age < kSunTableLife ? kSunHoldAfterShortLife : 2u);
        }
        g->sun_table_state = 2;
        if (++g->sun_seen < g->sun_hold)
            return hipSuccess;
    }
    const float dd = key[0] * key[0] + key[1] * key[1] + key[2] * key[2];
    double scene_abs_max = 0.0;
    for (int k = 0; k < 3; ++k)
        scene_abs_max = fmax(scene_abs_max, fmax(fabs((double)g->scene_min[k]), fabs((double)g->scene_max[k])));
    const bool too_large = !lit::margin_usable(lit::margin_for(scene_abs_max));
    constexpr float kMaxSunTanHalfAngle = 0.03f;
    if (too_large || !(dd > 0.0f) || !(dd < 1e30f) || !(key[3] >= 0.0f) || !(key[3] <= kMaxSunTanHalfAngle)) {
        if (g->sun_table_state != 0) {
            if (hipError_t e = quiesce(); e != hipSuccess)
                return e;
            hipLaunchKernelGGL(sun_table_clear_kernel, dim3((g->view.n_tris + 255) / 256), dim3(256), 0, stream, const_cast<float4*>(g->view.shade), g->view.n_tris);
            if (hipError_t em = mark_rewrite(g, stream); em != hipSuccess)
                return em;
        }
        g->sun_table_state = 0;
        g->sun_table_stale = false;
        return hipGetLastError();
    }
    if (!g->d_sun_counts) {
        void* p = nullptr;
        hipError_t e = hipMalloc(&p, 24 * sizeof(unsigned long long));
        if (e != hipSuccess)
            return e;
        g->allocs.push_back(p);
        g->d_sun_counts = (unsigned long long*)p;
    }
    hipError_t e = quiesce();
    if (e != hipSuccess)
        return e;
    e = hipMemsetAsync(g->d_sun_counts, 0, 24 * sizeof(unsigned long long), stream);
    if (e != hipSuccess)
        return e;
    SunTableArgs a;
    a.S = g->view;
    lit::make_frame(key, key[3], scene_abs_max, a.F);
    a.box_pad = fmax(1e-5, 1.1920928955078125e-7 * scene_abs_max);
    double hmax = -1e300;
    for (int k = 0; k < 8; ++k) {
        const double p[3] = {(k & 1) ? g->scene_max[0] : g->scene_min[0], (k & 2) ? g->scene_max[1] : g->scene_min[1],
                             (k & 4) ? g->scene_max[2] : g->scene_min[2]};
        hmax = fmax(hmax, p[0] * a.F.L[0] + p[1] * a.F.L[1] + p[2] * a.F.L[2]);
    }
    a.scene_hmax = hmax + fmax(1e-3, a.F.margin);
    a.shade = const_cast<float4*>(g->view.shade);
    a.counts = g->d_sun_counts;
    a.walk_stats = getenv("NEB_SUN_WALK_STATS") ? g->d_sun_counts + 8 : nullptr;
    if (g->sun_hint_list_cap < g->view.n_tris) {
        void* p = nullptr;
        if (hipError_t em = hipMalloc(&p, (size_t)g->view.n_tris * sizeof(uint32_t)); em != hipSuccess)
            return em;
        g->allocs.push_back(p);
        g->d_sun_hint_list = (uint32_t*)p;
        g->sun_hint_list_cap = g->view.n_tris;
    }
    a.hint_list = g->d_sun_hint_list;
    for (hipEvent_t& ev : g->sun_build_ev)
        if (!ev)
            if (hipError_t em = hipEventCreate(&ev); em != hipSuccess)
                return em;
    if (hipError_t em = hipEventRecord(g->sun_build_ev[0], stream); em != hipSuccess)
        return em;
    hipLaunchKernelGGL(sun_table_kernel<1>, dim3((g->view.n_tris + 63) / 64), dim3(64), 0, stream, a);
    hipLaunchKernelGGL(sun_table_kernel<2>, dim3((g->view.n_tris + 63) / 64), dim3(64), 0, stream, a);
    if (hipError_t em = hipEventRecord(g->sun_build_ev[1], stream); em != hipSuccess)
        return em;
    if (hipError_t em = mark_rewrite(g, stream); em != hipSuccess)
        return em;
    memcpy(g->sun_table_key, key, sizeof(key));
    g->sun_table_state = 1;
    g->sun_table_stale = false;
    g->sun_table_age = 0;
    g->sun_seen = 0;
    g->sun_table_builds++;
    g->tail_phase = g->tail_tune ? 1 : 0;
    g->tail_sorted = false;
    return hipGetLastError();
}

}
```

### nebulae_amd/renderer.py

```python
import ctypes as C
from dataclasses import dataclass, field

import numpy as np

from . import _lib, scene as S
from .svgf import PLANE_RADIANCE, SLOT_CURRENT, NebError, SVGFDenoiser

HIT_DTYPE = np.dtype([("t", np.float32), ("geometry", np.uint32), ("primitive", np.uint32), ("flags", np.uint32)])


@dataclass
class SceneSunUI:
    rough_diameter: float = 0.58
    direction: tuple = (0.5, -1.0, -0.2)
    radiance: tuple = (20.0, 20.0, 20.0)


@dataclass
class GlobalIlluminationUI:
    sky_color: tuple = (8.0, 8.0, 8.0)
    gi_samples_per_pixel: int = 1
    max_path_vertices: int = 2
    throughput_threshold: float = 0.01


@dataclass
class RenderInfo:
    scene: object
    camera: S.CameraDesc
    frame_index: int
    stream: int = 0
    timestep: float = 0.0


class DeferredRenderer:
    def __init__(self):
        self.svgf = SVGFDenoiser()
        self.sun = SceneSunUI()
        self.gi_ui = GlobalIlluminationUI()
        self._scene = None
        self._eye = None
        self._sun_key = None
        self.dynamic_scene_this_frame = False
        self.reset_history = False
        self.denoise_while_moving = False
        self.temporal_reprojection = False
        self.motion_vectors = False
        self.info = None

    def init(self, width, height, atrous_levels=None, device=0, row_begin=0, row_end=0):
        self.svgf.init(width, height, atrous_levels=atrous_levels, device=device, row_begin=row_begin, row_end=row_end)
        if self.motion_vectors and not self.temporal_reprojection:
            self.svgf.destroy()
            raise NebError("DeferredRenderer.init: motion_vectors needs temporal_reprojection")
        if self.temporal_reprojection:
            self.svgf.set_option("svgf_reproject", 1)
        if self.motion_vectors:
            self.svgf.set_option("svgf_motion", 1)
        self.width, self.height = width, height
        return True

    @property
    def _lib(self):
        return self.svgf._lib

    @property
    def _ctx(self):
        return self.svgf._ctx

    def _check(self, rc, what):
        _lib.check(self._lib, self._ctx, rc, what)

    def init_pathtracer_scene(self, scene, stream=0):
        G, ng, M, nm, T, nt = scene.descs()
        self._scene = None
        self._check(self._lib.neb_gi_set_scene(self._ctx, G, ng, M, nm, T, nt), "neb_gi_set_scene")
        self._check(self._lib.neb_gi_build_bvh(self._ctx, C.c_void_p(stream)), "neb_gi_build_bvh")
        self._scene = scene

    def update_transforms(self, indices, matrices, stream=None):
        if self._scene is None:
            raise NebError("update_transforms: no scene (init_pathtracer_scene first)")
        idx = np.ascontiguousarray(np.asarray(indices, np.int64).reshape(-1))
        if idx.size and (idx.min() < 0 or idx.max() > 0xFFFFFFFF):
            raise NebError("update_transforms: geometry index out of range")
        idx = idx.astype(np.uint32)
        mats = np.ascontiguousarray(np.asarray(matrices, np.float32).reshape(-1, 4, 4))
        if mats.shape[0] != idx.size:
            raise NebError(f"update_transforms: {idx.size} indices but {mats.shape[0]} matrices")
        st = C.c_void_p((self.info.stream if self.info else 0) if stream is None else stream)
        rc = self._lib.neb_gi_update_transforms(self._ctx, idx.ctypes.data_as(C.POINTER(C.c_uint32)),
                                                mats.ctypes.data_as(C.POINTER(C.c_float)), idx.size, st)
        self._check(rc, "neb_gi_update_transforms")
        for k, gi in enumerate(idx):
            self._scene.geometries[int(gi)]["M"] = mats[k].copy()

    def update_vertices(self, index, positions, normals=None, tangents=None, first_vertex=0, stream=None):
        if self._scene is None:
            raise NebError("update_vertices: no scene (init_pathtracer_scene first)")
        index, first_vertex = int(index), int(first_vertex)
        if not 0 <= index < len(self._scene.geometries) or not 0 <= first_vertex <= 0xFFFFFFFF:
            raise NebError("update_vertices: geometry index or first vertex out of range")
        arrays = {"positions": np.ascontiguousarray(np.asarray(positions, np.float32).reshape(-1, 3))}
        n = arrays["positions"].shape[0]
        for key, a, width in (("normals", normals, 3), ("tangents", tangents, 4)):
            if a is not None:
                arrays[key] = np.ascontiguousarray(np.asarray(a, np.float32).reshape(-1, width))
                if arrays[key].shape[0] != n:
                    raise NebError(f"update_vertices: {n} positions but {arrays[key].shape[0]} {key}")
        u = _lib.VertexUpdate(geometry=index, firstVertex=first_vertex, numVertices=n)
        for key, width in (("positions", 3), ("normals", 3), ("tangents", 4)):
            if key in arrays:
                setattr(u, key, arrays[key].ctypes.data)
                setattr(u, key[:-1] + "Stride", 4 * width)
        st = C.c_void_p((self.info.stream if self.info else 0) if stream is None else stream)
        self._check(self._lib.neb_gi_update_vertices(self._ctx, C.byref(u), 1, st), "neb_gi_update_vertices")
        gm = self._scene.geometries[index]
        for key, a in arrays.items():
            full = np.array(gm[key], np.float32, copy=True)
            full[first_vertex:first_vertex + n] = a
            gm[key] = full

    def scene_info(self):
        t, n = C.c_uint32(), C.c_uint32()
        self._check(self._lib.neb_gi_scene_info(self._ctx, C.byref(t), C.byref(n)), "neb_gi_scene_info")
        return t.value, n.value

    def scene_bytes(self):
        v = (C.c_uint64 * 3)()
        self._check(self._lib.neb_gi_scene_bytes(self._ctx, v), "neb_gi_scene_bytes")
        return dict(zip(("texture_tables", "triangles", "bvh_nodes"), [int(x) for x in v]))

    def bvh_depth(self):
        d = C.c_uint32()
        self._check(self._lib.neb_gi_bvh_depth(self._ctx, C.byref(d)), "neb_gi_bvh_depth")
        return d.value

    def build_ms(self):
        d = C.c_float()
        self._check(self._lib.neb_gi_build_ms(self._ctx, C.byref(d)), "neb_gi_build_ms")
        return float(d.value)

    def build_passes(self):
        d = C.c_uint32()
        self._check(self._lib.neb_gi_build_passes(self._ctx, C.byref(d)), "neb_gi_build_passes")
        return d.value

    def begin_frame(self, info):
        self.info = info
        if info.scene is not None and info.scene is not self._scene:
            self.init_pathtracer_scene(info.scene, info.stream)
        self.svgf.begin_frame(info.frame_index)
        if self.temporal_reprojection:
            self.svgf.set_camera(SLOT_CURRENT, info.camera)
        eye = tuple(info.camera.eye)
        sun_key = (self.sun.rough_diameter, tuple(self.sun.direction), tuple(self.sun.radiance))
        moved = (eye != self._eye) or (self._sun_key is not None and sun_key != self._sun_key)
        self._sun_key = sun_key
        if moved:
            self._eye = eye
            self.dynamic_scene_this_frame = True
        elif self.dynamic_scene_this_frame:
            self.dynamic_scene_this_frame = False
            self.reset_history = not (self.denoise_while_moving or self.temporal_reprojection)

    def end_frame(self):
        self.svgf.end_frame()

    def global_constants(self):
        import math
        c = S.GIConstants()
        c.frameIndex = self.info.frame_index & 0xFFFFFFFF
        c.samplesPerPixel = int(self.gi_ui.gi_samples_per_pixel)
        c.maxPathVertices = int(self.gi_ui.max_path_vertices)
        c.cameraWorldPos[:] = tuple(self.info.camera.eye)
        c.skyColor[:] = self.gi_ui.sky_color
        c.sunLightDirection[:] = self.sun.direction
        c.sunLightRadiance[:] = self.sun.radiance
        c.sunTanHalfAngle = math.tan(math.radians(self.sun.rough_diameter * 0.5))
        c.throughputThreshold = self.gi_ui.throughput_threshold
        return c

    def submit_commands_gbuffer(self):
        self._check(self._lib.neb_gbuffer_raycast(self._ctx, C.byref(self.info.camera), C.c_void_p(self.info.stream)),
                    "neb_gbuffer_raycast")

    def submit_commands_pbr_lighting(self):
        c = self.global_constants()
        self._check(self._lib.neb_pbr_direct(self._ctx, C.byref(c), C.c_void_p(self.info.stream)), "neb_pbr_direct")

    def submit_commands_hdr_tonemapping(self):
        self._check(self._lib.neb_tonemap(self._ctx, C.c_void_p(self.info.stream)), "neb_tonemap")

    def submit_commands_gi_pathtrace(self, rows=None, stream=None):
        c = self.global_constants()
        st = C.c_void_p(self.info.stream if stream is None else stream)
        if rows is None:
            rc = self._lib.neb_gi_trace(self._ctx, C.byref(c), st)
        else:
            rc = self._lib.neb_gi_trace_rows(self._ctx, C.byref(c), rows[0], rows[1], st)
        self._check(rc, "neb_gi_trace")

    def submit_commands_gi_pathtrace_begin(self, rows=None, stream=None):
        c = self.global_constants()
        st = C.c_void_p(self.info.stream if stream is None else stream)
        r0, r1 = (self.svgf.row_begin, self.svgf.row_end) if rows is None else rows
        self._check(self._lib.neb_gi_trace_begin(self._ctx, C.byref(c), r0, r1, st), "neb_gi_trace_begin")

    def submit_commands_gi_pathtrace_finish(self, stream=None, after_shade_event=None):
        self._check(self._lib.neb_gi_trace_finish(self._ctx, C.c_void_p(self.info.stream if stream is None else stream),
                                                  C.c_void_p(after_shade_event or 0)), "neb_gi_trace_finish")

    def set_defer_resolve(self, on=True):
        self.svgf.set_option("gi_defer_resolve", int(on))

    def submit_commands_gi_resolve(self, stream=None):
        self._check(self._lib.neb_gi_resolve(self._ctx, C.c_void_p(self.info.stream if stream is None else stream)), "neb_gi_resolve")

    def submit_commands_svgf_denoising(self):
        if self.dynamic_scene_this_frame and not (self.denoise_while_moving or self.temporal_reprojection):
            return False
        self._lib.neb_marker_push(b"SVGF Denoising")
        try:
            if self.reset_history:
                self.reset_history = False
                self.svgf.reset_history(self.info.stream)
            self.svgf.submit_temporal_accumulation(self.info.stream)
            self.svgf.submit_atrous_compute_wavelet(self.info.stream)
        finally:
            self._lib.neb_marker_pop()
        return True

    def ray_count(self, reset=False):
        v = C.c_uint64()
        self._check(self._lib.neb_gi_ray_count(self._ctx, C.byref(v), int(reset), C.c_void_p(self.info.stream if self.info else 0)),
                    "neb_gi_ray_count")
        return v.value

    def traversal_stats(self):
        v = (C.c_uint64 * 5)()
        self._check(self._lib.neb_gi_traversal_stats(self._ctx, v), "neb_gi_traversal_stats")
        return dict(zip(("rays", "bounce_nodes", "bounce_tris", "shadow_nodes", "shadow_tris"), [int(x) for x in v]))

    def wave_stats(self):
        v = (C.c_uint64 * 6)()
        self._check(self._lib.neb_gi_wave_stats(self._ctx, v), "neb_gi_wave_stats")
        return dict(zip(("waves", "iterations", "node_iterations", "node_lanes", "leaf_iterations", "leaf_lanes"), [int(x) for x in v]))

    def node_index_stats(self):
        v = (C.c_uint64 * 5)()
        self._check(self._lib.neb_gi_node_index_stats(self._ctx, v), "neb_gi_node_index_stats")
        return dict(zip(("below_64", "below_256", "below_1024", "below_4096", "deep_stack_phases"), [int(x) for x in v]))

    def sun_table_stats(self):
        v = (C.c_uint64 * 4)()
        self._check(self._lib.neb_gi_sun_table_stats(self._ctx, v, C.c_void_p(self.info.stream if self.info else 0)), "neb_gi_sun_table_stats")
        return dict(zip(("lit_plus", "lit_minus", "rays_answered", "builds"), [int(x) for x in v]))

    def sun_table_build_ms(self):
        ms = C.c_float()
        if self._lib.neb_gi_sun_table_build_ms(self._ctx, C.byref(ms)) != 0:
            return None
        return float(ms.value)

    def shadow_tail_mode(self):
        mode, us = C.c_int(), (C.c_float * 2)()
        self._check(self._lib.neb_gi_shadow_tail_mode(self._ctx, C.byref(mode), us), "neb_gi_shadow_tail_mode")
        return int(mode.value), (float(us[0]), float(us[1]))

    def set_debug_hits(self, on=True):
        self.svgf.set_option("gi_debug_hits", int(on))

    def download_hits(self):
        rows = self.svgf.row_end - self.svgf.row_begin
        out = np.zeros((rows, self.width), HIT_DTYPE)
        self._check(self._lib.neb_gi_download_hits(self._ctx, out.ctypes.data_as(C.c_void_p),
                                                   C.c_void_p(self.info.stream if self.info else 0)), "neb_gi_download_hits")
        return out

    def destroy(self):
        self.svgf.destroy()
```

Before: 1688.

## Prefetch shade header via stashed geometry id and split material map fetch from filtering

The trace kernels now stash the hit triangle's geometry id in ray_o.w, so the shade kernel can issue the shade-header load before the LDS staging barrier instead of after the triangle record arrives. Material texel loads are split from bilinear filtering so they can be issued early and overlap other work. Tail-tuning buffers are now allocated ahead of time at arm time, which drops the warm-up frame where compaction was disabled. This costs extra registers to hold the header and fetched texels, a debug mismatch counter, and an extra global read of the triangle record in the trace path.

After: 1688. No clear change (-0.0%).

```diff
diff --git a/include/nebulae_hip.h b/include/nebulae_hip.h
--- a/include/nebulae_hip.h
+++ b/include/nebulae_hip.h
@@ -212,6 +212,7 @@
 int neb_gi_shadow_tail_mode(neb_ctx* ctx, int* mode, float us[2]);
 int neb_gi_wave_stats(neb_ctx* ctx, uint64_t out[6]);
 int neb_gi_node_index_stats(neb_ctx* ctx, uint64_t out[5]);
+int neb_gi_debug_shade_geom_mismatches(neb_ctx* ctx, uint64_t* out);
 int neb_gi_debug_set_tile_order(neb_ctx* ctx, const uint32_t* order, uint32_t n);
 int neb_gi_debug_sun_walk_stats(neb_ctx* ctx, uint64_t out[12]);
 int neb_gi_download_hits(neb_ctx* ctx, neb_gi_hit* host, neb_stream stream);
diff --git a/nebulae_amd/_lib.py b/nebulae_amd/_lib.py
--- a/nebulae_amd/_lib.py
+++ b/nebulae_amd/_lib.py
@@ -114,6 +114,7 @@
         "neb_gi_traversal_stats": (C.c_int, [C.c_void_p, C.POINTER(C.c_uint64)]),
         "neb_gi_wave_stats": (C.c_int, [C.c_void_p, C.POINTER(C.c_uint64)]),
         "neb_gi_node_index_stats": (C.c_int, [C.c_void_p, C.POINTER(C.c_uint64)]),
+        "neb_gi_debug_shade_geom_mismatches": (C.c_int, [C.c_void_p, C.POINTER(C.c_uint64)]),
         "neb_gi_debug_set_tile_order": (C.c_int, [C.c_void_p, C.c_void_p, C.c_uint32]),
         "neb_gi_debug_sun_walk_stats": (C.c_int, [C.c_void_p, C.POINTER(C.c_uint64)]),
         "neb_gi_sun_table_build_ms": (C.c_int, [C.c_void_p, C.POINTER(C.c_float)]),
diff --git a/nebulae_amd/csrc/gi.hip b/nebulae_amd/csrc/gi.hip
--- a/nebulae_amd/csrc/gi.hip
+++ b/nebulae_amd/csrc/gi.hip
@@ -157,11 +157,11 @@
         const float3 org = worldPos + SN * 1e-2f;
         const bool bounce = a.c.maxPathVertices > 1;
         a.R.path[i] = make_float4(throughput.x, throughput.y, throughput.z, __uint_as_float(rng));
-        a.R.ray_o[i] = make_float4(org.x, org.y, org.z, 0.01f);
         a.R.ray_d[i] = make_float4(dir.x, dir.y, dir.z, bounce ? 1.0f : 0.0f);
         if (a.sample + 1 < a.c.samplesPerPixel)
             a.R.state[i] = make_float4(V.x, V.y, V.z, __uint_as_float(rng));
         float4 h = make_float4(bounce ? -1.0f : -2.0f, 0.f, 0.f, 0.f);
+        float ro_w = 0.01f;
         rays = bounce ? 1u : 0u;
         wave_stamp[0] = wave_stamp[1] = wave_stamp[2] = wave_stamp[3] = wave_stamp[4] = 0u;
         if (a.bsort_keys) {
@@ -172,8 +172,10 @@
             Hit hit;
             const bool found = a.stats ? traverse_t<false, true, kRgStack, true>(a.S, org, dir, 0.01f, kTraceMax, stack_mem + lane, hit, stack_mem, child_slot_mem + 4u * lane)
                                        : traverse_t<false, false, kRgStack, true>(a.S, org, dir, 0.01f, kTraceMax, stack_mem + lane, hit, stack_mem, child_slot_mem + 4u * lane);
-            if (found)
+            if (found) {
                 h = make_float4(hit.t, hit.u, hit.v, __uint_as_float(hit.tri));
+                ro_w = a.S.tris[3 * hit.tri + 2].y;
+            }
             if (a.stats) {
                 wave_stamp[0] = hit.w_iters, wave_stamp[1] = hit.w_node_iters, wave_stamp[2] = hit.w_node_lanes, wave_stamp[3] = hit.w_leaf_iters,
                 wave_stamp[4] = hit.w_leaf_lanes;
@@ -187,6 +189,7 @@
             }
         }
         a.R.hit[i] = h;
+        a.R.ray_o[i] = make_float4(org.x, org.y, org.z, ro_w);
     }
     count_rays(a.bounce_counts, rays);
     if (a.stats) {
@@ -226,8 +229,10 @@
             Hit hit;
             rays = 1;
             float4 h = make_float4(-1.0f, 0.f, 0.f, 0.f);
-            if (traverse(a.S, f3(ro.x, ro.y, ro.z), f3(rd.x, rd.y, rd.z), ro.w, kTraceMax, false, stack_mem + threadIdx.x, hit))
+            if (traverse(a.S, f3(ro.x, ro.y, ro.z), f3(rd.x, rd.y, rd.z), ro.w, kTraceMax, false, stack_mem + threadIdx.x, hit)) {
                 h = make_float4(hit.t, hit.u, hit.v, __uint_as_float(hit.tri));
+                a.R.ray_o[i].w = a.S.tris[3 * hit.tri + 2].y;
+            }
             a.R.hit[i] = h;
         }
     }
@@ -242,8 +247,8 @@
 };
 
 template <bool FAST>
-__device__ __forceinline__ void shade_pixel(const GiArgs& a, size_t i, const float4 h, const float4 pth, const float4 rd, const float4 ro, ShadeOut& o,
-                                            const float4* staged, uint32_t staged_swz)
+__device__ __forceinline__ void shade_pixel(const GiArgs& a, size_t i, const float4 h, const float4 pth, const float4 rd, const float4 ro, const ShadeHeadRaw& head_raw,
+                                            ShadeOut& o, const float4* staged, uint32_t staged_swz)
 {
     const uint32_t trav_iters = a.stats ? __float_as_uint(a.R.srec[4 * i + kSrContrib].w) : 0u;
     float3 throughput = f3(pth.x, pth.y, pth.z);
@@ -260,7 +265,9 @@
         const uint32_t tri = __float_as_uint(h.w);
         Surface surf;
         const TriShade ts = load_tri_shade_at(staged, staged_swz);
-        const ShadeHead head = load_shade_header(a.heads, ts.geom);
+        const ShadeHead head = unpack_shade_header(head_raw);
+        if (a.stats && ts.geom != __float_as_uint(ro.w))
+            atomicAdd(a.ray_counter + kGeomMismatchSlot, 1ull);
         const bool hint_fetch = a.sun_table && a.hint_pairs && !((ts.lit >> ts.hint_side) & 1u) && ts.hint[0] != kNoHint;
         float4 ha0 = make_float4(0.f, 0.f, 0.f, 0.f), hb0 = ha0, hc0 = ha0, ha1 = ha0, hb1 = ha0, hc1 = ha0;
         if (hint_fetch) {
@@ -268,7 +275,9 @@
             ha0 = a.S.tris[3 * h0], hb0 = a.S.tris[3 * h0 + 1], hc0 = a.S.tris[3 * h0 + 2];
             ha1 = a.S.tris[3 * h1], hb1 = a.S.tris[3 * h1 + 1], hc1 = a.S.tris[3 * h1 + 2];
         }
-        const bool shaded = reconstruct_surface<FAST>(a.S, head, ts, h.y, h.z, surf);
+        MapFetch maps;
+        fetch_material_maps(a.S, head, ts, h.y, h.z, maps);
+        const bool shaded = reconstruct_surface<FAST>(head, ts, h.y, h.z, maps, surf);
         dbg.t = h.x;
         dbg.geometry = ts.geom;
         if (a.hits)
@@ -304,8 +313,10 @@
                         continue;
                     }
                     const uint32_t h1 = ts.hint[pair + 1] != kNoHint ? ts.hint[pair + 1] : h0;
-                    const float4 a0 = a.S.tris[3 * h0], b0 = a.S.tris[3 * h0 + 1], c0 = a.S.tris[3 * h0 + 2];
+                    float4 a0 = a.S.tris[3 * h0];
+                    const float4 b0 = a.S.tris[3 * h0 + 1], c0 = a.S.tris[3 * h0 + 2];
                     const float4 a1 = a.S.tris[3 * h1], b1 = a.S.tris[3 * h1 + 1], c1 = a.S.tris[3 * h1 + 2];
+                    asm volatile("" : "+v"(a0.x), "+v"(a0.y), "+v"(a0.z));
                     hinted_hit = intersect_tri_regs(a0, b0, c0, so, inc, 0.001f, kTraceMax, tt, uu, vv) ||
                                  intersect_tri_regs(a1, b1, c1, so, inc, 0.001f, kTraceMax, tt, uu, vv);
                 }
@@ -389,6 +400,8 @@
     const uint32_t lane = threadIdx.x;
     const bool has_hit = active && h.x >= 0.0f;
     const uint32_t my_tri = has_hit ? __float_as_uint(h.w) : ~0u;
+    ShadeHeadRaw head;
+    load_shade_header(a.heads, has_hit && rd.w != 0.0f ? __float_as_uint(ro.w) : 0u, head);
 #pragma unroll
     for (uint32_t it = 0; it < 8; ++it) {
         const uint32_t src = it * 8u + (lane >> 3);
@@ -400,7 +413,7 @@
     }
     __syncthreads();
     if (active)
-        shade_pixel<FAST>(a, i, h, pth, rd, ro, o, smem + lane * 8u, lane & 7u);
+        shade_pixel<FAST>(a, i, h, pth, rd, ro, head, o, smem + lane * 8u, lane & 7u);
     if (a.list) {
         const bool trace = active && o.shadow_d.w != 0.0f;
         if (active && !trace) {
@@ -782,6 +795,35 @@
 
 extern "C" {
 
+static int gi_tail_buffers(neb_ctx* ctx, GiState* g, size_t npx, bool sorted_pass)
+{
+    const uint32_t wg_per_list = (uint32_t)(((size_t)((ctx->W + 7) / 8) * ((ctx->row_end - ctx->row_begin + 7) / 8 + 1) + kListSegments - 1) / kListSegments);
+    const size_t list_bytes = (size_t)kListSegments * wg_per_list * 64u * 64u + 4096u;
+    for (GiState::DispatchSet& ds : g->sets) {
+        if (!ds.d_list) {
+            void* p = nullptr;
+            GI_HIP(ctx, hipMalloc(&p, list_bytes));
+            g->allocs.push_back(p);
+            ds.d_list = (uint32_t*)p;
+            GI_HIP(ctx, hipMemset(p, 0, list_bytes));
+        }
+        if (sorted_pass && !ds.d_sort) {
+            void* p = nullptr;
+            GI_HIP(ctx, hipMalloc(&p, 8 * npx * sizeof(uint32_t)));
+            g->allocs.push_back(p);
+            ds.d_sort = (uint32_t*)p;
+            GI_HIP(ctx, hipMemset(p, 0, 8 * npx * sizeof(uint32_t)));
+            const size_t bytes = ray_sort_scratch_bytes(npx);
+            GI_HIP(ctx, hipMalloc(&p, bytes));
+            g->allocs.push_back(p);
+            ds.d_sort_temp = p;
+            g->sort_temp_bytes = bytes;
+            GI_HIP(ctx, hipMemset(p, 0, bytes));
+        }
+    }
+    return NEB_OK;
+}
+
 static int gi_dispatch(neb_ctx* ctx, const neb_gi_constants* c, uint32_t row0, uint32_t row1, neb_stream stream, int phase, hipEvent_t after_shade)
 {
     if (!ctx || !c)
@@ -875,12 +917,16 @@
         g->last_dispatch_stream = (hipStream_t)stream;
         g->last_dispatch_stream_set = true;
     }
+    if (g->tail_arm && phase != 1) {
+        g->tail_arm = false;
+        if (int rc = gi_tail_buffers(ctx, g, npx, g->sort_shadow_auto ? a.n_px >= 1500000u : g->sort_shadow))
+            return rc;
+    }
     a.heads = g->shade_heads;
     sun_frame(c->sunLightDirection, a.sun_L, a.sun_B, a.sun_T);
     a.sun_table = g->sun_table_state == 1 ? 1u : 0u;
     a.hint_pairs = (uint32_t)g->sun_hints / 2u;
     int tail_slot = -1;
-    bool tail_warm = false;
     if (a.sun_table && g->compact_shadow && g->tail_tune && phase != 1) {
         if (g->tail_phase == 3 && hipEventQuery(g->tail_ev[1]) == hipSuccess && hipEventQuery(g->tail_ev[3]) == hipSuccess) {
             float ms_lists = 0.f, ms_sorted = 0.f;
@@ -889,9 +935,6 @@
                 g->tail_sorted = ms_sorted < 0.95f * ms_lists;
             }
             g->tail_phase = 0;
-        } else if (g->tail_phase == 1 && !ds.d_list) {
-        } else if (g->tail_phase == 2 && !ds.d_sort && (g->sort_shadow_auto ? a.n_px >= 1500000u : g->sort_shadow)) {
-            tail_warm = true;
         } else if (g->tail_phase == 1 || g->tail_phase == 2) {
             tail_slot = g->tail_phase == 1 ? 0 : 2;
             for (int k = 0; k < 2; ++k)
@@ -901,7 +944,7 @@
         }
         (void)hipGetLastError();
     }
-    const bool compact = a.sun_table && g->compact_shadow && !tail_warm && (tail_slot >= 0 ? tail_slot == 0 : !g->tail_sorted);
+    const bool compact = a.sun_table && g->compact_shadow && (tail_slot >= 0 ? tail_slot == 0 : !g->tail_sorted);
     const bool sort_shadow = !compact && (g->sort_shadow_auto ? a.n_px >= 1500000u : g->sort_shadow);
     if (sort_shadow || g->sort_bounce) {
         if (!ds.d_sort) {
@@ -1156,7 +1199,7 @@
         return ctx ? gi_fail(ctx, NEB_ERR_STATE, "neb_gi_ray_count: no scene") : NEB_ERR_INVALID_ARG;
     GiState* g = ctx->gi;
     GI_GUARD(ctx);
-    unsigned long long v[16] = {};
+    unsigned long long v[kRayCounters] = {};
     uint32_t* arrays[3] = {g->sets[0].d_block_counts, g->sets[1].d_block_counts, g->d_direct_counts};
     const size_t n3 = 3 * g->n_block_counts;
     std::vector<uint32_t> counts(3 * n3);
@@ -1234,6 +1277,14 @@
     GI_GUARD(ctx);
     GI_HIP(ctx, hipDeviceSynchronize());
     GI_HIP(ctx, hipMemcpy(out, ctx->gi->d_sun_counts + 8, 12 * sizeof(uint64_t), hipMemcpyDeviceToHost));
+    return NEB_OK;
+}
+
+int neb_gi_debug_shade_geom_mismatches(neb_ctx* ctx, uint64_t* out)
+{
+    if (!ctx || !ctx->gi || !out)
+        return NEB_ERR_INVALID_ARG;
+    *out = ctx->gi->last_stats[kGeomMismatchSlot];
     return NEB_OK;
 }
 
@@ -1442,6 +1493,7 @@
     g->tail_tune = on == 1;
     g->tail_sorted = false;
     g->tail_phase = (g->tail_tune && g->sun_table_state == 1) ? 1 : 0;
+    g->tail_arm = g->tail_phase == 1;
     return NEB_OK;
 }
 int gi_set_sun_hold(neb_ctx* ctx, int n)
diff --git a/nebulae_amd/csrc/gi_build.hip b/nebulae_amd/csrc/gi_build.hip
--- a/nebulae_amd/csrc/gi_build.hip
+++ b/nebulae_amd/csrc/gi_build.hip
@@ -1316,7 +1316,8 @@
         g->view.texels = reinterpret_cast<const uint32_t*>(d_tables);
         g->view.bundles = d_bundles;
     }
-    std::vector<ShadeHeader> heads(n_geoms);
+    std::vector<ShadeHeader> heads(n_geoms ? n_geoms : 1u);
+    memset(heads.data(), 0, heads.size() * sizeof(ShadeHeader));
     for (uint32_t gi = 0; gi < n_geoms; ++gi) {
         ShadeHeader& hd = heads[gi];
         const DevGeom& d = dgeoms[gi];
@@ -1367,7 +1368,7 @@
         g->h_stage = (GiState::StageEntry*)stage;
     }
     void* ctr = nullptr;
-    if ((e = hipMalloc(&ctr, 16 * sizeof(unsigned long long))) != hipSuccess || (e = hipMemset(ctr, 0, 16 * sizeof(unsigned long long))) != hipSuccess) {
+    if ((e = hipMalloc(&ctr, kRayCounters * sizeof(unsigned long long))) != hipSuccess || (e = hipMemset(ctr, 0, kRayCounters * sizeof(unsigned long long))) != hipSuccess) {
         gi_destroy(g);
         return gi_fail(ctx, NEB_ERR_HIP, "neb_gi_set_scene: counter", e);
     }
diff --git a/nebulae_amd/csrc/gi_device.h b/nebulae_amd/csrc/gi_device.h
--- a/nebulae_amd/csrc/gi_device.h
+++ b/nebulae_amd/csrc/gi_device.h
@@ -713,10 +713,17 @@
     int32_t material;
     DevMat mat;
 };
-__device__ __forceinline__ ShadeHead load_shade_header(const ShadeHeader* heads, uint32_t geom)
+struct ShadeHeadRaw {
+    float4 q0, q1, q2, q3, q4, q5;
+};
+__device__ __forceinline__ void load_shade_header(const ShadeHeader* heads, uint32_t geom, ShadeHeadRaw& r)
 {
     const float4* q = reinterpret_cast<const float4*>(heads + geom);
-    const float4 q0 = q[0], q1 = q[1], q2 = q[2], q3 = q[3], q4 = q[4], q5 = q[5];
+    r.q0 = q[0], r.q1 = q[1], r.q2 = q[2], r.q3 = q[3], r.q4 = q[4], r.q5 = q[5];
+}
+__device__ __forceinline__ ShadeHead unpack_shade_header(const ShadeHeadRaw& r)
+{
+    const float4 q0 = r.q0, q1 = r.q1, q2 = r.q2, q3 = r.q3, q4 = r.q4, q5 = r.q5;
     ShadeHead h;
     h.m[0] = q0.x, h.m[1] = q0.y, h.m[2] = q0.z, h.m[3] = q0.w;
     h.m[4] = q1.x, h.m[5] = q1.y, h.m[6] = q1.z, h.m[7] = q1.w;
@@ -735,7 +742,70 @@
     return h;
 }
 
-template <bool FAST = false> __device__ __forceinline__ bool reconstruct_surface(const SceneView& S, const ShadeHead& g, const TriShade& ts, float bu, float bv, Surface& out)
+struct MapFetch {
+    uint4 q0 = {0u, 0u, 0u, 0u}, q1 = {0u, 0u, 0u, 0u}, q2 = {0u, 0u, 0u, 0u};
+    float fx0 = 0.f, fy0 = 0.f, fx1 = 0.f, fy1 = 0.f, fx2 = 0.f, fy2 = 0.f;
+};
+__device__ __forceinline__ void fetch_footprint(const SceneView& S, int ti, float u, float v, uint4& q, float& fx, float& fy)
+{
+    const DevTex t = S.texs[ti];
+    int x0, y0;
+    texel_position(t.w, t.h, u, v, x0, y0, fx, fy);
+    q = reinterpret_cast<const uint4*>(S.texels)[(size_t)t.offset + (size_t)y0 * (int)t.w + x0];
+}
+__device__ __forceinline__ void fetch_material_maps(const SceneView& S, const ShadeHead& g, const TriShade& ts, float bu, float bv, MapFetch& f)
+{
+    if (!g.valid || g.material < 0)
+        return;
+    const float b0 = 1.0f - (bu + bv), b1 = bu, b2 = bv;
+    const float u = ts.uv0.x * b0 + ts.uv1.x * b1 + ts.uv2.x * b2;
+    const float v = ts.uv0.y * b0 + ts.uv1.y * b1 + ts.uv2.y * b2;
+    const DevMat& m = g.mat;
+    if (m.bundle_w != 0) {
+        int x0, y0;
+        texel_position(m.bundle_w, m.bundle_h, u, v, x0, y0, f.fx0, f.fy0);
+        const uint4* e = S.bundles + 2 * ((size_t)m.bundle + (size_t)y0 * m.bundle_w + x0);
+        f.q0 = e[0], f.q1 = e[1];
+        return;
+    }
+    if (m.tex[0] >= 0)
+        fetch_footprint(S, m.tex[0], u, v, f.q0, f.fx0, f.fy0);
+    if (m.tex[1] >= 0)
+        fetch_footprint(S, m.tex[1], u, v, f.q1, f.fx1, f.fy1);
+    if (m.tex[2] >= 0)
+        fetch_footprint(S, m.tex[2], u, v, f.q2, f.fx2, f.fy2);
+}
+template <bool FAST = false> __device__ __forceinline__ void filter_material_maps(const DevMat& m, const MapFetch& f, MapSamples& out)
+{
+    if (m.bundle_w != 0) {
+        const uint4 top = f.q0, bot = f.q1;
+        const float fx = f.fx0, fy = f.fy0;
+        float ch[8];
+#pragma unroll
+        for (int c = 0; c < 8; ++c) {
+            auto un = [&](uint32_t lo, uint32_t hi) {
+                const float q = (float)(((c < 4 ? lo : hi) >> (8 * (c & 3))) & 0xffu);
+                return FAST ? q * (1.0f / 255.0f) : q / 255.0f;
+            };
+            const float a = un(top.x, top.y), b = un(top.z, top.w), cc = un(bot.x, bot.y), dd = un(bot.z, bot.w);
+            const float tp = a + fx * (b - a), bt = cc + fx * (dd - cc);
+            ch[c] = tp + fy * (bt - tp);
+        }
+        out.albedo = make_float4(ch[0], ch[1], ch[2], 0.0f);
+        out.normal = make_float4(ch[3], ch[4], ch[5], 0.0f);
+        out.rm = make_float4(0.0f, ch[6], ch[7], 0.0f);
+        return;
+    }
+    if (m.tex[0] >= 0)
+        out.albedo = filter_footprint<FAST>(f.q0, f.fx0, f.fy0);
+    if (m.tex[1] >= 0)
+        out.normal = filter_footprint<FAST>(f.q1, f.fx1, f.fy1);
+    if (m.tex[2] >= 0)
+        out.rm = filter_footprint<FAST>(f.q2, f.fx2, f.fy2);
+}
+
+template <bool FAST = false>
+__device__ __forceinline__ bool reconstruct_surface(const ShadeHead& g, const TriShade& ts, float bu, float bv, const MapFetch& fetched, Surface& out)
 {
     const float b0 = 1.0f - (bu + bv), b1 = bu, b2 = bv;
     if (!g.valid)
@@ -743,13 +813,11 @@
     const float3 n0 = ts.n0, n1 = ts.n1, n2 = ts.n2;
     const float3 gn = normalize3<FAST>(f3(n0.x * b0 + n1.x * b1 + n2.x * b2, n0.y * b0 + n1.y * b1 + n2.y * b2, n0.z * b0 + n1.z * b1 + n2.z * b2));
     out.GN = normalize3<FAST>(xform_dir(g.m, gn));
-    const float u = ts.uv0.x * b0 + ts.uv1.x * b1 + ts.uv2.x * b2;
-    const float v = ts.uv0.y * b0 + ts.uv1.y * b1 + ts.uv2.y * b2;
     if (g.material < 0)
         return false;
     const DevMat& m = g.mat;
     MapSamples maps;
-    sample_material_maps<FAST>(S, m, u, v, maps);
+    filter_material_maps<FAST>(m, fetched, maps);
     if (m.tex[0] < 0) {
         out.albedo = f3(m.albedo[0], m.albedo[1], m.albedo[2]);
     } else {
diff --git a/nebulae_amd/csrc/gi_internal.h b/nebulae_amd/csrc/gi_internal.h
--- a/nebulae_amd/csrc/gi_internal.h
+++ b/nebulae_amd/csrc/gi_internal.h
@@ -127,6 +127,8 @@
     int32_t root;
     uint32_t n_qnodes;
 };
+
+constexpr int kRayCounters = 24, kGeomMismatchSlot = 16;
 
 struct GiState {
     SceneView view{};
@@ -161,7 +163,7 @@
     uint32_t traces = 0, resolves = 0;
     uint32_t begun = 0, finished = 0;
     uint32_t* d_direct_counts = nullptr;
-    unsigned long long last_stats[16] = {};
+    unsigned long long last_stats[kRayCounters] = {};
     int defer_resolve = 0;
     bool exact_shade = false;
     bool sort_shadow = true;
@@ -189,6 +191,7 @@
     int sun_hints = 4;
     bool compact_shadow = true;
     bool tail_tune = true;
+    bool tail_arm = false;
     int tail_phase = 0;
     bool tail_sorted = false;
     hipEvent_t tail_ev[4] = {nullptr, nullptr, nullptr, nullptr};
diff --git a/nebulae_amd/csrc/gi_sun_table.hip b/nebulae_amd/csrc/gi_sun_table.hip
--- a/nebulae_amd/csrc/gi_sun_table.hip
+++ b/nebulae_amd/csrc/gi_sun_table.hip
@@ -560,6 +560,7 @@
     g->sun_seen = 0;
     g->sun_table_builds++;
     g->tail_phase = g->tail_tune ? 1 : 0;
+    g->tail_arm = g->tail_tune;
     g->tail_sorted = false;
     return hipGetLastError();
 }
diff --git a/nebulae_amd/renderer.py b/nebulae_amd/renderer.py
--- a/nebulae_amd/renderer.py
+++ b/nebulae_amd/renderer.py
@@ -252,6 +252,11 @@
         self._check(self._lib.neb_gi_node_index_stats(self._ctx, v), "neb_gi_node_index_stats")
         return dict(zip(("below_64", "below_256", "below_1024", "below_4096", "deep_stack_phases"), [int(x) for x in v]))
 
+    def shade_geom_mismatches(self):
+        v = C.c_uint64()
+        self._check(self._lib.neb_gi_debug_shade_geom_mismatches(self._ctx, C.byref(v)), "neb_gi_debug_shade_geom_mismatches")
+        return int(v.value)
+
     def sun_table_stats(self):
         v = (C.c_uint64 * 4)()
         self._check(self._lib.neb_gi_sun_table_stats(self._ctx, v, C.c_void_p(self.info.stream if self.info else 0)), "neb_gi_sun_table_stats")
```
